# CVLAB-Unibo/Real-time-self-adaptive-deep-stereo

Measured on AMD Instinct MI355X. Metric: adapted stereo pairs/sec (whole node), MADNet full-backprop online adaptation 1242x375, higher is better.
Workload: dtype bf16 MFMA operands, f32 accumulate/storage (forward: split-bf16 = 3 MFMAs per product on the large 3x3 layers, exact f32 MFMA on the others, so the disparity stays within 1e-3 px; gradients: plain bf16); 1 GPU; MADNet FULL adaptation step (fwd+SSIM/L1 loss+EPE+bwd+momentum), 1242x375, 1 pair/GPU/step, private model per stream; precision=mixed, launch=hipGraph replay, step_sync=stream, concurrent_private_streams_per_gpu=1

## Files before the change

### include/madnet_hip_tune.h

```cpp
#ifndef MADNET_HIP_TUNE_H
#define MADNET_HIP_TUNE_H
#include <stdint.h>
#ifdef __cplusplus
extern "C" {
#endif

int mh_tune_conv_tile(int bm, int bn);
int mh_tune_conv_thin(int min_pixels);
int mh_tune_conv_patch(int mode);
int mh_tune_conv_x3_igemm(int on);
int mh_tune_conv_rows(int min_pixels);
int mh_tune_conv_bank_tile(int max_wgs);
int mh_tune_conv_bank_small(int mode);
int mh_tune_conv_bank(int small_maxpix);
int mh_tune_wgrad_wgs(int target_workgroups);
int mh_tune_wgrad_target_pct(int pct);
int mh_tune_wgrad_image(int on);
int mh_tune_wgrad_stream(int dist);
int mh_tune_corr(int direct);
int mh_tune_corr_row(int on);

int mh_tune_conv_planes(int mode);

#ifdef __cplusplus
}
#endif
#endif
```

### real-time-self-adaptive-deep-stereo_amd/csrc/corr.hip

```cpp
#include <algorithm>
#include <atomic>
#include <type_traits>
#include "mh_common.h"

namespace {

constexpr int MAXD_SMALL = 9;

struct CorrArgs {
    const float* L; const float* R; const float* u; float* out;
    int l_ld, r_ld, out_ld, coff;
    int B, H, W, C, md, stride, D;
    int copy_left, zero_tail, segs;
    unsigned l_bytes, r_bytes;
    int remap;
};

template <int LPP, int TW>
__global__ __launch_bounds__(256) void corr_fwd_small(CorrArgs p) {
    HIP_DYNAMIC_SHARED(float, smem)
    const int tid = threadIdx.x;
    const int seg = blockIdx.x % p.segs;
    const int row = blockIdx.x / p.segs;
    const int x0 = seg * TW;
// ... 218 lines not shown
            }
        }
        __syncthreads();
    }
    float w0[DT], w1[DT], uc = 0.f;
    int o0[DT], o1[DT];
#pragma unroll
    for (int j = 0; j < DT; ++j) {
#if defined(__clang__)
#pragma clang fp contract(off)
#endif
        const int xs = x + j - p.md;
        const bool in = live && j < p.D && (unsigned)xs < (unsigned)p.W;
        const int xq = in ? xs : 0;
        const float srcx = (float)xq * p.sx;
        const int x0 = (int)srcx, x1 = min(x0 + 1, p.Wc - 1);
        const float tx = srcx - (float)x0;
        float tl, tr, bl, br;
        if constexpr (HEAD) {
            const float* const Vs = fsm + 4 * (p.cwcap + 2) * p.K + 9 * p.K;
            const int i0 = in ? x0 - c_lo : 0, i1 = in ? x1 - c_lo : 0;
            tl = Vs[i0]; tr = Vs[i1]; bl = Vs[p.cwcap + i0]; br = Vs[p.cwcap + i1];
        } else { tl = V0[x0]; tr = V0[x1]; bl = V1[x0]; br = V1[x1]; }
        const float top = tl + (tr - tl) * tx, bot = bl + (br - bl) * tx;
        const float uj = (top + (bot - top) * ty) * p.mul;
        if (j == p.md) uc = uj;
        const float cx = (float)xq + uj;
        const float f0 = floorf(cx), f1 = f0 + 1.0f;
        const float xmax = (float)(p.W - 1);
        const float f0s = fminf(fmaxf(f0, 0.f), xmax), f1s = fminf(fmaxf(f1, 0.f), xmax);
        w0[j] = in ? (f1 - cx) * (f0 == f0s ? 1.f : 0.f) : 0.f;
        w1[j] = in ? (cx - f0) * (f1 == f1s ? 1.f : 0.f) : 0.f;
        o0[j] = in ? (row + (int)f0s) * p.r_ld * 4 : MH_OOB;
        o1[j] = in ? (row + (int)f1s) * p.r_ld * 4 : MH_OOB;
    }
    float accd[DT];
#pragma unroll
    for (int j = 0; j < DT; ++j) accd[j] = 0.f;
    float* Op = p.out + (int64_t)pp * p.out_ld;
    for (int c4 = sub; c4 < C4; c4 += LPP) {
        const float4 l = mh_buf_load4(rsL, live ? (pp * p.l_ld + c4 * 4) * 4 : MH_OOB);
        float4 a[DT], bb[DT];
#pragma unroll
        for (int j = 0; j < DT; ++j) {
            a[j] = mh_buf_load4(rsR, o0[j] == MH_OOB ? MH_OOB : o0[j] + c4 * 16);
            bb[j] = mh_buf_load4(rsR, o1[j] == MH_OOB ? MH_OOB : o1[j] + c4 * 16);
        }
        if (live) *reinterpret_cast<float4*>(Op + c4 * 4) = l;
        if (live && p.out_hi) {
            uint2 hi, lo;
            mh_split_bf16x2(l.x, l.y, hi.x, lo.x);
            mh_split_bf16x2(l.z, l.w, hi.y, lo.y);
            *reinterpret_cast<uint2*>(p.out_hi + (int64_t)pp * p.out_pld + c4 * 4) = hi;
            if (p.out_lo) *reinterpret_cast<uint2*>(p.out_lo + (int64_t)pp * p.out_pld + c4 * 4) = lo;
        }
#pragma unroll
        for (int j = 0; j < DT; ++j) {
            float4 r;
            r.x = w0[j] * a[j].x + w1[j] * bb[j].x; r.y = w0[j] * a[j].y + w1[j] * bb[j].y;
            r.z = w0[j] * a[j].z + w1[j] * bb[j].z; r.w = w0[j] * a[j].w + w1[j] * bb[j].w;
            accd[j] += l.x * r.x + l.y * r.y + l.z * r.z + l.w * r.w;
            if (j == p.md && live) *reinterpret_cast<float4*>(p.Rw + (int64_t)pp * p.rw_ld + c4 * 4) = r;
        }
    }
#pragma unroll
    for (int j = 0; j < DT; ++j) {
#pragma unroll
        for (int o = LPP >> 1; o > 0; o >>= 1) accd[j] += __shfl_xor(accd[j], o);
    }
    if (live) {
        const int nout = p.zero_tail ? p.out_ld - p.coff : p.D + 1;
        for (int e = sub; e < nout; e += LPP) {
            float v = 0.f;
#pragma unroll
            for (int j = 0; j < DT; ++j) v = (e == j) ? accd[j] * inv_c : v;
            if (e == p.D) v = uc;
            Op[p.coff + e] = v;
            if (p.out_hi && e <= p.D) {
                unsigned hi, lo;
                mh_split_bf16x2(v, 0.f, hi, lo);
                p.out_hi[(int64_t)pp * p.out_pld + p.coff + e] = (unsigned short)hi;
                if (p.out_lo) p.out_lo[(int64_t)pp * p.out_pld + p.coff + e] = (unsigned short)lo;
            }
        }
        if (sub == 0) p.u[pp] = uc;
    }
}

template <int TW>
__global__ __launch_bounds__(256) void corr_fwd_large(CorrArgs p) {
    HIP_DYNAMIC_SHARED(float, smem)
    const int tid = threadIdx.x;
    const int seg = blockIdx.x % p.segs;
    const int row = blockIdx.x / p.segs;
    const int x0 = seg * TW;
    const int C4 = p.C >> 2;
    const int rs = p.C + 4;
    const int win = TW + 2 * p.md;
    float* Ls = smem;
    float* Rs = smem + TW * rs;
    const float* Rrow = p.R + (int64_t)row * p.W * p.r_ld;
    const float* Lrow = p.L + (int64_t)row * p.W * p.l_ld;
    for (int q = tid; q < win * C4; q += 256) {
        const int px = q / C4, c4 = q - px * C4;
        const int xs = x0 - p.md + px;
        float4 v = make_float4(0.f, 0.f, 0.f, 0.f);
        if (xs >= 0 && xs < p.W) v = *reinterpret_cast<const float4*>(Rrow + (int64_t)xs * p.r_ld + c4 * 4);
        *reinterpret_cast<float4*>(&Rs[px * rs + c4 * 4]) = v;
    }
    for (int q = tid; q < TW * C4; q += 256) {
        const int px = q / C4, c4 = q - px * C4;
        const int x = x0 + px;
        float4 v = make_float4(0.f, 0.f, 0.f, 0.f);
        if (x < p.W) {
            v = *reinterpret_cast<const float4*>(Lrow + (int64_t)x * p.l_ld + c4 * 4);
            if (p.copy_left) *reinterpret_cast<float4*>(p.out + ((int64_t)row * p.W + x) * p.out_ld + c4 * 4) = v;
        }
        *reinterpret_cast<float4*>(&Ls[px * rs + c4 * 4]) = v;
    }
    __syncthreads();
    const float inv_c = 1.0f / (float)p.C;
    for (int q = tid; q < TW * p.D; q += 256) {
        const int pp = q / p.D, j = q - pp * p.D;
        const int x = x0 + pp;
        if (x >= p.W) continue;
        const float* l = &Ls[pp * rs];
        const float* r = &Rs[(pp + j * p.stride) * rs];
        float acc = 0.f;
        for (int c4 = 0; c4 < C4; ++c4) {
            const float4 a = *reinterpret_cast<const float4*>(l + c4 * 4);
            const float4 b = *reinterpret_cast<const float4*>(r + c4 * 4);
            acc += a.x * b.x + a.y * b.y + a.z * b.z + a.w * b.w;
        }
        p.out[((int64_t)row * p.W + x) * p.out_ld + p.coff + j] = acc * inv_c;
    }
    for (int pp = tid; pp < TW; pp += 256) {
        const int x = x0 + pp;
        if (x >= p.W) continue;
        const int64_t pix = (int64_t)row * p.W + x;
        float* Op = p.out + pix * p.out_ld;
        int tail = p.coff + p.D;
        if (p.u) { Op[tail] = p.u[pix]; ++tail; }
        if (p.zero_tail)
            for (; tail < p.out_ld; ++tail) Op[tail] = 0.f;
    }
}

struct CorrBwdArgs {
    const float* g; const float* L; const float* R; float* dL; float* dR; float* du;
    int g_ld, coff, l_ld, r_ld, dl_ld, dr_ld;
    int acc_l, acc_r, acc_u;
    int B, H, W, C, md, stride, D, copy_left;
    int64_t total;
};

__global__ __launch_bounds__(256) void corr_bwd_kernel(CorrBwdArgs p) {
    const int C4 = p.C >> 2;
    const float inv_c = 1.0f / (float)p.C;
    for (int64_t q = (int64_t)blockIdx.x * 256 + threadIdx.x; q < p.total; q += (int64_t)gridDim.x * 256) {
        const int c4 = (int)(q % C4);
        const int64_t pix = q / C4;
        const int x = (int)(pix % p.W);
        const int64_t rowbase = pix - x;
        const float* gp = p.g + pix * p.g_ld;
        float4 a = make_float4(0.f, 0.f, 0.f, 0.f), r = make_float4(0.f, 0.f, 0.f, 0.f);
        for (int j = 0; j < p.D; ++j) {
            const int i = j * p.stride - p.md;
            const int xs = x + i;
            if (xs >= 0 && xs < p.W) {
                const float gv = gp[p.coff + j];
                const float4 rv = *reinterpret_cast<const float4*>(p.R + (rowbase + xs) * p.r_ld + c4 * 4);
                a.x += gv * rv.x; a.y += gv * rv.y; a.z += gv * rv.z; a.w += gv * rv.w;
            }
            const int xl = x - i;
            if (xl >= 0 && xl < p.W) {
                const float gv = p.g[(rowbase + xl) * p.g_ld + p.coff + j];
                const float4 lv = *reinterpret_cast<const float4*>(p.L + (rowbase + xl) * p.l_ld + c4 * 4);
                r.x += gv * lv.x; r.y += gv * lv.y; r.z += gv * lv.z; r.w += gv * lv.w;
            }
        }
        a.x *= inv_c; a.y *= inv_c; a.z *= inv_c; a.w *= inv_c;
        r.x *= inv_c; r.y *= inv_c; r.z *= inv_c; r.w *= inv_c;
        if (p.copy_left) {
            const float4 gl = *reinterpret_cast<const float4*>(gp + c4 * 4);
            a.x += gl.x; a.y += gl.y; a.z += gl.z; a.w += gl.w;
        }
        float4* dl = reinterpret_cast<float4*>(p.dL + pix * p.dl_ld + c4 * 4);
        if (p.acc_l) { const float4 o = *dl; a.x += o.x; a.y += o.y; a.z += o.z; a.w += o.w; }
        *dl = a;
        float4* dr = reinterpret_cast<float4*>(p.dR + pix * p.dr_ld + c4 * 4);
        if (p.acc_r) { const float4 o = *dr; r.x += o.x; r.y += o.y; r.z += o.z; r.w += o.w; }
        *dr = r;
        if (p.du && c4 == 0) {
            const float gu = gp[p.coff + p.D];
            p.du[pix] = p.acc_u ? p.du[pix] + gu : gu;
        }
    }
}

template <int DT>
__global__ __launch_bounds__(256) void corr_bwd_direct(CorrBwdArgs p) {
    const int C4 = p.C >> 2;
    const float inv_c = 1.0f / (float)p.C;
    const int npix = p.B * p.H * p.W;
    const int q = blockIdx.x * 256 + threadIdx.x;
    const bool live = q < npix * C4;
    const int pix = live ? q / C4 : 0, c4 = live ? q - pix * C4 : 0;
    const int x = pix % p.W;
    const int rowbase = pix - x;
    const __amdgpu_buffer_rsrc_t rs_g = mh_make_rsrc(p.g, (unsigned)((size_t)npix * p.g_ld * 4));
    const __amdgpu_buffer_rsrc_t rs_r = mh_make_rsrc(p.R, (unsigned)(((size_t)npix - 1) * p.r_ld * 4 + (size_t)p.C * 4));
    const __amdgpu_buffer_rsrc_t rs_l = mh_make_rsrc(p.L, (unsigned)(((size_t)npix - 1) * p.l_ld * 4 + (size_t)p.C * 4));
    const __amdgpu_buffer_rsrc_t rs_dl = mh_make_rsrc(p.dL, (unsigned)(((size_t)npix - 1) * p.dl_ld * 4 + (size_t)p.C * 4));
    const __amdgpu_buffer_rsrc_t rs_dr = mh_make_rsrc(p.dR, (unsigned)(((size_t)npix - 1) * p.dr_ld * 4 + (size_t)p.C * 4));
    float gvr[DT], gvl[DT];
    float4 rvv[DT], lvv[DT];
    bool okr[DT], okl[DT];
#pragma unroll
    for (int j = 0; j < DT; ++j) {
        const int i = j * p.stride - p.md;
        const int xs = x + i, xl = x - i;
        okr[j] = live && j < p.D && xs >= 0 && xs < p.W; okl[j] = live && j < p.D && xl >= 0 && xl < p.W;
        gvr[j] = mh_buf_load1(rs_g, okr[j] ? (pix * p.g_ld + p.coff + j) * 4 : MH_OOB);
        gvl[j] = mh_buf_load1(rs_g, okl[j] ? ((rowbase + xl) * p.g_ld + p.coff + j) * 4 : MH_OOB);
        rvv[j] = mh_buf_load4(rs_r, okr[j] ? ((rowbase + xs) * p.r_ld + c4 * 4) * 4 : MH_OOB);
        lvv[j] = mh_buf_load4(rs_l, okl[j] ? ((rowbase + xl) * p.l_ld + c4 * 4) * 4 : MH_OOB);
    }
    const float4 gl = mh_buf_load4(rs_g, (live && p.copy_left) ? (pix * p.g_ld + c4 * 4) * 4 : MH_OOB);
    const float4 ol = mh_buf_load4(rs_dl, (live && p.acc_l) ? (pix * p.dl_ld + c4 * 4) * 4 : MH_OOB);
    const float4 orr = mh_buf_load4(rs_dr, (live && p.acc_r) ? (pix * p.dr_ld + c4 * 4) * 4 : MH_OOB);
    float4 a = make_float4(0.f, 0.f, 0.f, 0.f), r = make_float4(0.f, 0.f, 0.f, 0.f);
#pragma unroll
    for (int j = 0; j < DT; ++j) {
        if (okr[j]) { a.x += gvr[j] * rvv[j].x; a.y += gvr[j] * rvv[j].y; a.z += gvr[j] * rvv[j].z; a.w += gvr[j] * rvv[j].w; }
        if (okl[j]) { r.x += gvl[j] * lvv[j].x; r.y += gvl[j] * lvv[j].y; r.z += gvl[j] * lvv[j].z; r.w += gvl[j] * lvv[j].w; }
    }
    a.x *= inv_c; a.y *= inv_c; a.z *= inv_c; a.w *= inv_c;
    r.x *= inv_c; r.y *= inv_c; r.z *= inv_c; r.w *= inv_c;
    if (p.copy_left) { a.x += gl.x; a.y += gl.y; a.z += gl.z; a.w += gl.w; }
    if (p.acc_l) { a.x += ol.x; a.y += ol.y; a.z += ol.z; a.w += ol.w; }
    if (p.acc_r) { r.x += orr.x; r.y += orr.y; r.z += orr.z; r.w += orr.w; }
    if (!live) return;
    *reinterpret_cast<float4*>(p.dL + (int64_t)pix * p.dl_ld + c4 * 4) = a;
    *reinterpret_cast<float4*>(p.dR + (int64_t)pix * p.dr_ld + c4 * 4) = r;
    if (p.du && c4 == 0) {
        const float gu = p.g[(int64_t)pix * p.g_ld + p.coff + p.D];
        p.du[pix] = p.acc_u ? p.du[pix] + gu : gu;
    }
}

struct CorrWarpBwdArgs {
    const float* g; const float* L; const float* Rw; const float* img; const float* u;
    float* dL; float* dimg; float* du;
    int g_ld, coff, l_ld, rw_ld, img_ld, dl_ld, dimg_ld;
    int acc_l;
    int acc_img;
    int B, H, W, C, md, stride, D, copy_left;
};
template <int LPP, int DT = 0>
__global__ __launch_bounds__(256) void corr_warp_bwd_kernel(CorrWarpBwdArgs p) {
    const int C4 = p.C >> 2;
    constexpr int PPB = 256 / LPP;
    const float inv_c = 1.0f / (float)p.C;
    const int sub = threadIdx.x % LPP;
    const int64_t npix = (int64_t)p.B * p.H * p.W;
    const int64_t nit = (npix + PPB - 1) / PPB;
    for (int64_t it = blockIdx.x; it < nit; it += gridDim.x) {
        const int64_t pix = it * PPB + threadIdx.x / LPP;
        const bool live = pix < npix;
        const int64_t pp = live ? pix : 0;
        const int x = (int)(pp % p.W);
        const int64_t rowbase = pp - x;
        const float* gp = p.g + pp * p.g_ld;
        const float cx = (float)x + p.u[pp];
        const float x0 = floorf(cx), x1 = x0 + 1.0f;
        const float xmax = (float)(p.W - 1);
        const float x0s = fminf(fmaxf(x0, 0.f), xmax), x1s = fminf(fmaxf(x1, 0.f), xmax);
        const float m0 = (x0 == x0s) ? 1.f : 0.f, m1 = (x1 == x1s) ? 1.f : 0.f;
        const float w0 = (x1 - cx) * m0, w1 = (cx - x0) * m1;
        const int i0 = (int)x0s, i1 = (int)x1s;
        float dcx = 0.f;
        float gvr[DT > 0 ? DT : 1], gvl[DT > 0 ? DT : 1];
        int orw[DT > 0 ? DT : 1], ol[DT > 0 ? DT : 1];
        __amdgpu_buffer_rsrc_t rs_g, rs_rw, rs_l;
        if constexpr (DT > 0) {
            rs_g = mh_make_rsrc(p.g, (unsigned)(npix * p.g_ld * 4));
            rs_rw = mh_make_rsrc(p.Rw, (unsigned)(npix * p.rw_ld * 4));
            rs_l = mh_make_rsrc(p.L, (unsigned)(npix * p.l_ld * 4));
#pragma unroll
            for (int j = 0; j < DT; ++j) {
                const int i = j * p.stride - p.md;
                const int xs = x + i, xl = x - i;
                const bool okr = live && j < p.D && xs >= 0 && xs < p.W, okl = live && j < p.D && xl >= 0 && xl < p.W;
                gvr[j] = mh_buf_load1(rs_g, okr ? (int)((pp * p.g_ld + p.coff + j) * 4) : MH_OOB);
                gvl[j] = mh_buf_load1(rs_g, okl ? (int)(((rowbase + xl) * p.g_ld + p.coff + j) * 4) : MH_OOB);
                orw[j] = okr ? (int)((rowbase + xs) * p.rw_ld * 4) : MH_OOB;
                ol[j] = okl ? (int)((rowbase + xl) * p.l_ld * 4) : MH_OOB;
            }
        }
        for (int c4 = sub; c4 < C4; c4 += LPP) {
            if (!live) continue;
            float4 a = make_float4(0.f, 0.f, 0.f, 0.f), r = make_float4(0.f, 0.f, 0.f, 0.f);
            if constexpr (DT > 0) {
                float4 rvv[DT], lvv[DT];
#pragma unroll
                for (int j = 0; j < DT; ++j) {
                    rvv[j] = mh_buf_load4(rs_rw, orw[j] == MH_OOB ? MH_OOB : orw[j] + c4 * 16);
                    lvv[j] = mh_buf_load4(rs_l, ol[j] == MH_OOB ? MH_OOB : ol[j] + c4 * 16);
                }
#pragma unroll
                for (int j = 0; j < DT; ++j) {
                    if (orw[j] != MH_OOB) { a.x += gvr[j] * rvv[j].x; a.y += gvr[j] * rvv[j].y; a.z += gvr[j] * rvv[j].z; a.w += gvr[j] * rvv[j].w; }
                    if (ol[j] != MH_OOB) { r.x += gvl[j] * lvv[j].x; r.y += gvl[j] * lvv[j].y; r.z += gvl[j] * lvv[j].z; r.w += gvl[j] * lvv[j].w; }
                }
            } else
            for (int j = 0; j < p.D; ++j) {
                const int i = j * p.stride - p.md;
                const int xs = x + i;
                if (xs >= 0 && xs < p.W) {
                    const float gv = gp[p.coff + j];
                    const float4 rv = *reinterpret_cast<const float4*>(p.Rw + (rowbase + xs) * p.rw_ld + c4 * 4);
                    a.x += gv * rv.x; a.y += gv * rv.y; a.z += gv * rv.z; a.w += gv * rv.w;
                }
                const int xl = x - i;
                if (xl >= 0 && xl < p.W) {
                    const float gv = p.g[(rowbase + xl) * p.g_ld + p.coff + j];
                    const float4 lv = *reinterpret_cast<const float4*>(p.L + (rowbase + xl) * p.l_ld + c4 * 4);
                    r.x += gv * lv.x; r.y += gv * lv.y; r.z += gv * lv.z; r.w += gv * lv.w;
                }
            }
            a.x *= inv_c; a.y *= inv_c; a.z *= inv_c; a.w *= inv_c;
            r.x *= inv_c; r.y *= inv_c; r.z *= inv_c; r.w *= inv_c;
            if (p.copy_left) {
                const float4 gl = *reinterpret_cast<const float4*>(gp + c4 * 4);
                a.x += gl.x; a.y += gl.y; a.z += gl.z; a.w += gl.w;
            }
            float4* dl = reinterpret_cast<float4*>(p.dL + pp * p.dl_ld + c4 * 4);
            if (p.acc_l) { const float4 o = *dl; a.x += o.x; a.y += o.y; a.z += o.z; a.w += o.w; }
            *dl = a;
            if (p.dimg) {
                float* d0 = p.dimg + (rowbase + i0) * p.dimg_ld + c4 * 4;
                float* d1 = p.dimg + (rowbase + i1) * p.dimg_ld + c4 * 4;
                if (w0 != 0.f) { mh_atomic_add(d0 + 0, w0 * r.x); mh_atomic_add(d0 + 1, w0 * r.y); mh_atomic_add(d0 + 2, w0 * r.z); mh_atomic_add(d0 + 3, w0 * r.w); }
                if (w1 != 0.f) { mh_atomic_add(d1 + 0, w1 * r.x); mh_atomic_add(d1 + 1, w1 * r.y); mh_atomic_add(d1 + 2, w1 * r.z); mh_atomic_add(d1 + 3, w1 * r.w); }
            }
            if (p.du) {
                const float4 s0 = *reinterpret_cast<const float4*>(p.img + (rowbase + i0) * p.img_ld + c4 * 4);
                const float4 s1 = *reinterpret_cast<const float4*>(p.img + (rowbase + i1) * p.img_ld + c4 * 4);
                dcx += r.x * (m1 * s1.x - m0 * s0.x) + r.y * (m1 * s1.y - m0 * s0.y) + r.z * (m1 * s1.z - m0 * s0.z) + r.w * (m1 * s1.w - m0 * s0.w);
            }
        }
        if (p.du) {
#pragma unroll
            for (int o = LPP >> 1; o > 0; o >>= 1) dcx += __shfl_xor(dcx, o);
            if (live && sub == 0) p.du[pp] = gp[p.coff + p.D] + dcx;
        }
    }
}

template <int LPP, int DT, bool DET>
__global__ __launch_bounds__(1024) void corr_warp_bwd_row_kernel(CorrWarpBwdArgs p) {
    HIP_DYNAMIC_SHARED(float, smem)
    constexpr int NT = 1024, PPB = NT / LPP;
    using acc_t = typename std::conditional<DET, unsigned long long, float>::type;
    acc_t* const racc = reinterpret_cast<acc_t*>(smem);
    float* const su = smem + (size_t)p.W * p.C * (DET ? 2 : 1);
    const int tid = threadIdx.x, sub = tid % LPP;
    const int C4 = p.C >> 2;
    const float inv_c = 1.0f / (float)p.C;
    const int row = blockIdx.x;
    const int rowbase = row * p.W;
    const int npix = p.B * p.H * p.W;
    const __amdgpu_buffer_rsrc_t rs_g = mh_make_rsrc(p.g, (unsigned)((size_t)npix * p.g_ld * 4));
    const __amdgpu_buffer_rsrc_t rs_rw = mh_make_rsrc(p.Rw, (unsigned)((size_t)npix * p.rw_ld * 4));
    const __amdgpu_buffer_rsrc_t rs_l = mh_make_rsrc(p.L, (unsigned)((size_t)npix * p.l_ld * 4));
    const __amdgpu_buffer_rsrc_t rs_img = mh_make_rsrc(p.img, (unsigned)((size_t)npix * p.img_ld * 4));
    const __amdgpu_buffer_rsrc_t rs_dl = mh_make_rsrc(p.dL, (unsigned)((size_t)npix * p.dl_ld * 4));
    const int nq = p.W * C4;
    if constexpr (DET) {
        for (int i = tid; i < p.W * p.C; i += NT) racc[i] = 0ull;
    } else {
        for (int q = tid; q < nq; q += NT) {
            const int x = q / C4, c4 = q - x * C4;
            float4 v = make_float4(0.f, 0.f, 0.f, 0.f);
            if (p.dimg) v = *reinterpret_cast<const float4*>(p.dimg + (int64_t)(rowbase + x) * p.dimg_ld + c4 * 4);
            *reinterpret_cast<float4*>(racc + x * p.C + c4 * 4) = v;
        }
    }
    for (int x = tid; x < p.W; x += NT) su[x] = p.u[rowbase + x];
    __syncthreads();
    for (int xb = 0; xb < p.W; xb += PPB) {
        const int x = xb + tid / LPP;
        const bool live = x < p.W;
        const int pp = rowbase + (live ? x : 0);
// ... 855 lines not shown
    return ((size_t)4 * (cw + 2) * K + 9 * K + 2 * cw) * sizeof(float) <= 48 * 1024 ? 1 : 0;
}

static int level_front_launch(const float* X, int32_t x_ld, int32_t K, const float* hw, const float* hb,
                              const float* Vc, int32_t Hc, int32_t Wc, float mul, const float* L, int32_t l_ld, const float* R,
                              int32_t r_ld, float* out, int32_t out_ld, int32_t coff, float* Rw, int32_t rw_ld, float* u,
                              int32_t B, int32_t H, int32_t W, int32_t C, int32_t max_disp, int32_t zero_tail,
                              void* out_hi, void* out_lo, int32_t out_pld, void* stream) {
    MH_REQUIRE(!out_lo || out_hi, MH_ERR_ARG, "mh_level_front_fwd_planes: the lo plane needs the hi plane");
    MH_REQUIRE(!out_hi || (out_pld >= coff + 2 * max_disp + 2 && (out_pld & 3) == 0 && (((uintptr_t)out_hi) & 7u) == 0 && (((uintptr_t)out_lo) & 7u) == 0), MH_ERR_ARG,
               "mh_level_front_fwd_planes: out_pld must cover coff + D + 1 (multiple of 4), planes 8-byte aligned");
    MH_REQUIRE(Vc && L && R && out && Rw && u, MH_ERR_ARG, "mh_level_front_fwd: null argument");
    MH_REQUIRE(B > 0 && H > 0 && W > 0 && C > 0 && Hc > 0 && Wc > 0 && max_disp >= 0, MH_ERR_ARG, "mh_level_front_fwd: bad dimension");
    const int D = 2 * max_disp + 1;
    MH_REQUIRE(D <= MAXD_SMALL, MH_ERR_UNSUPPORTED, "mh_level_front_fwd: at most %d shifts (use mh_resize_fwd + mh_warp_fwd + mh_corr_fwd)", MAXD_SMALL);
    MH_REQUIRE(C % 4 == 0 && l_ld % 4 == 0 && r_ld % 4 == 0 && rw_ld % 4 == 0 && out_ld % 4 == 0 && mh_aligned16(L) && mh_aligned16(R) &&
               mh_aligned16(Rw) && mh_aligned16(out), MH_ERR_ALIGN, "mh_level_front_fwd: 16-byte rows required");
    MH_REQUIRE(coff >= C && coff + D + 1 <= out_ld && rw_ld >= C, MH_ERR_ARG, "mh_level_front_fwd: out_ld / coff / rw_ld too small");
    const int64_t npix = (int64_t)B * H * W;
    const int64_t lb = ((npix - 1) * l_ld + C) * 4, rb = ((npix - 1) * r_ld + C) * 4;
    MH_REQUIRE(npix < (1ll << 31) - 256 && lb < (1ll << 31) - 64 && rb < (1ll << 31) - 64, MH_ERR_UNSUPPORTED, "mh_level_front_fwd: tensors must be < 2 GiB");
    FrontArgs a;
    a.Vc = Vc; a.L = L; a.R = R; a.out = out; a.Rw = Rw; a.u = u; a.Hc = Hc; a.Wc = Wc; a.mul = mul;
    a.sy = (float)Hc / (float)H; a.sx = (float)Wc / (float)W;
    a.l_ld = l_ld; a.r_ld = r_ld; a.out_ld = out_ld; a.rw_ld = rw_ld; a.coff = coff;
    a.B = B; a.H = H; a.W = W; a.C = C; a.md = max_disp; a.D = D; a.zero_tail = zero_tail;
    a.l_bytes = (unsigned)lb; a.r_bytes = (unsigned)rb;
    a.out_hi = (unsigned short*)out_hi; a.out_lo = (unsigned short*)out_lo; a.out_pld = out_pld;
    a.X = nullptr; a.hw = nullptr; a.hb = nullptr; a.Vw = nullptr; a.x_ld = 0; a.K = 0; a.segs = 0; a.cwcap = 0; a.x_bytes = 0; a.rows2 = 0; a.rowpairs = 0;
    hipStream_t s = (hipStream_t)stream;
    const int C4 = C / 4;
    const int lpp = C4 <= 4 ? 4 : (C4 <= 8 ? 8 : 16);
    if (X) {
        MH_REQUIRE(mh_level_front_head_ok(Hc, Wc, H, W, C, K, max_disp) == 1, MH_ERR_UNSUPPORTED,
                   "mh_level_front_head_fwd: K = %d channels / %dx%d -> %dx%d not served (ask mh_level_front_head_ok; run the head as a launch of its own)", K, Hc, Wc, H, W);
        MH_REQUIRE(hw && x_ld >= K && x_ld % 4 == 0 && mh_aligned16(X) && mh_aligned16(hw), MH_ERR_ALIGN, "mh_level_front_head_fwd: X rows / head weights must be 16-byte aligned");
        const int64_t xb = (((int64_t)B * Hc * Wc - 1) * x_ld + K) * 4;
        MH_REQUIRE(xb < (1ll << 31) - 64, MH_ERR_UNSUPPORTED, "mh_level_front_head_fwd: X must be < 2 GiB");
        a.X = X; a.hw = hw; a.hb = hb; a.Vw = const_cast<float*>(Vc); a.x_ld = x_ld; a.K = K; a.x_bytes = (unsigned)xb;
        const int ppb = 256 / lpp;
        a.rows2 = (H == 2 * Hc && g_front_rows2.load(std::memory_order_relaxed)) ? 1 : 0;
        const int wpx = a.rows2 ? ppb / 2 : ppb;
        a.rowpairs = H / 2;
        a.segs = mh_cdiv(W, wpx);
        a.cwcap = front_head_cwcap(Wc, W, wpx, max_disp);
        const size_t lds = ((size_t)4 * (a.cwcap + 2) * K + 9 * K + 2 * a.cwcap) * sizeof(float);
        const dim3 g((unsigned)((int64_t)a.segs * B * (a.rows2 ? H / 2 : H)));
#define MH_FRONTH(LPPv)                                                                                                      \
    { if (D <= 5) hipLaunchKernelGGL((level_front_kernel<LPPv, 5, true>), g, dim3(256), lds, s, a);                          \
      else hipLaunchKernelGGL((level_front_kernel<LPPv, MAXD_SMALL, true>), g, dim3(256), lds, s, a); }
        if (lpp == 4) MH_FRONTH(4) else if (lpp == 8) MH_FRONTH(8) else MH_FRONTH(16)
#undef MH_FRONTH
        mh_note_kernel("level_front_kernel<LPP=%d,DT=%d,HEAD=%d> grid %d lds %d", lpp, D <= 5 ? 5 : MAXD_SMALL, K, (int)g.x, (int)lds);
        return mh_check_launch("level_front_head_fwd");
    }
    auto grid = [&](int l) { return dim3((unsigned)((npix * l + 255) / 256)); };
#define MH_FRONT(LPPv)                                                                                              \
    { if (D <= 5) hipLaunchKernelGGL((level_front_kernel<LPPv, 5, false>), grid(LPPv), dim3(256), 0, s, a);                \
      else hipLaunchKernelGGL((level_front_kernel<LPPv, MAXD_SMALL, false>), grid(LPPv), dim3(256), 0, s, a); }
    if (lpp == 4) MH_FRONT(4) else if (lpp == 8) MH_FRONT(8) else MH_FRONT(16)
#undef MH_FRONT
    mh_note_kernel("level_front_kernel<LPP=%d,DT=%d>", lpp, D <= 5 ? 5 : MAXD_SMALL);
    return mh_check_launch("level_front_fwd");
}

extern "C" int mh_level_front_fwd_planes(const float* Vc, int32_t Hc, int32_t Wc, float mul, const float* L, int32_t l_ld, const float* R,
                                         int32_t r_ld, float* out, int32_t out_ld, int32_t coff, float* Rw, int32_t rw_ld, float* u,
                                         int32_t B, int32_t H, int32_t W, int32_t C, int32_t max_disp, int32_t zero_tail,
                                         void* out_hi, void* out_lo, int32_t out_pld, void* stream) {
    return level_front_launch(nullptr, 0, 0, nullptr, nullptr, Vc, Hc, Wc, mul, L, l_ld, R, r_ld, out, out_ld, coff, Rw, rw_ld, u, B, H, W, C, max_disp, zero_tail, out_hi, out_lo,
                              out_pld, stream);
}
extern "C" int mh_level_front_head_fwd(const float* X, int32_t x_ld, int32_t K, const float* hw, const float* hb, float* Vc, int32_t Hc, int32_t Wc, float mul,
                                       const float* L, int32_t l_ld, const float* R, int32_t r_ld, float* out, int32_t out_ld, int32_t coff, float* Rw, int32_t rw_ld,
                                       float* u, int32_t B, int32_t H, int32_t W, int32_t C, int32_t max_disp, int32_t zero_tail,
                                       void* out_hi, void* out_lo, int32_t out_pld, void* stream) {
    MH_REQUIRE(X, MH_ERR_ARG, "mh_level_front_head_fwd: null argument");
    return level_front_launch(X, x_ld, K, hw, hb, Vc, Hc, Wc, mul, L, l_ld, R, r_ld, out, out_ld, coff, Rw, rw_ld, u, B, H, W, C, max_disp, zero_tail, out_hi, out_lo, out_pld,
                              stream);
}

extern "C" int mh_corr_warp_bwd(const float* g, int32_t g_ld, int32_t coff, const float* L, int32_t l_ld, const float* Rw, int32_t rw_ld,
                                const float* img, int32_t img_ld, const float* u, float* dL, int32_t dl_ld, int32_t acc_l,
                                float* dimg, int32_t dimg_ld, float* du,
                                int32_t B, int32_t H, int32_t W, int32_t C, int32_t max_disp, int32_t stride, int32_t copy_left, void* stream) {
    MH_REQUIRE(g && L && Rw && img && u && dL && (dimg || du), MH_ERR_ARG, "mh_corr_warp_bwd: null argument");
    MH_REQUIRE(B > 0 && H > 0 && W > 0 && C > 0 && max_disp >= 0 && stride >= 1, MH_ERR_ARG, "mh_corr_warp_bwd: bad dimension");
    MH_REQUIRE(C % 4 == 0 && l_ld % 4 == 0 && rw_ld % 4 == 0 && img_ld % 4 == 0 && dl_ld % 4 == 0 && (!dimg || dimg_ld % 4 == 0) &&
               mh_aligned16(L) && mh_aligned16(Rw) && mh_aligned16(img) && mh_aligned16(dL), MH_ERR_ALIGN,
               "mh_corr_warp_bwd: channel counts / lds must be multiples of 4 and pointers 16-byte aligned");
    MH_REQUIRE(!copy_left || (g_ld % 4 == 0 && mh_aligned16(g)), MH_ERR_ALIGN, "mh_corr_warp_bwd: copy_left needs aligned g rows");
    CorrWarpBwdArgs a;
    a.g = g; a.L = L; a.Rw = Rw; a.img = img; a.u = u; a.dL = dL; a.dimg = dimg; a.du = du;
    a.g_ld = g_ld; a.coff = coff; a.l_ld = l_ld; a.rw_ld = rw_ld; a.img_ld = img_ld; a.dl_ld = dl_ld; a.dimg_ld = dimg_ld;
    a.acc_l = acc_l & 1;
    a.acc_img = (acc_l & MH_CORR_WARP_OVERWRITE_DIMG) ? 0 : 1;
    a.B = B; a.H = H; a.W = W; a.C = C; a.md = max_disp; a.stride = stride; a.D = 2 * max_disp / stride + 1; a.copy_left = copy_left;
    const int C4 = C / 4;
    const int64_t npix = (int64_t)B * H * W;
    hipStream_t s = (hipStream_t)stream;
    auto zero_dimg = [&]() -> int {
        if (a.acc_img || !dimg) return 0;
        hipError_t e = (dimg_ld == C) ? hipMemsetAsync(dimg, 0, (size_t)npix * C * 4, s) : hipMemset2DAsync(dimg, (size_t)dimg_ld * 4, 0, (size_t)C * 4, (size_t)npix, s);
        if (e != hipSuccess) { mh_set_error("mh_corr_warp_bwd: zeroing dimg: %s", hipGetErrorString(e)); return (int)e; }
        a.acc_img = 1;
        return 0;
    };
    auto grid = [&](int lpp) { int64_t b = (npix * lpp + 255) / 256; return (int)(b > (1 << 20) ? (1 << 20) : b); };
    const int64_t ldmax = g_ld > rw_ld ? (g_ld > l_ld ? g_ld : l_ld) : (rw_ld > l_ld ? rw_ld : l_ld);
    const bool fast = a.D <= 5 && npix * ldmax * 4 < (1ll << 31) - 64;
    const bool det = g_corr_det_ranges.load() > 0;
    const size_t row_lds = ((size_t)W * C * (det ? 8 : 4) + (size_t)W * 4 + 15) & ~(size_t)15;
    const int64_t ldmax2 = std::max<int64_t>(std::max<int64_t>(ldmax, img_ld), std::max<int64_t>(dl_ld, dimg ? dimg_ld : 0));
    if (g_corr_row.load() && fast && row_lds <= 150 * 1024 && npix * ldmax2 * 4 < (1ll << 31) - 64 && (int64_t)B * H < (1 << 30)) {
        const dim3 grid((unsigned)(B * H));
        const int lpp = C4 <= 8 ? 8 : C4 <= 16 ? 16 : 32;
        const size_t lds_st = ((size_t)3 * W * C + (size_t)W * (8 + 1 + 2 + 1 + 1 + 2 + 8) + 8) * 4;
        if ((g_corr_row.load() & 2) == 0 && C4 <= 32 && W <= 3 * (1024 / lpp) && (int64_t)W * C4 <= 3 * 1024 && W * 8 <= 3 * 1024 && W < 32768 && lds_st <= 155 * 1024) {
            if (g_corr_row.load() & 4) a.dimg = nullptr;
            if (lpp == 8) hipLaunchKernelGGL((corr_warp_bwd_rowlds_kernel<8, 5>), grid, dim3(1024), lds_st, s, a);
            else if (lpp == 16) hipLaunchKernelGGL((corr_warp_bwd_rowlds_kernel<16, 5>), grid, dim3(1024), lds_st, s, a);
            else hipLaunchKernelGGL((corr_warp_bwd_rowlds_kernel<32, 5>), grid, dim3(1024), lds_st, s, a);
            mh_note_kernel("corr_warp_bwd_rowlds_kernel<LPP=%d,DT=5> C=%d D=%d grid %d x 16 waves lds %d", lpp, C, a.D, B * H, (int)lds_st);
            return mh_check_launch("corr_warp_bwd_rowlds");
        }
        if (int rc = zero_dimg()) return rc;
#define MH_CWB_ROW(LPPv) { if (det) hipLaunchKernelGGL((corr_warp_bwd_row_kernel<LPPv, 5, true>), grid, dim3(1024), row_lds, s, a);   \
                           else hipLaunchKernelGGL((corr_warp_bwd_row_kernel<LPPv, 5, false>), grid, dim3(1024), row_lds, s, a); }
        if (C4 <= 4) MH_CWB_ROW(4) else if (C4 <= 8) MH_CWB_ROW(8) else MH_CWB_ROW(16)
#undef MH_CWB_ROW
        mh_note_kernel("corr_warp_bwd_row_kernel<LPP=%d,DT=5%s> C=%d D=%d grid %d x 16 waves lds %d", C4 <= 4 ? 4 : C4 <= 8 ? 8 : 16, det ? ",det" : "", C, a.D, B * H, (int)row_lds);
        return mh_check_launch("corr_warp_bwd_row");
    }
    if (int rc = zero_dimg()) return rc;
    if (fast) {
        if (C4 <= 4) hipLaunchKernelGGL((corr_warp_bwd_kernel<4, 5>), dim3(grid(4)), dim3(256), 0, s, a);
        else if (C4 <= 8) hipLaunchKernelGGL((corr_warp_bwd_kernel<8, 5>), dim3(grid(8)), dim3(256), 0, s, a);
        else hipLaunchKernelGGL((corr_warp_bwd_kernel<16, 5>), dim3(grid(16)), dim3(256), 0, s, a);
    } else if (C4 <= 4) hipLaunchKernelGGL((corr_warp_bwd_kernel<4>), dim3(grid(4)), dim3(256), 0, s, a);
    else if (C4 <= 8) hipLaunchKernelGGL((corr_warp_bwd_kernel<8>), dim3(grid(8)), dim3(256), 0, s, a);
    else hipLaunchKernelGGL((corr_warp_bwd_kernel<16>), dim3(grid(16)), dim3(256), 0, s, a);
    mh_note_kernel("corr_warp_bwd_kernel<LPP=%d%s> C=%d D=%d", C4 <= 4 ? 4 : C4 <= 8 ? 8 : 16, fast ? ",DT=5" : "", C, a.D);
    return mh_check_launch("corr_warp_bwd");
}

extern "C" int mh_corr_bwd(const float* g, int32_t g_ld, int32_t coff, const float* L, int32_t l_ld,
                           const float* R, int32_t r_ld, float* dL, int32_t dl_ld, int32_t acc_l,
                           float* dR, int32_t dr_ld, int32_t acc_r, float* du, int32_t acc_u,
                           int32_t B, int32_t H, int32_t W, int32_t C, int32_t max_disp, int32_t stride,
                           int32_t copy_left, void* stream) {
    return mh_corr_bwd_prec(g, g_ld, coff, L, l_ld, R, r_ld, dL, dl_ld, acc_l, dR, dr_ld, acc_r, du, acc_u, B, H, W, C, max_disp, stride, copy_left, 0, stream);
}

extern "C" int mh_corr_bwd_prec(const float* g, int32_t g_ld, int32_t coff, const float* L, int32_t l_ld,
                                const float* R, int32_t r_ld, float* dL, int32_t dl_ld, int32_t acc_l,
                                float* dR, int32_t dr_ld, int32_t acc_r, float* du, int32_t acc_u,
                                int32_t B, int32_t H, int32_t W, int32_t C, int32_t max_disp, int32_t stride,
                                int32_t copy_left, int32_t precision, void* stream) {
    MH_REQUIRE(precision >= 0 && precision <= 2, MH_ERR_ARG, "mh_corr_bwd_prec: precision must be 0 (fp32), 1 (bf16) or 2 (split-bf16: runs as fp32)");
    MH_REQUIRE(g && L && R && dL && dR, MH_ERR_ARG, "mh_corr_bwd: null argument");
    MH_REQUIRE(B > 0 && H > 0 && W > 0 && C > 0 && max_disp >= 0 && stride >= 1, MH_ERR_ARG, "mh_corr_bwd: bad dimension");
    MH_REQUIRE(C % 4 == 0 && l_ld % 4 == 0 && r_ld % 4 == 0 && dl_ld % 4 == 0 && dr_ld % 4 == 0 &&
               mh_aligned16(L) && mh_aligned16(R) && mh_aligned16(dL) && mh_aligned16(dR), MH_ERR_ALIGN,
               "mh_corr_bwd: channel counts / lds must be multiples of 4 and pointers 16-byte aligned");
    MH_REQUIRE(!copy_left || (g_ld % 4 == 0 && mh_aligned16(g)), MH_ERR_ALIGN, "mh_corr_bwd: copy_left needs aligned g rows");
    CorrBwdArgs a;
    a.g = g; a.L = L; a.R = R; a.dL = dL; a.dR = dR; a.du = du;
    a.g_ld = g_ld; a.coff = coff; a.l_ld = l_ld; a.r_ld = r_ld; a.dl_ld = dl_ld; a.dr_ld = dr_ld;
    a.acc_l = acc_l; a.acc_r = acc_r; a.acc_u = acc_u;
    a.B = B; a.H = H; a.W = W; a.C = C; a.md = max_disp; a.stride = stride; a.D = 2 * max_disp / stride + 1;
    a.copy_left = copy_left;
    a.total = (int64_t)B * H * W * (C / 4);
    if (precision == 1 && g_corr_direct && a.D > MAXD_SMALL && stride == 1 && !copy_left && !du && C % 16 == 0 && C >= 32 && C <= 256 &&
        (C == 32 || C == 64 || C == 128 || C == 256) && (int64_t)B * H * W * std::max(std::max(g_ld, l_ld), r_ld) * 4 < (1ll << 31) - 64) {
        const int nks = (2 * max_disp + 16 + 31) / 32, rows = 48 + 32 * nks, DPh = (((a.D + 3) & ~3) + 7) & ~7;
        const size_t tile = (size_t)64 * (C + 4) * 4;
        const size_t lds_r = std::max(tile, ((size_t)rows * (C + 16) + (size_t)rows * DPh) * 2);
        if (lds_r <= 150 * 1024) {
            const int segs = mh_cdiv(W, 64);
            const dim3 grid(segs * B * H);
            hipStream_t s = (hipStream_t)stream;
            const int remap = g_corr_remap.load();
#define MH_CORRBH(CSv) { if (g_corr_pair.load()) hipLaunchKernelGGL((corr_bwd_mfma_bf16_pair<CSv>), dim3(2 * segs * B * H), dim3(256), lds_r, s, a, segs, remap);  \
                         else { hipLaunchKernelGGL((corr_bwd_mfma_bf16_one<CSv, false>), dim3(segs * B * H), dim3(256), lds_r, s, a, segs, remap);                   \
                                hipLaunchKernelGGL((corr_bwd_mfma_bf16_one<CSv, true>), dim3(segs * B * H), dim3(256), lds_r, s, a, segs, remap); } }
            switch (C) {
                case 32: MH_CORRBH(2) break;
                case 64: MH_CORRBH(4) break;
                case 128: MH_CORRBH(8) break;
                default: MH_CORRBH(16) break;
            }
#undef MH_CORRBH
            mh_note_kernel("corr_bwd_mfma_bf16_pair<C/16=%d> left + right in %s of %d x 4 waves, lds %d", C / 16, g_corr_pair.load() ? "one grid" : "two grids", (g_corr_pair.load() ? 2 : 1) * segs * B * H, (int)lds_r);
            return mh_check_launch("corr_bwd_mfma_bf16");
        }
    }
    {
        const int nb = (2 * max_disp + 31) / 16, rows = 48 + 16 * nb, DP = (a.D + 3) & ~3;
        const size_t lds_l = ((size_t)rows * (C + 4) + 64 * DP) * sizeof(float), lds_r = ((size_t)rows * (C + 4) + (size_t)rows * DP) * sizeof(float);
        if (g_corr_direct && a.D > MAXD_SMALL && stride == 1 && !copy_left && !du && (C == 16 || C == 32 || C == 64 || C == 128 || C == 256) &&
            lds_r <= 150 * 1024 && (int64_t)B * H * W < (1ll << 31) / 64) {
            const int segs = mh_cdiv(W, 64);
            const dim3 grid(segs * B * H);
            hipStream_t s = (hipStream_t)stream;
#define MH_CORRB(CSv)                                                                                        \
            hipLaunchKernelGGL((corr_bwd_mfma<CSv, false>), grid, dim3(CSv >= 2 ? 512 : 256), lds_l, s, a, segs);  \
            hipLaunchKernelGGL((corr_bwd_mfma<CSv, true>), grid, dim3(CSv >= 2 ? 512 : 256), lds_r, s, a, segs);
            switch (C) {
                case 16: MH_CORRB(1) break;
                case 32: MH_CORRB(2) break;
                case 64: MH_CORRB(4) break;
                case 128: MH_CORRB(8) break;
                default: MH_CORRB(16) break;
            }
#undef MH_CORRB
            mh_note_kernel("corr_bwd_mfma<C/16=%d> left + right (exact fp32)", C / 16);
            return mh_check_launch("corr_bwd_mfma");
        }
    }
    {
        const int64_t npix = (int64_t)B * H * W;
        const int64_t ldm = std::max(std::max(std::max(g_ld, l_ld), std::max(r_ld, dl_ld)), dr_ld);
        if (g_corr_direct && a.D <= 5 && npix * ldm * 4 < (1ll << 31) - 64 && a.total < (1ll << 31) - 256) {
            hipLaunchKernelGGL(corr_bwd_direct<5>, dim3((unsigned)((a.total + 255) / 256)), dim3(256), 0, (hipStream_t)stream, a);
            mh_note_kernel("corr_bwd_direct<DT=5> C=%d D=%d", C, a.D);
            return mh_check_launch("corr_bwd_direct");
        }
    }
    int blocks = (int)((a.total + 255) / 256);
    if (blocks > 256 * 16) blocks = 256 * 16;
    hipLaunchKernelGGL(corr_bwd_kernel, dim3(blocks), dim3(256), 0, (hipStream_t)stream, a);
    mh_note_kernel("corr_bwd_kernel C=%d D=%d", C, a.D);
    return mh_check_launch("corr_bwd");
}

extern "C" int mh_det_sync_corr(const void* t) {
    g_corr_det_ranges = reinterpret_cast<const mh_det_table*>(t)->n;
    return mh_det_upload(*reinterpret_cast<const mh_det_table*>(t));
}
extern "C" int mh_det_ovf_corr(void) { return mh_det_overflow_take(); }
```

### real-time-self-adaptive-deep-stereo_amd/csrc/lib.hip

```cpp
#include "mh_common.h"
#include <stdarg.h>
#include <string.h>
#include <mutex>
#include <vector>

static thread_local char g_err[512] = "";

void mh_set_error(const char* fmt, ...) {
    va_list ap;
    va_start(ap, fmt);
    vsnprintf(g_err, sizeof(g_err), fmt, ap);
    va_end(ap);
}

static thread_local char g_last_kernel[160] = "";
void mh_note_kernel(const char* fmt, ...) {
    va_list ap;
    va_start(ap, fmt);
    vsnprintf(g_last_kernel, sizeof(g_last_kernel), fmt, ap);
    va_end(ap);
}
extern "C" const char* mh_last_kernel(void) { return g_last_kernel; }

int mh_check_launch(const char* what) {
// ... 196 lines not shown
            mh_conv_desc d; desc_from_op(o, d);
            return mh_conv2d_planes_bwd(&d, p[0], i[23], p[1], p[2], i[24], (float*)p[3], p[4], i[25], s);
        }
        case MH_OP_CONV_IMAGE:
            return mh_conv_image_fwd((const float*)p[0], i[0], i[1], i[2], i[3], i[4], i[5], i[6], i[7], o.f[0], o.f[1], (const float*)p[1], (const float*)p[2], i[8], i[9], i[10],
                                     i[11], o.f[2], (float*)p[3], i[12], p[4], i[13], s);
        case MH_OP_DET_FLUSH:
            return mh_det_flush((float*)p[0], p[1], o.n, s);
        case MH_OP_ALLREDUCE: {
            float* bufs[MH_ALLREDUCE_MAX_BUFS]; int64_t counts[MH_ALLREDUCE_MAX_BUFS];
            const int nb = i[0];
            if (nb < 1 || nb > MH_ALLREDUCE_MAX_BUFS) { mh_set_error("MH_OP_ALLREDUCE: %d buffers", nb); return MH_ERR_ARG; }
            for (int k = 0; k < nb; ++k) { bufs[k] = (float*)p[1 + k]; counts[k] = i[1 + k]; }
            return mh_allreduce_sum(bufs, counts, nb, p[0], s);
        }
        case MH_OP_FETCH_INPUTS: {
            float* dst[MH_FETCH_MAX]; int64_t cnt[MH_FETCH_MAX];
            const int nb = i[0];
            if (nb < 1 || nb > MH_FETCH_MAX) { mh_set_error("MH_OP_FETCH_INPUTS: %d entries", nb); return MH_ERR_ARG; }
            for (int k = 0; k < nb; ++k) { dst[k] = (float*)p[1 + k]; cnt[k] = i[1 + k]; }
            return mh_fetch_inputs((const mh_input_table*)p[0], dst, cnt, nb, s);
        }
        case MH_OP_STAMP:
            return mh_stamp(p[0], s);
        case MH_OP_PLANE_SPLIT:
            return mh_plane_split((const mh_plane_seg*)p[0], i[0], i[1], s);
        case MH_OP_PACK_W:
            return mh_pack_weights((const mh_pack_seg*)p[0], i[0], i[1], s);
        case MH_OP_WGRAD_REDUCE:
            return mh_wgrad_reduce((const mh_wgrad_seg*)p[0], i[0], i[1], s);
        case MH_OP_CORR_FWD:
            return mh_corr_fwd_prec((const float*)p[0], i[0], (const float*)p[1], i[1], (const float*)p[2], (float*)p[3], i[2], i[3],
                                    i[4], i[5], i[6], i[7], i[8], i[9], i[10], i[11], i[12], s);
        case MH_OP_CORR_BWD:
            return mh_corr_bwd_prec((const float*)p[0], i[0], i[1], (const float*)p[1], i[2], (const float*)p[2], i[3],
                                    (float*)p[3], i[4], i[5], (float*)p[4], i[6], i[7], (float*)p[5], i[8],
                                    i[9], i[10], i[11], i[12], i[13], i[14], i[15], i[16], s);
        case MH_OP_WARP_FWD:
            return mh_warp_fwd((const float*)p[0], i[0], (const float*)p[1], (float*)p[2], i[1], i[2], i[3], i[4], i[5], s);
        case MH_OP_WARP_BWD:
            return mh_warp_bwd((const float*)p[0], i[0], (const float*)p[1], i[1], (const float*)p[2], (float*)p[3], i[2],
                               (float*)p[4], i[3], i[4], i[5], i[6], i[7], s);
        case MH_OP_RESIZE_FWD:
            return mh_resize_fwd((const float*)p[0], (float*)p[1], i[0], i[1], i[2], i[3], i[4], i[5], i[6], i[7], i[8], o.f[0], i[9], s);
        case MH_OP_RESIZE_BWD:
            return mh_resize_bwd((const float*)p[0], (const float*)p[1], (float*)p[2], i[10], i[0], i[1], i[2], i[3], i[4], i[5], i[6],
                                 i[7], i[8], o.f[0], i[9], s);
        case MH_OP_LEVEL_FRONT:
            if (p[8])
                return mh_level_front_head_fwd((const float*)p[8], i[14], i[15], (const float*)p[9], (const float*)p[10], (float*)p[0], i[0], i[1], o.f[0],
                                               (const float*)p[1], i[2], (const float*)p[2], i[3], (float*)p[3], i[4], i[5], (float*)p[4], i[6], (float*)p[5],
                                               i[7], i[8], i[9], i[10], i[11], i[12], p[6], p[7], i[13], s);
            return mh_level_front_fwd_planes((const float*)p[0], i[0], i[1], o.f[0], (const float*)p[1], i[2], (const float*)p[2], i[3], (float*)p[3],
                                             i[4], i[5], (float*)p[4], i[6], (float*)p[5], i[7], i[8], i[9], i[10], i[11], i[12], p[6], p[7], i[13], s);
        case MH_OP_RESIZE_IMAGE:
            return mh_resize_image_fwd((const float*)p[0], (float*)p[1], i[0], i[1], i[2], i[3], i[4], i[5], s);
        case MH_OP_PAD_REFLECT:
            return mh_pad_reflect((const float*)p[0], (float*)p[1], i[0], i[1], i[2], i[3], i[4], i[5], i[6], i[7], i[8], o.f[0], o.f[1], s);
        case MH_OP_LOSS:
            return mh_reprojection_loss_phase((const float*)p[0], (const float*)p[1], (const float*)p[2], (float*)p[3], (float*)p[4],
                                              (float*)p[5], o.f[0], i[0], i[1], i[2], i[3], s);
        case MH_OP_METRICS:
            return mh_metrics((const float*)p[0], (const float*)p[1], (float*)p[2], (float*)p[3], o.f[0], i[0], i[1], i[2], s);
        case MH_OP_MOMENTUM:
            return mh_momentum((float*)p[0], (float*)p[1], (const float*)p[2], o.n, o.f[0], o.f[1], o.f[2], s);
        case MH_OP_COPY_CH:
            return mh_copy_channels((const float*)p[0], i[0], (float*)p[1], i[1], o.n, i[2], o.f[0], i[3], s);
        case MH_OP_LEAKY_BWD:
            return mh_leaky_bwd((float*)p[0], i[0], (const float*)p[1], i[1], o.n, i[2], o.f[0], s);
        case MH_OP_FILL:
            return mh_fill((float*)p[0], o.n, o.f[0], s);
        case MH_OP_BIAS_GRAD:
            if (i[2] > 0) return mh_bias_grad_partial((const float*)p[0], i[0], o.n, i[1], (float*)p[1], i[2], s);
            return mh_bias_grad((const float*)p[0], i[0], o.n, i[1], (float*)p[1], s);
        default:
            mh_set_error("mh_plan_run: unknown op kind %d", o.kind);
            return MH_ERR_ARG;
    }
}

#define MH_HIP(call)                                                        \
    do {                                                                    \
        hipError_t e_ = (call);                                             \
        if (e_ != hipSuccess) {                                             \
            mh_set_error("%s: %s", #call, hipGetErrorString(e_));           \
            return (int)e_;                                                 \
        }                                                                   \
    } while (0)

namespace {
struct Lanes {
    hipStream_t aux[MH_MAX_LANES] = {};
    hipEvent_t ev[32] = {};
    int next = 0;
    bool ready = false;
};
struct LanePool {
    std::mutex m;
    std::vector<Lanes*> free_[16];
};
LanePool& lane_pool() { static LanePool* p = new LanePool; return *p; }
struct ThreadLanes {
    Lanes* l[16] = {};
    ~ThreadLanes() {
        LanePool& P = lane_pool();
        std::lock_guard<std::mutex> g(P.m);
        for (int d = 0; d < 16; ++d)
            if (l[d]) { P.free_[d].push_back(l[d]); l[d] = nullptr; }
    }
};
thread_local ThreadLanes t_lanes;

int lane_device(int* dev) {
    MH_HIP(hipGetDevice(dev));
    MH_REQUIRE(*dev >= 0 && *dev < 16, MH_ERR_UNSUPPORTED, "device index %d out of range", *dev);
    return 0;
}
int lanes_take(int dev, Lanes** out) {
    LanePool& P = lane_pool();
    Lanes* L = nullptr;
    {
        std::lock_guard<std::mutex> g(P.m);
        if (!P.free_[dev].empty()) { L = P.free_[dev].back(); P.free_[dev].pop_back(); }
    }
    if (!L) {
        L = new Lanes;
        for (int k = 1; k < MH_MAX_LANES; ++k) MH_HIP(hipStreamCreateWithFlags(&L->aux[k], hipStreamNonBlocking));
        for (auto& e : L->ev) MH_HIP(hipEventCreateWithFlags(&e, hipEventDisableTiming));
        L->ready = true;
    }
    *out = L;
    return 0;
}
int lanes_get(Lanes** out) {
    int dev = 0;
    if (int e = lane_device(&dev)) return e;
    if (!t_lanes.l[dev])
        if (int e = lanes_take(dev, &t_lanes.l[dev])) return e;
    *out = t_lanes.l[dev];
    return 0;
}
}
static int mh_lanes_init() { Lanes* L = nullptr; return lanes_get(&L); }
namespace {
int lane_edge(Lanes& L, hipStream_t from, hipStream_t to) {
    hipEvent_t e = L.ev[L.next];
    L.next = (L.next + 1) & 31;
    MH_HIP(hipEventRecord(e, from));
    MH_HIP(hipStreamWaitEvent(to, e, 0));
    return 0;
}
}

static int run_wgrad_batch(const mh_op* ops, int m, void* s) {
    mh_wgrad_item items[16];
    for (int k = 0; k < m; ++k) {
        const mh_op& o = ops[k];
        desc_from_op(o, items[k].d);
        items[k].in = (const float*)o.p[0]; items[k].dout = (const float*)o.p[1];
        items[k].ws = (float*)o.p[2]; items[k].db = (float*)o.p[3];
        items[k].dout_ld = o.i[21]; items[k].splits = o.i[23];
        items[k].group_max_m = o.i[24]; items[k].reserved = 0;
    }
    return mh_conv2d_wgrad_partial_group(items, m, s);
}

static int plan_run_impl(const mh_op* ops, int32_t nops, void* stream, Lanes* fixed) {
    MH_REQUIRE(ops || nops == 0, MH_ERR_ARG, "mh_plan_run: null plan");
    Lanes* L = fixed;
    bool dirty[MH_MAX_LANES] = {};
    bool stale[MH_MAX_LANES];
    for (bool& b : stale) b = true;
    hipStream_t main_s = (hipStream_t)stream;
    auto join = [&]() -> int {
        for (int l = 1; l < MH_MAX_LANES; ++l)
            if (dirty[l]) { if (int e = lane_edge(*L, L->aux[l], main_s)) return e; dirty[l] = false; }
        return 0;
    };
    struct Deferred { int32_t k; int m, lane; };
    Deferred deferred[64];
    int ndef = 0;
    auto flush_deferred = [&]() -> int {
        for (int q = 0; q < ndef; ++q) {
            const Deferred& d = deferred[q];
            const int e = d.m > 1 ? run_wgrad_batch(ops + d.k, d.m, (void*)L->aux[d.lane]) : run_op(ops[d.k], (void*)L->aux[d.lane]);
            if (e) { ndef = 0; return e; }
        }
        ndef = 0;
        return 0;
    };
    for (int32_t k = 0; k < nops; ++k) {
        const int sched = ops[k].i[26];
        const int lane = sched & 0xff;
        int e = 0;
        if (lane >= MH_MAX_LANES) { mh_set_error("lane %d out of range", lane); e = MH_ERR_ARG; }
        if (!e && ndef && ((sched & MH_OP_JOIN) || ((sched >> 16) & 0xff) || ndef >= 60)) e = flush_deferred();
        if (!e && (sched & MH_OP_JOIN)) e = join();
        if (!e && ((sched >> 16) & 0xff)) {
            if (lane > 0 && !L) e = lanes_get(&L);
            hipStream_t tgt = lane > 0 ? L->aux[lane] : main_s;
            for (int l = 1; l < MH_MAX_LANES && !e; ++l)
                if ((((sched >> 16) >> l) & 1) && l != lane && dirty[l]) {
                    e = lane_edge(*L, L->aux[l], tgt);
                    if (lane == 0) dirty[l] = false;
                }
        }
        int m = 1;
        if (ops[k].kind == MH_OP_WGRAD_PARTIAL)
            while (m < 16 && k + m < nops && ops[k + m].kind == MH_OP_WGRAD_PARTIAL && (ops[k + m].i[26] & ~MH_OP_NODEFER) == lane) ++m;
        auto run = [&](void* s) -> int { return m > 1 ? run_wgrad_batch(ops + k, m, s) : run_op(ops[k], s); };
        if (!e && lane > 0) {
            if (!L) e = lanes_get(&L);
            if (!e && stale[lane]) { e = lane_edge(*L, main_s, L->aux[lane]); stale[lane] = false; }
            if (!e) {
                dirty[lane] = true;
                const bool at_once = (sched & MH_OP_NODEFER) && !((sched >> 16) & 0xff);
                if (!at_once) { deferred[ndef].k = k; deferred[ndef].m = m; deferred[ndef].lane = lane; ++ndef; }
                else {
                    if (ndef) e = flush_deferred();
                    if (!e) e = run((void*)L->aux[lane]);
                }
            }
        } else if (!e) {
            e = run(stream);
            for (bool& b : stale) b = true;
            if (!e && ndef) e = flush_deferred();
        }
        if (e != 0) {
            char tmp[400];
            strncpy(tmp, g_err, sizeof(tmp) - 1); tmp[sizeof(tmp) - 1] = 0;
            mh_set_error("plan op %d (kind %d): %s", k, ops[k].kind, tmp);
            ndef = 0;
            join();
            return e;
        }
        k += m - 1;
    }
    if (ndef) { if (int e = flush_deferred()) { join(); return e; } }
    return join();
}

extern "C" int mh_plan_run(const mh_op* ops, int32_t nops, void* stream) { return plan_run_impl(ops, nops, stream, nullptr); }

namespace {
struct ThreadBranches {
    std::vector<Lanes*> sets[16];
    ~ThreadBranches() {
        LanePool& P = lane_pool();
        std::lock_guard<std::mutex> g(P.m);
        for (int d = 0; d < 16; ++d) { for (Lanes* L : sets[d]) P.free_[d].push_back(L); sets[d].clear(); }
    }
};
thread_local ThreadBranches t_branches;
int branch_get(int idx, Lanes** out) {
    int dev = 0;
    if (int e = lane_device(&dev)) return e;
    auto& v = t_branches.sets[dev];
    while ((int)v.size() <= idx) {
        Lanes* L = nullptr;
        if (int e = lanes_take(dev, &L)) return e;
        v.push_back(L);
    }
    *out = v[idx];
    return 0;
}
}
extern "C" int mh_plans_prepare(int32_t nplans) {
    MH_REQUIRE(nplans >= 1 && nplans <= 16, MH_ERR_ARG, "mh_plans_prepare: 1 .. 16 plans");
    for (int i = 1; i < nplans; ++i) { Lanes* L = nullptr; if (int e = branch_get(i - 1, &L)) return e; }
    return mh_lanes_init();
}
extern "C" int mh_plans_run(const mh_plan_ref* plans, int32_t nplans, void* stream) {
    MH_REQUIRE(plans && nplans >= 1 && nplans <= 16, MH_ERR_ARG, "mh_plans_run: 1 .. 16 plans");
    for (int i = 0; i < nplans; ++i) {
        MH_REQUIRE(plans[i].ops || plans[i].nops == 0, MH_ERR_ARG, "mh_plans_run: null plan %d", i);
        for (int k = 0; k < plans[i].nops; ++k)
            MH_REQUIRE((plans[i].ops[k].i[26] & 0xff) < MH_MAX_LANES - 1, MH_ERR_UNSUPPORTED, "mh_plans_run: plan %d uses lane %d (the last lane is the branch stream)", i,
                       plans[i].ops[k].i[26] & 0xff);
    }
    hipStream_t s0 = (hipStream_t)stream;
    Lanes* sets[16] = {};
    for (int i = 1; i < nplans; ++i) {
        if (int e = branch_get(i - 1, &sets[i])) return e;
        if (int e = lane_edge(*sets[i], s0, sets[i]->aux[MH_MAX_LANES - 1])) return e;
    }
    int rc = 0;
    for (int i = 0; i < nplans && !rc; ++i)
        rc = plan_run_impl(plans[i].ops, plans[i].nops, i == 0 ? (void*)s0 : (void*)sets[i]->aux[MH_MAX_LANES - 1], i == 0 ? nullptr : sets[i]);
    for (int i = 1; i < nplans; ++i)
        if (int e = lane_edge(*sets[i], sets[i]->aux[MH_MAX_LANES - 1], s0)) { if (!rc) rc = e; }
    return rc;
}


extern "C" int mh_graph_begin(void* stream) {
    { Lanes* L = nullptr; if (int e = lanes_get(&L)) return e; }
    MH_HIP(hipStreamBeginCapture((hipStream_t)stream, hipStreamCaptureModeThreadLocal));
    return 0;
}
extern "C" int mh_graph_end(void* stream, void** graph_exec_out) {
    MH_REQUIRE(graph_exec_out, MH_ERR_ARG, "mh_graph_end: null output");
    hipGraph_t g = nullptr;
    MH_HIP(hipStreamEndCapture((hipStream_t)stream, &g));
    hipGraphExec_t ge = nullptr;
    hipError_t e = hipGraphInstantiate(&ge, g, nullptr, nullptr, 0);
    (void)hipGraphDestroy(g);
    if (e != hipSuccess) { mh_set_error("hipGraphInstantiate: %s", hipGetErrorString(e)); return (int)e; }
    *graph_exec_out = (void*)ge;
    return 0;
}
extern "C" int mh_graph_launch(void* graph_exec, void* stream) {
    MH_HIP(hipGraphLaunch((hipGraphExec_t)graph_exec, (hipStream_t)stream));
    return 0;
}
extern "C" int mh_graph_destroy(void* graph_exec) {
    if (graph_exec) MH_HIP(hipGraphExecDestroy((hipGraphExec_t)graph_exec));
    return 0;
}
extern "C" int mh_event_create(void** ev) {
    MH_REQUIRE(ev, MH_ERR_ARG, "mh_event_create: null output");
    hipEvent_t e; MH_HIP(hipEventCreate(&e)); *ev = (void*)e; return 0;
}
extern "C" int mh_event_record(void* ev, void* stream) { MH_HIP(hipEventRecord((hipEvent_t)ev, (hipStream_t)stream)); return 0; }
extern "C" int mh_event_elapsed_ms(void* a, void* b, float* ms) {
    MH_REQUIRE(ms, MH_ERR_ARG, "mh_event_elapsed_ms: null output");
    MH_HIP(hipEventSynchronize((hipEvent_t)b));
    MH_HIP(hipEventElapsedTime(ms, (hipEvent_t)a, (hipEvent_t)b));
    return 0;
}
extern "C" int mh_event_destroy(void* ev) { if (ev) MH_HIP(hipEventDestroy((hipEvent_t)ev)); return 0; }
extern "C" int mh_stream_sync(void* stream) { MH_HIP(hipStreamSynchronize((hipStream_t)stream)); return 0; }
```

### real-time-self-adaptive-deep-stereo_amd/csrc/ops.hip

```cpp
#include "mh_common.h"

namespace {

__device__ __forceinline__ float clampf(float v, float lo, float hi) { return fminf(fmaxf(v, lo), hi); }

struct WarpArgs {
    const float* img; const float* u; const float* g; float* out; float* dimg; float* du;
    int img_ld, out_ld, g_ld, dimg_ld, acc_u;
    int B, H, W, C;
    int64_t total;
};

__global__ __launch_bounds__(256) void warp_fwd_kernel(WarpArgs p) {
    const int C4 = p.C >> 2;
    for (int64_t q = (int64_t)blockIdx.x * 256 + threadIdx.x; q < p.total; q += (int64_t)gridDim.x * 256) {
        const int c4 = (int)(q % C4);
        const int64_t pix = q / C4;
        const int x = (int)(pix % p.W);
        const int64_t rowbase = pix - x;
        const float cx = (float)x + p.u[pix];
        const float x0 = floorf(cx), x1 = x0 + 1.0f;
        const float xmax = (float)(p.W - 1);
        const float x0s = clampf(x0, 0.f, xmax), x1s = clampf(x1, 0.f, xmax);
        const float w0 = (x1 - cx) * (x0 == x0s ? 1.f : 0.f);
        const float w1 = (cx - x0) * (x1 == x1s ? 1.f : 0.f);
        const float4 a = *reinterpret_cast<const float4*>(p.img + (rowbase + (int)x0s) * p.img_ld + c4 * 4);
        const float4 b = *reinterpret_cast<const float4*>(p.img + (rowbase + (int)x1s) * p.img_ld + c4 * 4);
        float4 o;
        o.x = w0 * a.x + w1 * b.x; o.y = w0 * a.y + w1 * b.y;
        o.z = w0 * a.z + w1 * b.z; o.w = w0 * a.w + w1 * b.w;
        *reinterpret_cast<float4*>(p.out + pix * p.out_ld + c4 * 4) = o;
    }
}

template <int LPP>
__global__ __launch_bounds__(256) void warp_bwd_kernel(WarpArgs p) {
    const int C4 = p.C >> 2;
    constexpr int PPB = 256 / LPP;
    const int sub = threadIdx.x % LPP;
    const int64_t npix = (int64_t)p.B * p.H * p.W;
    const int64_t nit = (npix + PPB - 1) / PPB;
    for (int64_t it = blockIdx.x; it < nit; it += gridDim.x) {
        const int64_t pix = it * PPB + threadIdx.x / LPP;
        const bool live = pix < npix;
        const int64_t pp = live ? pix : 0;
        const int x = (int)(pp % p.W);
        const int64_t rowbase = pp - x;
        const float cx = (float)x + p.u[pp];
        const float x0 = floorf(cx), x1 = x0 + 1.0f;
        const float xmax = (float)(p.W - 1);
        const float x0s = clampf(x0, 0.f, xmax), x1s = clampf(x1, 0.f, xmax);
        const float m0 = (x0 == x0s) ? 1.f : 0.f, m1 = (x1 == x1s) ? 1.f : 0.f;
        const float w0 = (x1 - cx) * m0, w1 = (cx - x0) * m1;
        const int i0 = (int)x0s, i1 = (int)x1s;
        float dcx = 0.f;
        for (int c4 = sub; c4 < C4; c4 += LPP) {
            if (!live) continue;
            const float4 gv = *reinterpret_cast<const float4*>(p.g + pp * p.g_ld + c4 * 4);
            if (p.dimg) {
                float* d0 = p.dimg + (rowbase + i0) * p.dimg_ld + c4 * 4;
                float* d1 = p.dimg + (rowbase + i1) * p.dimg_ld + c4 * 4;
                if (w0 != 0.f) { mh_atomic_add(d0 + 0, w0 * gv.x); mh_atomic_add(d0 + 1, w0 * gv.y); mh_atomic_add(d0 + 2, w0 * gv.z); mh_atomic_add(d0 + 3, w0 * gv.w); }
                if (w1 != 0.f) { mh_atomic_add(d1 + 0, w1 * gv.x); mh_atomic_add(d1 + 1, w1 * gv.y); mh_atomic_add(d1 + 2, w1 * gv.z); mh_atomic_add(d1 + 3, w1 * gv.w); }
            }
            if (p.du) {
                const float4 a = *reinterpret_cast<const float4*>(p.img + (rowbase + i0) * p.img_ld + c4 * 4);
                const float4 b = *reinterpret_cast<const float4*>(p.img + (rowbase + i1) * p.img_ld + c4 * 4);
                dcx += gv.x * (m1 * b.x - m0 * a.x) + gv.y * (m1 * b.y - m0 * a.y) +
                       gv.z * (m1 * b.z - m0 * a.z) + gv.w * (m1 * b.w - m0 * a.w);
            }
        }
        if (p.du) {
#pragma unroll
            for (int o = LPP >> 1; o > 0; o >>= 1) dcx += __shfl_xor(dcx, o);
            if (live && sub == 0) p.du[pp] = p.acc_u ? p.du[pp] + dcx : dcx;
        }
    }
}

struct ResizeArgs {
    const float* in; const float* g; float* out; float* din;
    int B, Hi, Wi, Hr, Wr, cy, cx, Ho, Wo, mode, accumulate;
    float mul, sy, sx;
};

__device__ __forceinline__ void interp1(int i, float scale, int n, int& lo, int& hi, float& t) {
    const float src = (float)i * scale;
    lo = (int)src;
    hi = min(lo + 1, n - 1);
    t = src - (float)lo;
}

__device__ __forceinline__ float bilerp(const float* img, int Wi, int y0, int y1, float ty, int x0, int x1, float tx,
                                        float mul, bool relu_in) {
#if defined(__clang__)
#pragma clang fp contract(off)
#endif
    float tl = img[(int64_t)y0 * Wi + x0], tr = img[(int64_t)y0 * Wi + x1];
    float bl = img[(int64_t)y1 * Wi + x0], br = img[(int64_t)y1 * Wi + x1];
    if (relu_in) {
        tl = fmaxf(tl * mul, 0.f); tr = fmaxf(tr * mul, 0.f);
        bl = fmaxf(bl * mul, 0.f); br = fmaxf(br * mul, 0.f);
    }
    const float top = tl + (tr - tl) * tx;
    const float bot = bl + (br - bl) * tx;
    return top + (bot - top) * ty;
}

__global__ __launch_bounds__(256) void resize_fwd_kernel(ResizeArgs p) {
    const int64_t total = (int64_t)p.B * p.Ho * p.Wo;
    for (int64_t q = (int64_t)blockIdx.x * 256 + threadIdx.x; q < total; q += (int64_t)gridDim.x * 256) {
        const int x = (int)(q % p.Wo);
        const int64_t t2 = q / p.Wo;
        const int y = (int)(t2 % p.Ho);
        const int b = (int)(t2 / p.Ho);
        int y0, y1, x0, x1; float ty, tx;
        interp1(y + p.cy, p.sy, p.Hi, y0, y1, ty);
        interp1(x + p.cx, p.sx, p.Wi, x0, x1, tx);
        const float* img = p.in + (int64_t)b * p.Hi * p.Wi;
        float v = bilerp(img, p.Wi, y0, y1, ty, x0, x1, tx, p.mul, p.mode == 1);
        if (p.mode == 0) v *= p.mul;
        else if (p.mode == 2) v = fmaxf(v * p.mul, 0.f);
        p.out[q] = v;
    }
}

template <int LPP>
__global__ __launch_bounds__(256) void resize_bwd_kernel(ResizeArgs p) {
    const int64_t total = (int64_t)p.B * p.Hi * p.Wi;
    const float isy = 1.0f / p.sy, isx = 1.0f / p.sx;
    const int sub = LPP > 1 ? (int)(threadIdx.x % LPP) : 0;
    const int64_t nit = (total * LPP + 255) / 256;
    for (int64_t it = blockIdx.x; it < nit; it += gridDim.x) {
        const int64_t q0 = (it * 256 + threadIdx.x) / LPP;
        const bool live = q0 < total;
        const int64_t q = live ? q0 : 0;
        const int sx = (int)(q % p.Wi);
        const int64_t t2 = q / p.Wi;
        const int sy = (int)(t2 % p.Hi);
        const int b = (int)(t2 / p.Hi);
        const float* img = p.in + (int64_t)b * p.Hi * p.Wi;
        const float* gimg = p.g + (int64_t)b * p.Ho * p.Wo;
        const int ya = max(p.cy, (int)floorf((float)(sy - 1) * isy) - 1);
        const int yb = min(p.cy + p.Ho - 1, (int)ceilf((float)(sy + 1) * isy) + 1);
        const int xa = max(p.cx, (int)floorf((float)(sx - 1) * isx) - 1);
        const int xb = min(p.cx + p.Wo - 1, (int)ceilf((float)(sx + 1) * isx) + 1);
        float acc = 0.f;
        for (int Y = ya + sub; Y <= yb && live; Y += LPP) {
            int y0, y1; float ty;
            interp1(Y, p.sy, p.Hi, y0, y1, ty);
            const float wy = (y0 == sy ? 1.0f - ty : 0.f) + (y1 == sy ? ty : 0.f);
            if (wy == 0.f) continue;
            for (int X = xa; X <= xb; ++X) {
                int x0, x1; float tx;
                interp1(X, p.sx, p.Wi, x0, x1, tx);
                const float wx = (x0 == sx ? 1.0f - tx : 0.f) + (x1 == sx ? tx : 0.f);
                if (wx == 0.f) continue;
                float gv = gimg[(int64_t)(Y - p.cy) * p.Wo + (X - p.cx)];
                if (p.mode == 2) {
                    const float z = bilerp(img, p.Wi, y0, y1, ty, x0, x1, tx, p.mul, false) * p.mul;
                    if (!(z > 0.f)) gv = 0.f;
                }
                acc += gv * wy * wx;
            }
        }
#pragma unroll
        for (int o = LPP >> 1; o > 0; o >>= 1) acc += __shfl_xor(acc, o);
        if (live && sub == 0) {
            acc *= p.mul;
            if (p.mode == 1 && !(img[(int64_t)sy * p.Wi + sx] * p.mul > 0.f)) acc = 0.f;
            p.din[q] = p.accumulate ? p.din[q] + acc : acc;
        }
    }
}

struct HeadBwdArgs {
    ResizeArgs rz;
    const float* a1; const float* a2; int a1_ld, a2_ld;
    float* dV; unsigned short* dV_sh; int dV_sh_ld;
    const float* w; float* dx; const float* mask_ref; unsigned short* dx_sh;
    int N, dx_ld, mask_ld, dx_sh_ld, acc_dx, kind;
    float mask_alpha;
    int tiles_x, tiles_y;
};
#define HB_TH 4
#define HB_TW 32
__device__ __forceinline__ float head_dv_from_du(const ResizeArgs& p, int b, int sy, int sx, bool exact2) {
    const float* gimg = p.g + (int64_t)b * p.Ho * p.Wo;
    if (exact2) {
        float v[9], wgt[9];
        bool ok[9];
#pragma unroll
        for (int dy = -1; dy <= 1; ++dy) {
            const int Y = 2 * sy + dy;
            const bool oky = (unsigned)Y < (unsigned)p.Ho;
            const int Yc = oky ? Y : 2 * sy;
            const float wy = dy == 0 ? 1.0f : ((dy == 1 && sy == p.Hi - 1) ? 1.0f : 0.5f);
#pragma unroll
            for (int dx = -1; dx <= 1; ++dx) {
                const int X = 2 * sx + dx;
                const bool okx = (unsigned)X < (unsigned)p.Wo;
                const int Xc = okx ? X : 2 * sx;
                const float wx = dx == 0 ? 1.0f : ((dx == 1 && sx == p.Wi - 1) ? 1.0f : 0.5f);
                const int k = (dy + 1) * 3 + dx + 1;
                v[k] = gimg[(int64_t)Yc * p.Wo + Xc] * wy;
                wgt[k] = wx; ok[k] = oky && okx;
            }
        }
        float acc = 0.f;
#pragma unroll
        for (int k = 0; k < 9; ++k) acc += ok[k] ? v[k] * wgt[k] : 0.f;
        return acc * p.mul;
    }
    const float isy = 1.0f / p.sy, isx = 1.0f / p.sx;
    const int ya = max(p.cy, (int)floorf((float)(sy - 1) * isy) - 1);
    const int yb = min(p.cy + p.Ho - 1, (int)ceilf((float)(sy + 1) * isy) + 1);
    const int xa = max(p.cx, (int)floorf((float)(sx - 1) * isx) - 1);
    const int xb = min(p.cx + p.Wo - 1, (int)ceilf((float)(sx + 1) * isx) + 1);
    float acc = 0.f;
    for (int Y = ya; Y <= yb; ++Y) {
        int y0, y1; float ty;
        interp1(Y, p.sy, p.Hi, y0, y1, ty);
        const float wy = (y0 == sy ? 1.0f - ty : 0.f) + (y1 == sy ? ty : 0.f);
        if (wy == 0.f) continue;
        for (int X = xa; X <= xb; ++X) {
            int x0, x1; float tx;
            interp1(X, p.sx, p.Wi, x0, x1, tx);
            const float wx = (x0 == sx ? 1.0f - tx : 0.f) + (x1 == sx ? tx : 0.f);
            if (wx == 0.f) continue;
            acc += gimg[(int64_t)(Y - p.cy) * p.Wo + (X - p.cx)] * wy * wx;
        }
    }
    return acc * p.mul;
}
__global__ __launch_bounds__(256) void head_bwd_kernel(HeadBwdArgs p) {
    __shared__ float sV[(HB_TH + 2) * (HB_TW + 2)];
    __shared__ __attribute__((aligned(16))) float sW[9 * 64];
    const int tid = threadIdx.x;
    const int H = p.rz.Hi, W = p.rz.Wi;
    const int tx = blockIdx.x % p.tiles_x;
    const int t2 = blockIdx.x / p.tiles_x;
    const int ty = t2 % p.tiles_y, b = t2 / p.tiles_y;
    const int y0 = ty * HB_TH, x0 = tx * HB_TW;
    const bool exact2 = p.kind == 0 && p.rz.Hr == 2 * H && p.rz.Wr == 2 * W && p.rz.cy == 0 && p.rz.cx == 0 && p.rz.Ho == p.rz.Hr && p.rz.Wo == p.rz.Wr;
    for (int i = tid; i < 9 * p.N; i += 256) sW[i] = p.w[i];
    if (tid < (HB_TH + 2) * (HB_TW + 2)) {
        const int ly = tid / (HB_TW + 2), lx = tid - ly * (HB_TW + 2);
        const int y = y0 - 1 + ly, x = x0 - 1 + lx;
        float v = 0.f;
        if ((unsigned)y < (unsigned)H && (unsigned)x < (unsigned)W) {
            const int64_t pix = ((int64_t)b * H + y) * W + x;
            if (p.kind == 0) v = head_dv_from_du(p.rz, b, y, x, exact2);
            else v = (p.a1 ? p.a1[pix * p.a1_ld] : 0.f) + (p.a2 ? p.a2[pix * p.a2_ld] : 0.f);
            if (ly >= 1 && ly <= HB_TH && lx >= 1 && lx <= HB_TW) {
                p.dV[pix] = v;
                if (p.dV_sh) p.dV_sh[pix * p.dV_sh_ld] = (unsigned short)mh_pack_bf16(v, 0.f);
            }
        }
        sV[tid] = v;
    }
    __syncthreads();
    const int G4 = p.N >> 2;
    if (G4 <= 16 && (p.acc_dx || p.mask_ref)) {
        constexpr int MAXIT = HB_TH * HB_TW * 16 / 256;
        float4 oldv[MAXIT], mkv[MAXIT];
#pragma unroll
        for (int it = 0; it < MAXIT; ++it) {
            const int i = tid + it * 256;
            const int g = i % G4, px = i / G4;
            const int iy = px / HB_TW, ix = px - iy * HB_TW;
            const int y = y0 + iy, x = x0 + ix;
            const bool live = i < HB_TH * HB_TW * G4 && y < H && x < W;
            const int64_t m = ((int64_t)b * H + (live ? y : y0)) * W + (live ? x : x0);
            oldv[it] = (live && p.acc_dx) ? *reinterpret_cast<const float4*>(p.dx + m * p.dx_ld + g * 4) : make_float4(0.f, 0.f, 0.f, 0.f);
            mkv[it] = (live && p.mask_ref) ? *reinterpret_cast<const float4*>(p.mask_ref + m * p.mask_ld + g * 4) : make_float4(1.f, 1.f, 1.f, 1.f);
        }
#pragma unroll
        for (int it = 0; it < MAXIT; ++it) {
            const int i = tid + it * 256;
            if (i >= HB_TH * HB_TW * G4) break;
            const int g = i % G4, px = i / G4;
            const int iy = px / HB_TW, ix = px - iy * HB_TW;
            const int y = y0 + iy, x = x0 + ix;
            if (y >= H || x >= W) continue;
            const int n = g * 4;
            float4 v = make_float4(0.f, 0.f, 0.f, 0.f);
#pragma unroll
            for (int t = 0; t < 9; ++t) {
                const int ky = t / 3, kx = t - ky * 3;
                const float z = sV[(iy + 2 - ky) * (HB_TW + 2) + ix + 2 - kx];
                const float4 w = *reinterpret_cast<const float4*>(sW + t * p.N + n);
                v.x += z * w.x; v.y += z * w.y; v.z += z * w.z; v.w += z * w.w;
            }
            const int64_t m = ((int64_t)b * H + y) * W + x;
            float* dst = p.dx + m * p.dx_ld + n;
            if (p.acc_dx) { const float4 o = oldv[it]; v.x += o.x; v.y += o.y; v.z += o.z; v.w += o.w; }
            if (p.mask_ref) {
                const float4 mk = mkv[it];
                v.x *= mk.x > 0.f ? 1.0f : p.mask_alpha; v.y *= mk.y > 0.f ? 1.0f : p.mask_alpha;
                v.z *= mk.z > 0.f ? 1.0f : p.mask_alpha; v.w *= mk.w > 0.f ? 1.0f : p.mask_alpha;
            }
            *reinterpret_cast<float4*>(dst) = v;
            if (p.dx_sh) *reinterpret_cast<uint2*>(p.dx_sh + m * p.dx_sh_ld + n) = make_uint2(mh_pack_bf16(v.x, v.y), mh_pack_bf16(v.z, v.w));
        }
        return;
    }
    for (int i = tid; i < HB_TH * HB_TW * G4; i += 256) {
        const int g = i % G4, px = i / G4;
        const int iy = px / HB_TW, ix = px - iy * HB_TW;
        const int y = y0 + iy, x = x0 + ix;
        if (y >= H || x >= W) continue;
        const int n = g * 4;
        float4 v = make_float4(0.f, 0.f, 0.f, 0.f);
#pragma unroll
        for (int t = 0; t < 9; ++t) {
            const int ky = t / 3, kx = t - ky * 3;
            const float z = sV[(iy + 2 - ky) * (HB_TW + 2) + ix + 2 - kx];
            const float4 w = *reinterpret_cast<const float4*>(sW + t * p.N + n);
            v.x += z * w.x; v.y += z * w.y; v.z += z * w.z; v.w += z * w.w;
        }
        const int64_t m = ((int64_t)b * H + y) * W + x;
        float* dst = p.dx + m * p.dx_ld + n;
        if (p.acc_dx) { const float4 o = *reinterpret_cast<const float4*>(dst); v.x += o.x; v.y += o.y; v.z += o.z; v.w += o.w; }
        if (p.mask_ref) {
            const float4 mk = *reinterpret_cast<const float4*>(p.mask_ref + m * p.mask_ld + n);
            v.x *= mk.x > 0.f ? 1.0f : p.mask_alpha; v.y *= mk.y > 0.f ? 1.0f : p.mask_alpha;
            v.z *= mk.z > 0.f ? 1.0f : p.mask_alpha; v.w *= mk.w > 0.f ? 1.0f : p.mask_alpha;
        }
        *reinterpret_cast<float4*>(dst) = v;
        if (p.dx_sh) *reinterpret_cast<uint2*>(p.dx_sh + m * p.dx_sh_ld + n) = make_uint2(mh_pack_bf16(v.x, v.y), mh_pack_bf16(v.z, v.w));
    }
}

struct ResizeImgArgs { const float* in; const float* g; float* out; float* din; int B, Hi, Wi, C, Ho, Wo; float sy, sx; };

__global__ __launch_bounds__(256) void resize_image_fwd_kernel(ResizeImgArgs p) {
    const int64_t total = (int64_t)p.B * p.Ho * p.Wo * p.C;
    for (int64_t q = (int64_t)blockIdx.x * 256 + threadIdx.x; q < total; q += (int64_t)gridDim.x * 256) {
        const int c = (int)(q % p.C);
        int64_t t = q / p.C;
        const int x = (int)(t % p.Wo); t /= p.Wo;
        const int y = (int)(t % p.Ho);
        const int b = (int)(t / p.Ho);
        int y0, y1, x0, x1; float ty, tx;
        interp1(y, p.sy, p.Hi, y0, y1, ty);
        interp1(x, p.sx, p.Wi, x0, x1, tx);
        const float* img = p.in + (int64_t)b * p.Hi * p.Wi * p.C + c;
        const float tl = img[((int64_t)y0 * p.Wi + x0) * p.C], tr = img[((int64_t)y0 * p.Wi + x1) * p.C];
        const float bl = img[((int64_t)y1 * p.Wi + x0) * p.C], br = img[((int64_t)y1 * p.Wi + x1) * p.C];
        const float top = tl + (tr - tl) * tx, bot = bl + (br - bl) * tx;
        p.out[q] = top + (bot - top) * ty;
    }
}

__global__ __launch_bounds__(256) void resize_image_bwd_kernel(ResizeImgArgs p) {
    const int64_t total = (int64_t)p.B * p.Hi * p.Wi * p.C;
    const float isy = 1.0f / p.sy, isx = 1.0f / p.sx;
    for (int64_t q = (int64_t)blockIdx.x * 256 + threadIdx.x; q < total; q += (int64_t)gridDim.x * 256) {
        const int c = (int)(q % p.C);
        int64_t t = q / p.C;
        const int sx = (int)(t % p.Wi); t /= p.Wi;
        const int sy = (int)(t % p.Hi);
        const int b = (int)(t / p.Hi);
        const float* gimg = p.g + (int64_t)b * p.Ho * p.Wo * p.C + c;
        const int ya = max(0, (int)floorf((float)(sy - 1) * isy) - 1), yb = min(p.Ho - 1, (int)ceilf((float)(sy + 1) * isy) + 1);
        const int xa = max(0, (int)floorf((float)(sx - 1) * isx) - 1), xb = min(p.Wo - 1, (int)ceilf((float)(sx + 1) * isx) + 1);
        float acc = 0.f;
        for (int Y = ya; Y <= yb; ++Y) {
            int y0, y1; float ty;
            interp1(Y, p.sy, p.Hi, y0, y1, ty);
            const float wy = (y0 == sy ? 1.0f - ty : 0.f) + (y1 == sy ? ty : 0.f);
            if (wy == 0.f) continue;
            for (int X = xa; X <= xb; ++X) {
                int x0, x1; float tx;
                interp1(X, p.sx, p.Wi, x0, x1, tx);
                const float wx = (x0 == sx ? 1.0f - tx : 0.f) + (x1 == sx ? tx : 0.f);
                if (wx != 0.f) acc += gimg[((int64_t)Y * p.Wo + X) * p.C] * wy * wx;
            }
        }
        p.din[q] = acc;
    }
}

struct SamplerArgs { const float* img; const float* coords; const float* g; float* out; float* dcoords; float* dimg;
                     int B, Hs, Ws, C, Ht, Wt; };

__device__ __forceinline__ void sampler_taps(const SamplerArgs& p, int b, float cx, float cy, int64_t (&idx)[4], float (&w)[4],
                                             float& wx0, float& wx1, float& wy0, float& wy1) {
    const float x0 = floorf(cx), x1 = x0 + 1.0f, y0 = floorf(cy), y1 = y0 + 1.0f;
    wx0 = x1 - cx; wx1 = cx - x0; wy0 = y1 - cy; wy1 = cy - y0;
    const float xm = (float)(p.Ws - 1), ym = (float)(p.Hs - 1);
    const float x0s = clampf(x0, 0.f, xm), x1s = clampf(x1, 0.f, xm), y0s = clampf(y0, 0.f, ym), y1s = clampf(y1, 0.f, ym);
    const float dim2 = (float)p.Ws, base = (float)b * (float)(p.Ws * p.Hs);
    const float by0 = base + y0s * dim2, by1 = base + y1s * dim2;
    idx[0] = (int64_t)(int)(x0s + by0); idx[1] = (int64_t)(int)(x0s + by1);
    idx[2] = (int64_t)(int)(x1s + by0); idx[3] = (int64_t)(int)(x1s + by1);
    w[0] = wx0 * wy0; w[1] = wx0 * wy1; w[2] = wx1 * wy0; w[3] = wx1 * wy1;
}

__global__ __launch_bounds__(256) void sampler_fwd_kernel(SamplerArgs p) {
    const int64_t total = (int64_t)p.B * p.Ht * p.Wt;
    for (int64_t q = (int64_t)blockIdx.x * 256 + threadIdx.x; q < total; q += (int64_t)gridDim.x * 256) {
        const int b = (int)(q / ((int64_t)p.Ht * p.Wt));
        int64_t idx[4]; float w[4], wx0, wx1, wy0, wy1;
        sampler_taps(p, b, p.coords[q * 2], p.coords[q * 2 + 1], idx, w, wx0, wx1, wy0, wy1);
        for (int c = 0; c < p.C; ++c) {
            float v = w[0] * p.img[idx[0] * p.C + c];
            v += w[1] * p.img[idx[1] * p.C + c];
            v += w[2] * p.img[idx[2] * p.C + c];
            v += w[3] * p.img[idx[3] * p.C + c];
            p.out[q * p.C + c] = v;
        }
    }
}

__global__ __launch_bounds__(256) void sampler_bwd_kernel(SamplerArgs p) {
    const int64_t total = (int64_t)p.B * p.Ht * p.Wt;
    for (int64_t q = (int64_t)blockIdx.x * 256 + threadIdx.x; q < total; q += (int64_t)gridDim.x * 256) {
        const int b = (int)(q / ((int64_t)p.Ht * p.Wt));
        int64_t idx[4]; float w[4], wx0, wx1, wy0, wy1;
        sampler_taps(p, b, p.coords[q * 2], p.coords[q * 2 + 1], idx, w, wx0, wx1, wy0, wy1);
        float gx = 0.f, gy = 0.f;
        for (int c = 0; c < p.C; ++c) {
            const float gv = p.g[q * p.C + c];
            const float i00 = p.img[idx[0] * p.C + c], i01 = p.img[idx[1] * p.C + c], i10 = p.img[idx[2] * p.C + c], i11 = p.img[idx[3] * p.C + c];
            gx += gv * (wy0 * (i10 - i00) + wy1 * (i11 - i01));
            gy += gv * (wx0 * (i01 - i00) + wx1 * (i11 - i10));
            if (p.dimg) {
                mh_atomic_add(p.dimg + idx[0] * p.C + c, gv * w[0]); mh_atomic_add(p.dimg + idx[1] * p.C + c, gv * w[1]);
                mh_atomic_add(p.dimg + idx[2] * p.C + c, gv * w[2]); mh_atomic_add(p.dimg + idx[3] * p.C + c, gv * w[3]);
            }
        }
        if (p.dcoords) { p.dcoords[q * 2] = gx; p.dcoords[q * 2 + 1] = gy; }
    }
}

struct PadArgs { const float* in; float* out; int B, H, W, C, Hp, Wp, pt, pl, out_ld; float div, sub; };

__global__ __launch_bounds__(256) void pad_reflect_kernel(PadArgs p) {
    const int64_t total = (int64_t)p.B * p.Hp * p.Wp;
    for (int64_t q = (int64_t)blockIdx.x * 256 + threadIdx.x; q < total; q += (int64_t)gridDim.x * 256) {
        const int x = (int)(q % p.Wp);
        const int64_t t2 = q / p.Wp;
        const int y = (int)(t2 % p.Hp);
        const int b = (int)(t2 / p.Hp);
        int sy = y - p.pt, sx = x - p.pl;
        sy = sy < 0 ? -sy : (sy >= p.H ? 2 * (p.H - 1) - sy : sy);
        sx = sx < 0 ? -sx : (sx >= p.W ? 2 * (p.W - 1) - sx : sx);
        const float* src = p.in + (((int64_t)b * p.H + sy) * p.W + sx) * p.C;
        float* dst = p.out + q * p.out_ld;
        for (int c = 0; c < p.out_ld; ++c) dst[c] = c < p.C ? (p.div == 1.0f ? src[c] : src[c] / p.div) - p.sub : 0.f;
    }
}

struct LossArgs {
    const float* left; const float* right; const float* disp;
    float* rep; float* drep; float* coef; float* part1; float* part2; float* result; float* ddisp;
    int B, H, W, nblk1, nblk2;
    float grad_scale;
};

__device__ __forceinline__ float block_sum(float v, float* red) {
    v = mh_wave_sum(v);
    const int lane = threadIdx.x & 63, wave = threadIdx.x >> 6;
    __syncthreads();
    if (lane == 0) red[wave] = v;
    __syncthreads();
    return red[0] + red[1] + red[2] + red[3];
}

#define LT_H 16
#define LT_W 32
#define LT_HH (LT_H + 4)
#define LT_HW (LT_W + 4)
#define LT_WH (LT_H + 2)
#define LT_WW (LT_W + 2)
__global__ __launch_bounds__(256) void loss_tile_kernel(LossArgs p, int tiles_x, int tiles_y, int with_grad) {
    __shared__ float red[4];
    __shared__ float s_rep[LT_HH * LT_HW * 3];
    __shared__ float s_y[LT_HH * LT_HW * 3];
    __shared__ float s_drep[LT_H * LT_W * 3];
    __shared__ float s_coef[LT_WH * LT_WW * 9];
    const int tid = threadIdx.x;
    const int tx = blockIdx.x % tiles_x;
    const int t2 = blockIdx.x / tiles_x;
    const int ty = t2 % tiles_y, b = t2 / tiles_y;
    const int y0t = ty * LT_H, x0t = tx * LT_W;
    const float s = 1.0f / 256.0f;
    const float xmax = (float)(p.W - 1);
    float l1 = 0.f;
    {
        constexpr int NI = (LT_HH * LT_HW + 255) / 256;
        const unsigned npx = (unsigned)p.B * (unsigned)p.H * (unsigned)p.W;
        const __amdgpu_buffer_rsrc_t rs_d = mh_make_rsrc(p.disp, npx * 4u);
        const __amdgpu_buffer_rsrc_t rs_l = mh_make_rsrc(p.left, npx * 12u);
        const __amdgpu_buffer_rsrc_t rs_r = mh_make_rsrc(p.right, npx * 12u);
        int qv[NI], rbv[NI];
        bool inb[NI];
        float dv[NI];
#pragma unroll
        for (int u = 0; u < NI; ++u) {
            const int i = tid + u * 256;
            const int ly = i / LT_HW, lx = i - ly * LT_HW;
            const int y = y0t - 2 + ly, x = x0t - 2 + lx;
            inb[u] = i < LT_HH * LT_HW && (unsigned)y < (unsigned)p.H && (unsigned)x < (unsigned)p.W;
            rbv[u] = (b * p.H + y) * p.W;
            qv[u] = rbv[u] + x;
            dv[u] = mh_buf_load1(rs_d, inb[u] ? qv[u] * 4 : MH_OOB);
        }
        float av[NI][3], bv[NI][3], lv[NI][3], w0v[NI], w1v[NI];
#pragma unroll
        for (int u = 0; u < NI; ++u) {
            const int i = tid + u * 256;
            const int ly = i / LT_HW, lx = i - ly * LT_HW;
            const int x = x0t - 2 + lx;
            const float cx = (float)x - dv[u];
            const float xf0 = floorf(cx), xf1 = xf0 + 1.0f;
            w0v[u] = xf1 - cx; w1v[u] = cx - xf0;
            const int i0 = (int)clampf(xf0, 0.f, xmax), i1 = (int)clampf(xf1, 0.f, xmax);
            int o0 = (rbv[u] + i0) * 12, o1 = (rbv[u] + i1) * 12, ol = qv[u] * 12;
            MH_KEEP_VGPR(o0); MH_KEEP_VGPR(o1); MH_KEEP_VGPR(ol);
#pragma unroll
            for (int c = 0; c < 3; ++c) {
                av[u][c] = mh_buf_load1(rs_r, inb[u] ? o0 + 4 * c : MH_OOB);
                bv[u][c] = mh_buf_load1(rs_r, inb[u] ? o1 + 4 * c : MH_OOB);
                lv[u][c] = mh_buf_load1(rs_l, inb[u] ? ol + 4 * c : MH_OOB);
            }
        }
#pragma unroll
        for (int u = 0; u < NI; ++u) {
            const int i = tid + u * 256;
            if (i >= LT_HH * LT_HW) break;
            const int ly = i / LT_HW, lx = i - ly * LT_HW;
            float r0v = 0.f, r1v = 0.f, r2v = 0.f, y0v = 0.f, y1v = 0.f, y2v = 0.f;
            if (inb[u]) {
                const float a0 = av[u][0] * s, a1 = av[u][1] * s, a2 = av[u][2] * s;
                const float b0 = bv[u][0] * s, b1 = bv[u][1] * s, b2 = bv[u][2] * s;
                const float w0 = w0v[u], w1 = w1v[u];
                r0v = w0 * a0 + w1 * b0; r1v = w0 * a1 + w1 * b1; r2v = w0 * a2 + w1 * b2;
                y0v = lv[u][0] * s; y1v = lv[u][1] * s; y2v = lv[u][2] * s;
                const int iy = ly - 2, ix = lx - 2;
                if ((unsigned)iy < (unsigned)LT_H && (unsigned)ix < (unsigned)LT_W) {
                    float* d = s_drep + (iy * LT_W + ix) * 3;
                    d[0] = b0 - a0; d[1] = b1 - a1; d[2] = b2 - a2;
                    l1 += fabsf(r0v - y0v) + fabsf(r1v - y1v) + fabsf(r2v - y2v);
                }
            }
            s_rep[i * 3 + 0] = r0v; s_rep[i * 3 + 1] = r1v; s_rep[i * 3 + 2] = r2v;
            s_y[i * 3 + 0] = y0v; s_y[i * 3 + 1] = y1v; s_y[i * 3 + 2] = y2v;
        }
    }
    __syncthreads();
    const int Hw = p.H - 2, Ww = p.W - 2;
    float ssum = 0.f;
    for (int i = tid; i < LT_WH * LT_WW; i += 256) {
        const int ly = i / LT_WW, lx = i - ly * LT_WW;
        const int wy = y0t - 2 + ly, wx = x0t - 2 + lx;
        float co[9] = {0, 0, 0, 0, 0, 0, 0, 0, 0};
        if ((unsigned)wy < (unsigned)Hw && (unsigned)wx < (unsigned)Ww) {
            const float C1 = 0.01f * 0.01f, C2 = 0.03f * 0.03f;
            float sx[3] = {0, 0, 0}, sy[3] = {0, 0, 0}, sxx[3] = {0, 0, 0}, syy[3] = {0, 0, 0}, sxy[3] = {0, 0, 0};
            for (int dy = 0; dy < 3; ++dy)
                for (int dx = 0; dx < 3; ++dx) {
                    const int h = ((ly + dy) * LT_HW + lx + dx) * 3;
#pragma unroll
                    for (int c = 0; c < 3; ++c) {
                        const float xv = s_rep[h + c], yv = s_y[h + c];
                        sx[c] += xv; sy[c] += yv; sxx[c] += xv * xv; syy[c] += yv * yv; sxy[c] += xv * yv;
                    }
                }
            const bool own = ly >= 2 && lx >= 2 && ly < 2 + LT_H && lx < 2 + LT_W;
#pragma unroll
            for (int c = 0; c < 3; ++c) {
                const float inv9 = 1.0f / 9.0f;
                const float mx = sx[c] * inv9, my = sy[c] * inv9;
                const float vx = sxx[c] * inv9 - mx * mx, vy = syy[c] * inv9 - my * my, vxy = sxy[c] * inv9 - mx * my;
                const float n1 = 2.f * mx * my + C1, n2 = 2.f * vxy + C2;
                const float d1 = mx * mx + my * my + C1, d2 = vx + vy + C2;
                const float S = (n1 * n2) / (d1 * d2);
                const float mraw = (1.0f - S) * 0.5f;
                if (own) ssum += clampf(mraw, 0.f, 1.f);
                const float pass = (mraw >= 0.f && mraw <= 1.f) ? -0.5f * (2.0f / 9.0f) : 0.f;
                const float idd = 1.0f / (d1 * d2);
                const float beta = n1 * idd;
                const float gamma = -S / d2;
                const float alpha = (my * n2 - n1 * my) * idd - S * (mx * d2 - d1 * mx) * idd;
                co[c * 3 + 0] = pass * alpha; co[c * 3 + 1] = pass * beta; co[c * 3 + 2] = pass * gamma;
            }
        }
#pragma unroll
        for (int k = 0; k < 9; ++k) s_coef[i * 9 + k] = co[k];
    }
    const float tot1 = block_sum(l1, red);
    const float tot2 = block_sum(ssum, red);
    if (tid == 0) { p.part1[blockIdx.x] = tot1; p.part2[blockIdx.x] = tot2; }
    if (!with_grad) return;
    const float k_ssim = 0.85f / ((float)p.B * (float)Hw * (float)Ww * 3.0f);
    const float k_l1 = 0.15f / ((float)p.B * (float)p.H * (float)p.W * 3.0f);
    for (int i = tid; i < LT_H * LT_W; i += 256) {
        const int iy = i / LT_W, ix = i - iy * LT_W;
        const int y = y0t + iy, x = x0t + ix;
        if (y >= p.H || x >= p.W) continue;
        float A[3] = {0, 0, 0}, Bc[3] = {0, 0, 0}, Gc[3] = {0, 0, 0};
        for (int dy = 0; dy < 3; ++dy)
            for (int dx = 0; dx < 3; ++dx) {
                const float* cp = s_coef + ((iy + dy) * LT_WW + ix + dx) * 9;
                A[0] += cp[0]; Bc[0] += cp[1]; Gc[0] += cp[2];
                A[1] += cp[3]; Bc[1] += cp[4]; Gc[1] += cp[5];
                A[2] += cp[6]; Bc[2] += cp[7]; Gc[2] += cp[8];
            }
        const int h = ((iy + 2) * LT_HW + ix + 2) * 3;
        float gd = 0.f;
#pragma unroll
        for (int c = 0; c < 3; ++c) {
            const float xv = s_rep[h + c], yv = s_y[h + c];
            const float diff = xv - yv;
            const float sgn = diff > 0.f ? 1.f : (diff < 0.f ? -1.f : 0.f);
            const float grep = k_ssim * (A[c] + Bc[c] * yv + Gc[c] * xv) + k_l1 * sgn;
            gd -= grep * s_drep[i * 3 + c];
        }
        p.ddisp[((int64_t)b * p.H + y) * p.W + x] = gd * p.grad_scale;
    }
}

__global__ __launch_bounds__(256) void loss_final_kernel(LossArgs p) {
    __shared__ double red[256];
    double a = 0.0, b = 0.0;
    for (int i = threadIdx.x; i < p.nblk1; i += 256) a += (double)p.part1[i];
    for (int i = threadIdx.x; i < p.nblk2; i += 256) b += (double)p.part2[i];
    red[threadIdx.x] = a; __syncthreads();
    for (int o = 128; o > 0; o >>= 1) { if ((int)threadIdx.x < o) red[threadIdx.x] += red[threadIdx.x + o]; __syncthreads(); }
    const double l1 = red[0]; __syncthreads();
    red[threadIdx.x] = b; __syncthreads();
    for (int o = 128; o > 0; o >>= 1) { if ((int)threadIdx.x < o) red[threadIdx.x] += red[threadIdx.x + o]; __syncthreads(); }
    if (threadIdx.x == 0) {
        const double n1 = (double)p.B * p.H * p.W * 3.0;
        const double n2 = (double)p.B * (p.H - 2) * (p.W - 2) * 3.0;
        const double ms = red[0] / n2, ml = l1 / n1;
        p.result[0] = (float)(0.85 * ms + 0.15 * ml);
        p.result[1] = (float)ms;
        p.result[2] = (float)ml;
    }
}

struct MetArgs { const float* disp; const float* gt; float* part; float* result; int64_t total; int nblk; float th; };

__global__ __launch_bounds__(256) void metrics_kernel(MetArgs p) {
    __shared__ float red[4];
    const int64_t q = (int64_t)blockIdx.x * 256 + threadIdx.x;
    float e = 0.f, bad = 0.f, v = 0.f;
    if (q < p.total) {
        const float gt = p.gt[q];
        v = (gt == 0.f) ? 0.f : 1.f;
        e = fabsf(p.disp[q] - gt) * v;
        bad = e > p.th ? 1.f : 0.f;
    }
    const float se = block_sum(e, red);
    const float sb = block_sum(bad, red);
    const float sv = block_sum(v, red);
    if (threadIdx.x == 0) { p.part[blockIdx.x * 3 + 0] = se; p.part[blockIdx.x * 3 + 1] = sb; p.part[blockIdx.x * 3 + 2] = sv; }
}
// ... 66 lines not shown
}

struct ProxySArgs { const float* pred; const float* proxy; float* part; const float* result; float* dpred; int B, H, W, Hs, Ws; float sy, sx, fs, weight, gs; };

__device__ __forceinline__ void interp1_exact(int i, float scale, int n, int& lo, int& hi, float& t) {
#if defined(__clang__)
#pragma clang fp contract(off)
#endif
    const float src = (float)i * scale;
    lo = (int)src;
    hi = min(lo + 1, n - 1);
    t = src - (float)lo;
}

__device__ __forceinline__ float proxy_s_diff(const ProxySArgs& p, const float* pred, const float* proxy, int y0, int y1, float ty, int x0, int x1, float tx,
                                              float& v) {
    const float pv = bilerp(pred, p.W, y0, y1, ty, x0, x1, tx, 1.0f, false);
    const float q = bilerp(proxy, p.W, y0, y1, ty, x0, x1, tx, 1.0f, false) / p.fs;
    v = (q <= 0.f || q >= 192.0f) ? 0.f : 1.f;
    return pv - q;
}

__global__ __launch_bounds__(256) void proxy_s_partial_kernel(ProxySArgs p) {
    __shared__ float red[4];
    const int64_t total = (int64_t)p.B * p.Hs * p.Ws;
    const int64_t q = (int64_t)blockIdx.x * 256 + threadIdx.x;
    float e = 0.f, v = 0.f;
    if (q < total) {
        const int x = (int)(q % p.Ws);
        const int64_t t2 = q / p.Ws;
        const int y = (int)(t2 % p.Hs);
        const int64_t off = (t2 / p.Hs) * p.H * p.W;
        int y0, y1, x0, x1; float ty, tx;
        interp1_exact(y, p.sy, p.H, y0, y1, ty);
        interp1_exact(x, p.sx, p.W, x0, x1, tx);
        e = fabsf(proxy_s_diff(p, p.pred + off, p.proxy + off, y0, y1, ty, x0, x1, tx, v)) * v;
    }
    const float se = block_sum(e, red);
    const float sv = block_sum(v, red);
    if (threadIdx.x == 0) { p.part[blockIdx.x * 2 + 0] = se; p.part[blockIdx.x * 2 + 1] = sv; }
}

__global__ __launch_bounds__(256) void proxy_s_grad_kernel(ProxySArgs p) {
    const int64_t total = (int64_t)p.B * p.H * p.W;
    const float isy = 1.0f / p.sy, isx = 1.0f / p.sx;
    const float k = p.gs * p.weight;
    const float nvalid = p.result[1];
    for (int64_t q = (int64_t)blockIdx.x * 256 + threadIdx.x; q < total; q += (int64_t)gridDim.x * 256) {
        const int sx = (int)(q % p.W);
        const int64_t t2 = q / p.W;
        const int sy = (int)(t2 % p.H);
        const int64_t off = (t2 / p.H) * p.H * p.W;
        const int ya = max(0, (int)floorf((float)(sy - 1) * isy) - 1), yb = min(p.Hs - 1, (int)ceilf((float)(sy + 1) * isy) + 1);
        const int xa = max(0, (int)floorf((float)(sx - 1) * isx) - 1), xb = min(p.Ws - 1, (int)ceilf((float)(sx + 1) * isx) + 1);
        float acc = 0.f;
        for (int Y = ya; Y <= yb; ++Y) {
            int y0, y1; float ty;
            interp1_exact(Y, p.sy, p.H, y0, y1, ty);
            const float wy = (y0 == sy ? 1.0f - ty : 0.f) + (y1 == sy ? ty : 0.f);
            if (wy == 0.f) continue;
            for (int X = xa; X <= xb; ++X) {
                int x0, x1; float tx;
                interp1_exact(X, p.sx, p.W, x0, x1, tx);
                const float wx = (x0 == sx ? 1.0f - tx : 0.f) + (x1 == sx ? tx : 0.f);
                if (wx == 0.f) continue;
                float v;
                const float d = proxy_s_diff(p, p.pred + off, p.proxy + off, y0, y1, ty, x0, x1, tx, v);
                const float sgn = d > 0.f ? 1.f : (d < 0.f ? -1.f : 0.f);
                acc += v * sgn * wy * wx;
            }
        }
        p.dpred[q] = k * acc / nvalid;
    }
}

struct KittiArgs { const float* disp; const float* gt; float* part; float* result; int64_t total; int nblk; };

__global__ __launch_bounds__(256) void metrics_kitti_kernel(KittiArgs p) {
    __shared__ float red[4];
    __shared__ double dred[256];
    const int64_t q = (int64_t)blockIdx.x * 256 + threadIdx.x;
    float diff = 0.f, bad = 0.f, v = 0.f;
    if (q < p.total) {
        const float gt = p.gt[q];
        if (gt > 0.f) {
            v = 1.f;
            diff = fabsf(gt - p.disp[q]);
            bad = (diff > 3.0f && diff / gt >= 0.05f) ? 1.f : 0.f;
        }
    }
    dred[threadIdx.x] = (double)diff;
    __syncthreads();
    for (int o = 128; o > 0; o >>= 1) { if ((int)threadIdx.x < o) dred[threadIdx.x] += dred[threadIdx.x + o]; __syncthreads(); }
    const float sb = block_sum(bad, red);
    const float sv = block_sum(v, red);
    if (threadIdx.x == 0) { p.part[blockIdx.x * 3 + 0] = (float)dred[0]; p.part[blockIdx.x * 3 + 1] = sb; p.part[blockIdx.x * 3 + 2] = sv; }
}

__global__ __launch_bounds__(256) void metrics_kitti_final_kernel(KittiArgs p) {
    __shared__ double red[3][256];
    double a = 0, b = 0, c = 0;
    for (int i = threadIdx.x; i < p.nblk; i += 256) { a += p.part[i * 3]; b += p.part[i * 3 + 1]; c += p.part[i * 3 + 2]; }
    red[0][threadIdx.x] = a; red[1][threadIdx.x] = b; red[2][threadIdx.x] = c;
    __syncthreads();
    for (int o = 128; o > 0; o >>= 1) {
        if ((int)threadIdx.x < o) {
            red[0][threadIdx.x] += red[0][threadIdx.x + o];
            red[1][threadIdx.x] += red[1][threadIdx.x + o];
            red[2][threadIdx.x] += red[2][threadIdx.x + o];
        }
        __syncthreads();
    }
    if (threadIdx.x == 0) {
        p.result[0] = (float)(red[0][0] / red[2][0]);
        p.result[1] = (float)(100.0 * (red[1][0] / red[2][0]));
        p.result[2] = (float)red[2][0];
    }
}

__global__ __launch_bounds__(256) void momentum4_kernel(float4* var, float4* acc, const float4* g, int64_t n4, float lr, float mom, float gs) {
    for (int64_t i = (int64_t)blockIdx.x * 256 + threadIdx.x; i < n4; i += (int64_t)gridDim.x * 256) {
        const float4 m = acc[i], gg = g[i];
        float4 v = var[i];
        float4 a;
        a.x = mom * m.x + gs * gg.x; a.y = mom * m.y + gs * gg.y; a.z = mom * m.z + gs * gg.z; a.w = mom * m.w + gs * gg.w;
        acc[i] = a;
        v.x -= lr * a.x; v.y -= lr * a.y; v.z -= lr * a.z; v.w -= lr * a.w;
        var[i] = v;
    }
}
__global__ __launch_bounds__(256) void momentum_kernel(float* var, float* acc, const float* g, int64_t n, float lr, float mom, float gs) {
    for (int64_t i = (int64_t)blockIdx.x * 256 + threadIdx.x; i < n; i += (int64_t)gridDim.x * 256) {
        const float a = mom * acc[i] + gs * g[i];
        acc[i] = a;
        var[i] -= lr * a;
    }
}

__global__ __launch_bounds__(256) void adam_kernel(float* var, float* m, float* v, const float* g, int64_t n, const float* state,
                                                   float lr, float b1, float b2, float eps, float gs) {
    const float lr_t = lr * sqrtf(1.0f - state[1]) / (1.0f - state[0]);
    for (int64_t i = (int64_t)blockIdx.x * 256 + threadIdx.x; i < n; i += (int64_t)gridDim.x * 256) {
        const float gi = gs * g[i];
        const float mi = m[i] + (gi - m[i]) * (1.0f - b1);
        const float vi = v[i] + (gi * gi - v[i]) * (1.0f - b2);
        m[i] = mi; v[i] = vi;
        var[i] -= (mi * lr_t) / (sqrtf(vi) + eps);
    }
}
__global__ void adam_advance_kernel(float* state, float b1, float b2) {
    if (threadIdx.x == 0 && blockIdx.x == 0) { state[0] *= b1; state[1] *= b2; }
}

__global__ __launch_bounds__(256) void copy_channels_kernel(const float* src, int src_ld, float* dst, int dst_ld, int64_t npix,
                                                            int nch, float scale, int accumulate) {
    const int64_t total = npix * nch;
    for (int64_t q = (int64_t)blockIdx.x * 256 + threadIdx.x; q < total; q += (int64_t)gridDim.x * 256) {
        const int c = (int)(q % nch);
        const int64_t pix = q / nch;
        const float v = scale * src[pix * src_ld + c];
        float* d = dst + pix * dst_ld + c;
        *d = accumulate ? *d + v : v;
    }
}

__global__ __launch_bounds__(256) void leaky_bwd_kernel(float* dy, int dy_ld, const float* y, int y_ld, int64_t npix, int nch, float alpha) {
    const int64_t total = npix * nch;
    for (int64_t q = (int64_t)blockIdx.x * 256 + threadIdx.x; q < total; q += (int64_t)gridDim.x * 256) {
        const int c = (int)(q % nch);
        const int64_t pix = q / nch;
        if (!(y[pix * y_ld + c] > 0.f)) dy[pix * dy_ld + c] *= alpha;
    }
}

__global__ __launch_bounds__(256) void bias_grad_kernel(const float* dz, int dz_ld, int64_t npix, int nch, float* db, int nchp, float* ws) {
    __shared__ float red[4][64];
    const int lane = threadIdx.x & 63, w = threadIdx.x >> 6;
    const int ppw = 64 / nchp;
    const int c = blockIdx.y * 64 + (lane & (nchp - 1));
    const int pl = lane / nchp;
    float v = 0.f;
    if (c < nch) {
        const int64_t st = (int64_t)gridDim.x * 4 * ppw;
        int64_t q = ((int64_t)blockIdx.x * 4 + w) * ppw + pl;
        float a[8] = {0.f, 0.f, 0.f, 0.f, 0.f, 0.f, 0.f, 0.f};
        for (; q + 7 * st < npix; q += 8 * st) {
            float t[8];
#pragma unroll
            for (int u = 0; u < 8; ++u) t[u] = dz[(q + u * st) * dz_ld + c];
#pragma unroll
            for (int u = 0; u < 8; ++u) a[u] += t[u];
        }
        for (; q < npix; q += st) a[0] += dz[q * dz_ld + c];
        v = ((a[0] + a[1]) + (a[2] + a[3])) + ((a[4] + a[5]) + (a[6] + a[7]));
    }
    for (int o = nchp; o < 64; o <<= 1) v += __shfl_xor(v, o);
    red[w][lane] = v;
    __syncthreads();
    if (w == 0 && pl == 0 && c < nch) {
        const float t = (red[0][lane] + red[1][lane]) + (red[2][lane] + red[3][lane]);
        if (ws) ws[(int64_t)blockIdx.x * nch + c] = t; else mh_atomic_add(db + c, t);
    }
}

__global__ __launch_bounds__(256) void fill_kernel(float* p, int64_t n, float v) {
    for (int64_t i = (int64_t)blockIdx.x * 256 + threadIdx.x; i < n; i += (int64_t)gridDim.x * 256) p[i] = v;
}

inline int grid_for(int64_t n, int cap = 256 * 16) {
    int64_t b = (n + 255) / 256;
    if (b > cap) b = cap;
    if (b < 1) b = 1;
    return (int)b;
}

}

extern "C" int mh_warp_fwd(const float* img, int32_t img_ld, const float* u, float* out, int32_t out_ld,
                           int32_t B, int32_t H, int32_t W, int32_t C, void* stream) {
    MH_REQUIRE(img && u && out, MH_ERR_ARG, "mh_warp_fwd: null argument");
    MH_REQUIRE(B > 0 && H > 0 && W > 0 && C > 0, MH_ERR_ARG, "mh_warp_fwd: bad dimension");
    MH_REQUIRE(C % 4 == 0 && img_ld % 4 == 0 && out_ld % 4 == 0 && mh_aligned16(img) && mh_aligned16(out), MH_ERR_ALIGN,
               "mh_warp_fwd: C and lds must be multiples of 4, pointers 16-byte aligned");
    WarpArgs a{}; a.img = img; a.u = u; a.out = out; a.img_ld = img_ld; a.out_ld = out_ld;
    a.B = B; a.H = H; a.W = W; a.C = C; a.total = (int64_t)B * H * W * (C / 4);
    hipLaunchKernelGGL(warp_fwd_kernel, dim3(grid_for(a.total)), dim3(256), 0, (hipStream_t)stream, a);
    return mh_check_launch("warp_fwd");
}

extern "C" int mh_warp_bwd(const float* g, int32_t g_ld, const float* img, int32_t img_ld, const float* u,
                           float* dimg, int32_t dimg_ld, float* du, int32_t acc_u,
                           int32_t B, int32_t H, int32_t W, int32_t C, void* stream) {
    MH_REQUIRE(g && img && u && (dimg || du), MH_ERR_ARG, "mh_warp_bwd: null argument");
    MH_REQUIRE(B > 0 && H > 0 && W > 0 && C > 0, MH_ERR_ARG, "mh_warp_bwd: bad dimension");
    MH_REQUIRE(C % 4 == 0 && img_ld % 4 == 0 && g_ld % 4 == 0 && mh_aligned16(img) && mh_aligned16(g), MH_ERR_ALIGN,
               "mh_warp_bwd: C and lds must be multiples of 4, pointers 16-byte aligned");
    WarpArgs a{}; a.g = g; a.img = img; a.u = u; a.dimg = dimg; a.du = du; a.acc_u = acc_u;
    a.g_ld = g_ld; a.img_ld = img_ld; a.dimg_ld = dimg_ld; a.B = B; a.H = H; a.W = W; a.C = C;
    const int C4 = C / 4;
    const int64_t npix = (int64_t)B * H * W;
    hipStream_t s = (hipStream_t)stream;
    if (C4 <= 4) hipLaunchKernelGGL((warp_bwd_kernel<4>), dim3(grid_for(npix * 4)), dim3(256), 0, s, a);
    else if (C4 <= 8) hipLaunchKernelGGL((warp_bwd_kernel<8>), dim3(grid_for(npix * 8)), dim3(256), 0, s, a);
    else hipLaunchKernelGGL((warp_bwd_kernel<16>), dim3(grid_for(npix * 16)), dim3(256), 0, s, a);
    return mh_check_launch("warp_bwd");
}

static int resize_args(ResizeArgs& a, int B, int Hi, int Wi, int Hr, int Wr, int cy, int cx, int Ho, int Wo, float mul, int mode) {
    MH_REQUIRE(B > 0 && Hi > 0 && Wi > 0 && Hr > 0 && Wr > 0 && Ho > 0 && Wo > 0, MH_ERR_ARG, "mh_resize: bad dimension");
    MH_REQUIRE(cy >= 0 && cx >= 0 && cy + Ho <= Hr && cx + Wo <= Wr, MH_ERR_ARG, "mh_resize: crop outside the resized image");
    MH_REQUIRE(mode >= 0 && mode <= 2, MH_ERR_ARG, "mh_resize: mode must be 0,1,2");
    a.B = B; a.Hi = Hi; a.Wi = Wi; a.Hr = Hr; a.Wr = Wr; a.cy = cy; a.cx = cx; a.Ho = Ho; a.Wo = Wo; a.mode = mode;
    a.mul = mul; a.sy = (float)Hi / (float)Hr; a.sx = (float)Wi / (float)Wr;
    return 0;
}

extern "C" int mh_resize_fwd(const float* in, float* out, int32_t B, int32_t Hi, int32_t Wi, int32_t Hr, int32_t Wr,
                             int32_t cy, int32_t cx, int32_t Ho, int32_t Wo, float mul, int32_t mode, void* stream) {
    MH_REQUIRE(in && out, MH_ERR_ARG, "mh_resize_fwd: null argument");
    ResizeArgs a{}; a.in = in; a.out = out;
    if (int e = resize_args(a, B, Hi, Wi, Hr, Wr, cy, cx, Ho, Wo, mul, mode)) return e;
    hipLaunchKernelGGL(resize_fwd_kernel, dim3(grid_for((int64_t)B * Ho * Wo)), dim3(256), 0, (hipStream_t)stream, a);
    return mh_check_launch("resize_fwd");
}

__global__ __launch_bounds__(256) void u8_to_f32_kernel(const unsigned char* __restrict__ in, float* __restrict__ out, int64_t n) {
    const int64_t q4 = ((int64_t)blockIdx.x * 256 + threadIdx.x) * 4;
    if (q4 + 4 <= n && ((((uintptr_t)in) | ((uintptr_t)out)) & 3u) == 0 && (((uintptr_t)out) & 15u) == 0) {
        const unsigned v = *reinterpret_cast<const unsigned*>(in + q4);
        *reinterpret_cast<float4*>(out + q4) = make_float4((float)(v & 0xffu), (float)((v >> 8) & 0xffu), (float)((v >> 16) & 0xffu), (float)(v >> 24));
    } else {
        for (int64_t q = q4; q < q4 + 4 && q < n; ++q) out[q] = (float)in[q];
    }
}

struct FetchArgs { const mh_input_table* tab; float* dst[MH_FETCH_MAX]; int64_t n[MH_FETCH_MAX]; int64_t q0[MH_FETCH_MAX + 1]; };
__global__ __launch_bounds__(256) void fetch_inputs_kernel(FetchArgs a) {
    const int64_t q = (int64_t)blockIdx.x * 256 + threadIdx.x;
    int k = 0;
#pragma unroll
    for (int j = 1; j < MH_FETCH_MAX; ++j) k += q >= a.q0[j] ? 1 : 0;
    if (q >= a.q0[MH_FETCH_MAX]) return;
    const void* src = a.tab->src[k];
    float* dst = a.dst[k];
    if (!src || src == (const void*)dst) return;
    const int64_t e0 = (q - a.q0[k]) * 4, n = a.n[k];
    if (a.tab->u8[k]) {
        const unsigned char* in = (const unsigned char*)src;
        if (e0 + 4 <= n && ((((uintptr_t)in) & 3u) | (((uintptr_t)dst) & 15u)) == 0) {
            const unsigned v = *reinterpret_cast<const unsigned*>(in + e0);
            *reinterpret_cast<float4*>(dst + e0) = make_float4((float)(v & 0xffu), (float)((v >> 8) & 0xffu), (float)((v >> 16) & 0xffu), (float)(v >> 24));
        } else {
            for (int64_t e = e0; e < e0 + 4 && e < n; ++e) dst[e] = (float)in[e];
        }
    } else {
        const float* in = (const float*)src;
        if (e0 + 4 <= n && ((((uintptr_t)in) | ((uintptr_t)dst)) & 15u) == 0) *reinterpret_cast<float4*>(dst + e0) = *reinterpret_cast<const float4*>(in + e0);
        else for (int64_t e = e0; e < e0 + 4 && e < n; ++e) dst[e] = in[e];
    }
}

extern "C" int mh_fetch_inputs(const mh_input_table* table, float* const* dst, const int64_t* n, int32_t count, void* stream) {
    MH_REQUIRE(table && dst && n && count >= 1 && count <= MH_FETCH_MAX, MH_ERR_ARG, "mh_fetch_inputs: bad argument");
    FetchArgs a{};
    a.tab = table;
    int64_t q = 0;
    for (int k = 0; k < MH_FETCH_MAX; ++k) {
        a.q0[k] = q;
        if (k < count) {
            MH_REQUIRE(dst[k] && n[k] >= 0, MH_ERR_ARG, "mh_fetch_inputs: null destination / negative count");
            a.dst[k] = dst[k]; a.n[k] = n[k];
            q += (n[k] + 3) / 4;
        }
    }
    a.q0[MH_FETCH_MAX] = q;
    if (q == 0) return 0;
// ... 711 lines not shown
    for (int k = 0; k < 4; ++k) {
        const int i = (int)threadIdx.x + 256 * k, x = x0 + (i & (SGM_ST_W - 1)), y = y0 + i / SGM_ST_W;
        if (x >= a.W || y >= a.H) continue;
        const int g = frame + y * a.W + x, r = root[k];
        a.parent[g] = r < 0 ? -1 : frame + (y0 + r / SGM_ST_W) * a.W + x0 + (r & (SGM_ST_W - 1));
        a.cnt[g] = r == i ? s_cnt[i] : 0;
    }
}

__device__ __forceinline__ int sgm_speckle_find_atomic(int* parent, int x) {
    for (;;) { const int p = atomicMin(parent + x, x); if (p == x) return x; x = p; }
}

__device__ __forceinline__ int sgm_speckle_local_root(const SpeckleArgs& a, int x) { return a.cnt[x] > 0 ? x : a.parent[x]; }

__global__ __launch_bounds__(256) void sgm_speckle_merge_kernel(SpeckleArgs a) {
    int e = (int)blockIdx.x * 256 + (int)threadIdx.x;
    const int frame = (int)blockIdx.y * a.H * a.W;
    int p, q, back;
    if (e < a.nvb * a.H) { const int bx = e / a.H, y = e - bx * a.H; q = frame + y * a.W + (bx + 1) * SGM_ST_W; p = q - 1; back = y ? a.W : 0; }
    else {
        e -= a.nvb * a.H;
        if (e >= a.nhb * a.W) return;
        const int by = e / a.W, x = e - by * a.W;
        q = frame + (by + 1) * SGM_ST_H * a.W + x; p = q - a.W; back = x ? 1 : 0;
    }
    if (!sgm_speckle_joined(a.in[p], a.in[q], a.max_diff)) return;
    const int pp = p - back, pq = q - back;
    p = sgm_speckle_local_root(a, p); q = sgm_speckle_local_root(a, q);
    if (back && sgm_speckle_joined(a.in[pp], a.in[pq], a.max_diff) && sgm_speckle_local_root(a, pp) == p && sgm_speckle_local_root(a, pq) == q) return;
    for (;;) {
        p = sgm_speckle_find_atomic(a.parent, p); q = sgm_speckle_find_atomic(a.parent, q);
        if (p == q) return;
        if (p < q) { const int t = p; p = q; q = t; }
        const int old = atomicMin(a.parent + p, q);
        if (old == p) return;
        p = old;
    }
}

__device__ __forceinline__ int sgm_speckle_find(const int* __restrict__ parent, int x) {
    for (;;) { const int p = parent[x]; if (p == x) return x; x = p; }
}

__global__ __launch_bounds__(256) void sgm_speckle_count_kernel(SpeckleArgs a) {
    const int p = (int)blockIdx.x * 256 + (int)threadIdx.x;
    if (p >= a.npix) return;
    const int c = a.cnt[p];
    if (c <= 0) return;
    const int r = sgm_speckle_find(a.parent, p);
    if (r == p) return;
    atomicAdd(a.cnt + r, c);
    a.cnt[p] = -(r + 1);
}

__global__ __launch_bounds__(256) void sgm_speckle_apply_kernel(SpeckleArgs a) {
    const int p = (int)blockIdx.x * 256 + (int)threadIdx.x;
    if (p >= a.npix) return;
    const float v = a.in[p];
    float o = 0.f;
    if (v > 0.f) {
        int n = a.cnt[p];
        if (n == 0) n = a.cnt[a.parent[p]];
        if (n < 0) n = a.cnt[-n - 1];
        if (n > a.max_size) o = v;
    }
    a.out[p] = o;
}

extern "C" int64_t mh_sgm_speckle_ws_bytes(int32_t B, int32_t H, int32_t W) {
    if (B <= 0 || H <= 0 || W <= 0) return 0;
    return 2 * sgm_align16((int64_t)B * H * W * 4);
}

extern "C" int mh_sgm_speckle(const float* labels, float* out, void* ws, int32_t B, int32_t H, int32_t W, int32_t max_size, float max_diff, void* stream) {
    MH_REQUIRE(labels && out && ws, MH_ERR_ARG, "mh_sgm_speckle: null argument");
    MH_REQUIRE(B > 0 && H > 0 && W > 0, MH_ERR_ARG, "mh_sgm_speckle: bad dimension");
    MH_REQUIRE(max_size >= 0, MH_ERR_ARG, "mh_sgm_speckle: max_size must not be negative");
    MH_REQUIRE(max_diff >= 0.f && max_diff < __builtin_inff(), MH_ERR_ARG, "mh_sgm_speckle: max_diff must be finite and not negative");
    MH_REQUIRE(mh_aligned16(ws), MH_ERR_ALIGN, "mh_sgm_speckle: ws must be 16-byte aligned");
    MH_REQUIRE((int64_t)B * H * W < (1ll << 31) - 256 && B < 65536 && H < 65536 * SGM_ST_H, MH_ERR_UNSUPPORTED, "mh_sgm_speckle: too many pixels or frames");
    const int64_t npix = (int64_t)B * H * W;
    SpeckleArgs a{};
    a.in = labels; a.out = out;
    a.parent = (int*)ws; a.cnt = (int*)((char*)ws + sgm_align16(npix * 4));
    a.B = B; a.H = H; a.W = W; a.npix = (int)npix; a.max_size = max_size; a.max_diff = max_diff;
    a.nvb = (W - 1) / SGM_ST_W; a.nhb = (H - 1) / SGM_ST_H;
    hipStream_t s = (hipStream_t)stream;
    hipLaunchKernelGGL(sgm_speckle_tile_kernel, dim3((unsigned)mh_cdiv(W, SGM_ST_W), (unsigned)mh_cdiv(H, SGM_ST_H), (unsigned)B), dim3(256), 0, s, a);
    if (int e = mh_check_launch("sgm_speckle_tile")) return e;
    const int64_t pairs = (int64_t)a.nvb * H + (int64_t)a.nhb * W;
    if (pairs > 0) {
        hipLaunchKernelGGL(sgm_speckle_merge_kernel, dim3((unsigned)mh_cdiv(pairs, 256), (unsigned)B), dim3(256), 0, s, a);
        if (int e = mh_check_launch("sgm_speckle_merge")) return e;
        hipLaunchKernelGGL(sgm_speckle_count_kernel, dim3((unsigned)mh_cdiv(npix, 256)), dim3(256), 0, s, a);
        if (int e = mh_check_launch("sgm_speckle_count")) return e;
    }
    hipLaunchKernelGGL(sgm_speckle_apply_kernel, dim3((unsigned)mh_cdiv(npix, 256)), dim3(256), 0, s, a);
    mh_note_kernel("sgm_speckle_tile_kernel grid %d x %d x %d, %d launches", mh_cdiv(W, SGM_ST_W), mh_cdiv(H, SGM_ST_H), B, pairs > 0 ? 4 : 2);
    return mh_check_launch("sgm_speckle_apply");
}

extern "C" int mh_resize_image_fwd(const float* in, float* out, int32_t B, int32_t Hi, int32_t Wi, int32_t C, int32_t Ho, int32_t Wo,
                                   void* stream) {
    MH_REQUIRE(in && out && B > 0 && Hi > 0 && Wi > 0 && C > 0 && Ho > 0 && Wo > 0, MH_ERR_ARG, "mh_resize_image_fwd: bad argument");
    ResizeImgArgs a{in, nullptr, out, nullptr, B, Hi, Wi, C, Ho, Wo, (float)Hi / (float)Ho, (float)Wi / (float)Wo};
    hipLaunchKernelGGL(resize_image_fwd_kernel, dim3(grid_for((int64_t)B * Ho * Wo * C)), dim3(256), 0, (hipStream_t)stream, a);
    return mh_check_launch("resize_image_fwd");
}

extern "C" int mh_resize_image_bwd(const float* g, float* din, int32_t B, int32_t Hi, int32_t Wi, int32_t C, int32_t Ho, int32_t Wo,
                                   void* stream) {
    MH_REQUIRE(g && din && B > 0 && Hi > 0 && Wi > 0 && C > 0 && Ho > 0 && Wo > 0, MH_ERR_ARG, "mh_resize_image_bwd: bad argument");
    ResizeImgArgs a{nullptr, g, nullptr, din, B, Hi, Wi, C, Ho, Wo, (float)Hi / (float)Ho, (float)Wi / (float)Wo};
    hipLaunchKernelGGL(resize_image_bwd_kernel, dim3(grid_for((int64_t)B * Hi * Wi * C)), dim3(256), 0, (hipStream_t)stream, a);
    return mh_check_launch("resize_image_bwd");
}

extern "C" int mh_bilinear_sampler_fwd(const float* imgs, const float* coords, float* out, int32_t B, int32_t Hs, int32_t Ws, int32_t C,
                                       int32_t Ht, int32_t Wt, void* stream) {
    MH_REQUIRE(imgs && coords && out && B > 0 && Hs > 0 && Ws > 0 && C > 0 && Ht > 0 && Wt > 0, MH_ERR_ARG, "mh_bilinear_sampler_fwd: bad argument");
    MH_REQUIRE((int64_t)B * Hs * Ws < (1 << 24), MH_ERR_UNSUPPORTED,
               "mh_bilinear_sampler_fwd: B*Hs*Ws must stay below 2^24 (the reference computes the gather index in float32)");
    SamplerArgs a{imgs, coords, nullptr, out, nullptr, nullptr, B, Hs, Ws, C, Ht, Wt};
    hipLaunchKernelGGL(sampler_fwd_kernel, dim3(grid_for((int64_t)B * Ht * Wt)), dim3(256), 0, (hipStream_t)stream, a);
    return mh_check_launch("bilinear_sampler_fwd");
}

extern "C" int mh_bilinear_sampler_bwd(const float* g, const float* imgs, const float* coords, float* dcoords, float* dimgs, int32_t B,
                                       int32_t Hs, int32_t Ws, int32_t C, int32_t Ht, int32_t Wt, void* stream) {
    MH_REQUIRE(g && imgs && coords && (dcoords || dimgs) && B > 0 && Hs > 0 && Ws > 0 && C > 0 && Ht > 0 && Wt > 0, MH_ERR_ARG,
               "mh_bilinear_sampler_bwd: bad argument");
    MH_REQUIRE((int64_t)B * Hs * Ws < (1 << 24), MH_ERR_UNSUPPORTED, "mh_bilinear_sampler_bwd: B*Hs*Ws must stay below 2^24");
    SamplerArgs a{imgs, coords, g, nullptr, dcoords, dimgs, B, Hs, Ws, C, Ht, Wt};
    hipLaunchKernelGGL(sampler_bwd_kernel, dim3(grid_for((int64_t)B * Ht * Wt)), dim3(256), 0, (hipStream_t)stream, a);
    return mh_check_launch("bilinear_sampler_bwd");
}

extern "C" int mh_resize_bwd(const float* g, const float* in, float* din, int32_t accumulate, int32_t B, int32_t Hi, int32_t Wi,
                             int32_t Hr, int32_t Wr, int32_t cy, int32_t cx, int32_t Ho, int32_t Wo, float mul, int32_t mode,
                             void* stream) {
    MH_REQUIRE(g && in && din, MH_ERR_ARG, "mh_resize_bwd: null argument");
    ResizeArgs a{}; a.in = in; a.g = g; a.din = din; a.accumulate = accumulate;
    if (int e = resize_args(a, B, Hi, Wi, Hr, Wr, cy, cx, Ho, Wo, mul, mode)) return e;
    const int64_t npx = (int64_t)B * Hi * Wi;
    hipStream_t s = (hipStream_t)stream;
    if (a.sy <= 1.0f / 12.0f) hipLaunchKernelGGL((resize_bwd_kernel<64>), dim3(grid_for(npx * 64)), dim3(256), 0, s, a);
    else if (a.sy <= 1.0f / 6.0f) hipLaunchKernelGGL((resize_bwd_kernel<16>), dim3(grid_for(npx * 16)), dim3(256), 0, s, a);
    else if (a.sy <= 1.0f / 3.0f) hipLaunchKernelGGL((resize_bwd_kernel<4>), dim3(grid_for(npx * 4)), dim3(256), 0, s, a);
    else hipLaunchKernelGGL((resize_bwd_kernel<1>), dim3(grid_for(npx)), dim3(256), 0, s, a);
    return mh_check_launch("resize_bwd");
}

extern "C" int mh_head_bwd(const mh_head_bwd_desc* d, const float* src0, const float* src1, float* dV, void* dV_shadow, const float* w,
                           float* dx, const float* mask_ref, void* dx_shadow, void* stream) {
    MH_REQUIRE(d && dV && w && dx && (src0 || src1), MH_ERR_ARG, "mh_head_bwd: null argument");
    MH_REQUIRE(d->kind == 0 || d->kind == 1, MH_ERR_ARG, "mh_head_bwd: kind must be 0 (resize gradient of a finer level's du) or 1 (addends)");
    MH_REQUIRE(d->B > 0 && d->H > 0 && d->W > 0 && d->N >= 4 && d->N <= 64 && d->N % 4 == 0, MH_ERR_ARG, "mh_head_bwd: bad dimension (N = 4 .. 64, multiple of 4)");
    MH_REQUIRE(d->dx_ld % 4 == 0 && d->dx_ld >= d->N && mh_aligned16(dx) && mh_aligned16(w) && (!mask_ref || (d->mask_ld % 4 == 0 && mh_aligned16(mask_ref))) &&
               (!dx_shadow || mh_aligned16(dx_shadow)), MH_ERR_ALIGN, "mh_head_bwd: dx / mask / w must be 16-byte aligned with lds that are multiples of 4");
    HeadBwdArgs a{};
    if (d->kind == 0) {
        MH_REQUIRE(src0, MH_ERR_ARG, "mh_head_bwd: kind 0 needs the finer level's coordinate gradient");
        a.rz.g = src0;
        if (int e = resize_args(a.rz, d->B, d->H, d->W, d->Hr, d->Wr, d->cy, d->cx, d->Ho, d->Wo, d->mul, 0)) return e;
    } else {
        a.rz.B = d->B; a.rz.Hi = d->H; a.rz.Wi = d->W;
        a.a1 = src0; a.a2 = src1; a.a1_ld = d->src0_ld; a.a2_ld = d->src1_ld;
        MH_REQUIRE((!src0 || d->src0_ld >= 1) && (!src1 || d->src1_ld >= 1), MH_ERR_ARG, "mh_head_bwd: addend pixel strides must be >= 1");
    }
    a.dV = dV; a.dV_sh = (unsigned short*)dV_shadow; a.dV_sh_ld = 32;
    a.w = w; a.dx = dx; a.mask_ref = mask_ref; a.dx_sh = (unsigned short*)dx_shadow;
    a.N = d->N; a.dx_ld = d->dx_ld; a.mask_ld = d->mask_ld; a.dx_sh_ld = (d->N + 31) / 32 * 32; a.acc_dx = d->accumulate_dx; a.kind = d->kind;
    a.mask_alpha = d->mask_alpha;
    a.tiles_x = (d->W + HB_TW - 1) / HB_TW; a.tiles_y = (d->H + HB_TH - 1) / HB_TH;
    const int64_t grid = (int64_t)d->B * a.tiles_x * a.tiles_y;
    MH_REQUIRE(grid < (1ll << 31), MH_ERR_ARG, "mh_head_bwd: too many tiles");
    hipLaunchKernelGGL(head_bwd_kernel, dim3((unsigned)grid), dim3(256), 0, (hipStream_t)stream, a);
    mh_note_kernel("head_bwd_kernel kind %d N=%d", d->kind, d->N);
    return mh_check_launch("head_bwd");
}

extern "C" int mh_pad_reflect(const float* in, float* out, int32_t B, int32_t H, int32_t W, int32_t C,
                              int32_t Hp, int32_t Wp, int32_t pad_t, int32_t pad_l, int32_t out_ld,
                              float div, float sub, void* stream) {
    MH_REQUIRE(in && out, MH_ERR_ARG, "mh_pad_reflect: null argument");
    MH_REQUIRE(B > 0 && H > 1 && W > 1 && C > 0 && Hp >= H && Wp >= W && out_ld >= C, MH_ERR_ARG, "mh_pad_reflect: bad dimension");
    MH_REQUIRE(pad_t >= 0 && pad_l >= 0 && pad_t < H && pad_l < W && Hp - H - pad_t < H && Wp - W - pad_l < W &&
               Hp - H - pad_t >= 0 && Wp - W - pad_l >= 0, MH_ERR_ARG, "mh_pad_reflect: REFLECT pad must be smaller than the image");
    MH_REQUIRE(div != 0.f, MH_ERR_ARG, "mh_pad_reflect: div must be non-zero");
    PadArgs a{in, out, B, H, W, C, Hp, Wp, pad_t, pad_l, out_ld, div, sub};
    hipLaunchKernelGGL(pad_reflect_kernel, dim3(grid_for((int64_t)B * Hp * Wp)), dim3(256), 0, (hipStream_t)stream, a);
    return mh_check_launch("pad_reflect");
}

static inline int64_t nblk(int64_t n) { return (n + 255) / 256; }

static inline int64_t loss_tiles(int32_t B, int32_t H, int32_t W) { return (int64_t)B * mh_cdiv(W, LT_W) * mh_cdiv(H, LT_H); }

extern "C" int64_t mh_loss_ws_floats(int32_t B, int32_t H, int32_t W) {
    const int64_t n = (int64_t)B * H * W, nw = (int64_t)B * (H - 2) * (W - 2);
    return 8 * n + 12 * nw + 2 * loss_tiles(B, H, W);
}

extern "C" int mh_reprojection_loss(const float* left, const float* right, const float* disp, float* ws, float* result,
                                    float* ddisp, float grad_scale, int32_t B, int32_t H, int32_t W, void* stream) {
    return mh_reprojection_loss_phase(left, right, disp, ws, result, ddisp, grad_scale, B, H, W, 0, stream);
}

extern "C" int mh_reprojection_loss_phase(const float* left, const float* right, const float* disp, float* ws, float* result,
                                          float* ddisp, float grad_scale, int32_t B, int32_t H, int32_t W, int32_t phase, void* stream) {
    MH_REQUIRE(phase >= 0 && phase <= 2, MH_ERR_ARG, "mh_reprojection_loss_phase: phase must be 0 (all), 1 (maps + gradient) or 2 (final reduction)");
    MH_REQUIRE(left && right && disp && ws && result, MH_ERR_ARG, "mh_reprojection_loss: null argument");
    MH_REQUIRE(B > 0 && H >= 3 && W >= 3, MH_ERR_ARG, "mh_reprojection_loss: image must be at least 3x3");
    MH_REQUIRE(mh_aligned16(ws), MH_ERR_ALIGN, "mh_reprojection_loss: workspace must be 16-byte aligned");
    const int64_t n = (int64_t)B * H * W, nw = (int64_t)B * (H - 2) * (W - 2);
    MH_REQUIRE(n * 12 < (1ll << 31) - 64, MH_ERR_ARG, "mh_reprojection_loss: too many pixels (32-bit byte offsets into the frames)");
    LossArgs a{};
    a.left = left; a.right = right; a.disp = disp; a.result = result; a.ddisp = ddisp; a.grad_scale = grad_scale;
    a.B = B; a.H = H; a.W = W;
    const int tiles_x = mh_cdiv(W, LT_W), tiles_y = mh_cdiv(H, LT_H);
    const int64_t ntiles = loss_tiles(B, H, W);
    MH_REQUIRE(ntiles < (1ll << 31), MH_ERR_ARG, "mh_reprojection_loss: too many tiles");
    a.rep = ws; a.drep = ws + 4 * n; a.coef = ws + 8 * n;
    a.part1 = ws + 8 * n + 12 * nw; a.nblk1 = (int)ntiles;
    a.part2 = a.part1 + ntiles; a.nblk2 = (int)ntiles;
    hipStream_t s = (hipStream_t)stream;
    if (phase != 2) hipLaunchKernelGGL(loss_tile_kernel, dim3((unsigned)ntiles), dim3(256), 0, s, a, tiles_x, tiles_y, ddisp ? 1 : 0);
    if (phase != 1) hipLaunchKernelGGL(loss_final_kernel, dim3(1), dim3(256), 0, s, a);
    return mh_check_launch("reprojection_loss");
}

extern "C" int64_t mh_metrics_ws_floats(int32_t B, int32_t H, int32_t W) { return 3 * nblk((int64_t)B * H * W) + 16; }

extern "C" int mh_metrics(const float* disp, const float* gt, float* ws, float* result, float pixel_th,
                          int32_t B, int32_t H, int32_t W, void* stream) {
    MH_REQUIRE(disp && gt && ws && result, MH_ERR_ARG, "mh_metrics: null argument");
    MH_REQUIRE(B > 0 && H > 0 && W > 0, MH_ERR_ARG, "mh_metrics: bad dimension");
    MetArgs a{disp, gt, ws, result, (int64_t)B * H * W, (int)nblk((int64_t)B * H * W), pixel_th};
    hipStream_t s = (hipStream_t)stream;
    hipLaunchKernelGGL(metrics_kernel, dim3(a.nblk), dim3(256), 0, s, a);
    hipLaunchKernelGGL(metrics_final_kernel, dim3(1), dim3(256), 0, s, a);
    return mh_check_launch("metrics");
}

extern "C" int64_t mh_proxy_ws_floats(int32_t B, int32_t H, int32_t W) { return 2 * nblk((int64_t)B * H * W); }

static int masked_l1(const char* what, const float* pred, const float* target, float* ws, float* result, float* dpred, float weight,
                     float grad_scale, float hi, int zero_only, int32_t B, int32_t H, int32_t W, void* stream) {
    MH_REQUIRE(pred && target && ws && result, MH_ERR_ARG, "%s: null argument", what);
    MH_REQUIRE(B > 0 && H > 0 && W > 0, MH_ERR_ARG, "%s: bad dimension", what);
    ProxyArgs a{pred, target, ws, result, dpred, (int64_t)B * H * W, (int)nblk((int64_t)B * H * W), weight, grad_scale, hi, zero_only};
    hipStream_t s = (hipStream_t)stream;
    hipLaunchKernelGGL(proxy_partial_kernel, dim3(a.nblk), dim3(256), 0, s, a);
    hipLaunchKernelGGL(proxy_final_kernel, dim3(1), dim3(256), 0, s, a);
    if (dpred) hipLaunchKernelGGL(proxy_grad_kernel, dim3(a.nblk), dim3(256), 0, s, a);
    return mh_check_launch(what);
}

extern "C" int mh_proxy_loss(const float* pred, const float* proxy, float* ws, float* result, float* dpred, float weight,
                             float grad_scale, int32_t B, int32_t H, int32_t W, void* stream) {
    return masked_l1("mh_proxy_loss", pred, proxy, ws, result, dpred, weight, grad_scale, 192.0f, 0, B, H, W, stream);
}

extern "C" int mh_supervised_loss(const float* pred, const float* target, float* ws, float* result, float* dpred, float weight,
                                  float grad_scale, float max_disp, int32_t B, int32_t H, int32_t W, void* stream) {
    MH_REQUIRE(max_disp > 0.f, MH_ERR_ARG, "mh_supervised_loss: max_disp must be positive");
    return masked_l1("mh_supervised_loss", pred, target, ws, result, dpred, weight, grad_scale, max_disp, 1, B, H, W, stream);
}

extern "C" int64_t mh_proxy_scaled_ws_floats(int32_t B, int32_t H, int32_t W, int32_t scale) {
    if (scale < 1) scale = 1;
    return 2 * nblk((int64_t)B * (H / scale) * (W / scale));
}

extern "C" int mh_proxy_loss_scaled(const float* pred, const float* proxy, float* ws, float* result, float* dpred, float weight,
                                    float grad_scale, int32_t scale, int32_t B, int32_t H, int32_t W, void* stream) {
    MH_REQUIRE(pred && proxy && ws && result, MH_ERR_ARG, "mh_proxy_loss_scaled: null argument");
    MH_REQUIRE(B > 0 && H > 0 && W > 0 && H < 65536 && W < 65536, MH_ERR_ARG, "mh_proxy_loss_scaled: bad dimension");
    MH_REQUIRE(scale >= 1 && scale <= H && scale <= W, MH_ERR_ARG, "mh_proxy_loss_scaled: scale must lie in 1 .. min(H, W)");
    const int Hs = H / scale, Ws = W / scale;
    const int64_t nout = (int64_t)B * Hs * Ws;
    MH_REQUIRE((int64_t)B * H * W < (1ll << 31), MH_ERR_ARG, "mh_proxy_loss_scaled: too many pixels");
    ProxySArgs a{pred, proxy, ws, result, dpred, B, H, W, Hs, Ws, (float)H / (float)Hs, (float)W / (float)Ws, (float)scale, weight, grad_scale};
    ProxyArgs f{};
    f.part = ws; f.result = result; f.nblk = (int)nblk(nout); f.weight = weight;
    hipStream_t s = (hipStream_t)stream;
    hipLaunchKernelGGL(proxy_s_partial_kernel, dim3(f.nblk), dim3(256), 0, s, a);
    hipLaunchKernelGGL(proxy_final_kernel, dim3(1), dim3(256), 0, s, f);
    if (dpred) hipLaunchKernelGGL(proxy_s_grad_kernel, dim3(grid_for((int64_t)B * H * W)), dim3(256), 0, s, a);
    return mh_check_launch("mh_proxy_loss_scaled");
}

extern "C" int64_t mh_metrics_kitti_ws_floats(int32_t B, int32_t H, int32_t W) { return 3 * nblk((int64_t)B * H * W) + 16; }

extern "C" int mh_metrics_kitti(const float* disp, const float* gt, float* ws, float* result, int32_t B, int32_t H, int32_t W, void* stream) {
    MH_REQUIRE(disp && gt && ws && result, MH_ERR_ARG, "mh_metrics_kitti: null argument");
    MH_REQUIRE(B > 0 && H > 0 && W > 0, MH_ERR_ARG, "mh_metrics_kitti: bad dimension");
    MH_REQUIRE((int64_t)B * H * W < (1ll << 31), MH_ERR_ARG, "mh_metrics_kitti: too many pixels");
    KittiArgs a{disp, gt, ws, result, (int64_t)B * H * W, (int)nblk((int64_t)B * H * W)};
    hipStream_t s = (hipStream_t)stream;
    hipLaunchKernelGGL(metrics_kitti_kernel, dim3(a.nblk), dim3(256), 0, s, a);
    hipLaunchKernelGGL(metrics_kitti_final_kernel, dim3(1), dim3(256), 0, s, a);
    return mh_check_launch("mh_metrics_kitti");
}

extern "C" int mh_adam(float* var, float* m, float* v, const float* grad, int64_t n, const float* state, float lr, float beta1,
                       float beta2, float eps, float grad_scale, void* stream) {
    MH_REQUIRE(var && m && v && grad && state && n > 0, MH_ERR_ARG, "mh_adam: bad argument");
    MH_REQUIRE(beta1 >= 0.f && beta1 < 1.f && beta2 >= 0.f && beta2 < 1.f, MH_ERR_ARG, "mh_adam: beta out of [0, 1)");
    hipLaunchKernelGGL(adam_kernel, dim3(grid_for(n)), dim3(256), 0, (hipStream_t)stream, var, m, v, grad, n, state, lr, beta1, beta2, eps, grad_scale);
    return mh_check_launch("adam");
}

extern "C" int mh_adam_advance(float* state, float beta1, float beta2, void* stream) {
    MH_REQUIRE(state, MH_ERR_ARG, "mh_adam_advance: null state");
    hipLaunchKernelGGL(adam_advance_kernel, dim3(1), dim3(64), 0, (hipStream_t)stream, state, beta1, beta2);
    return mh_check_launch("adam_advance");
}

extern "C" int mh_momentum(float* var, float* accum, const float* grad, int64_t n, float lr, float momentum,
                           float grad_scale, void* stream) {
    MH_REQUIRE(var && accum && grad && n > 0, MH_ERR_ARG, "mh_momentum: bad argument");
    const int64_t n4 = n >> 2;
    if (n4 > 0 && (((uintptr_t)var | (uintptr_t)accum | (uintptr_t)grad) & 15u) == 0)
        hipLaunchKernelGGL(momentum4_kernel, dim3(grid_for(n4)), dim3(256), 0, (hipStream_t)stream, (float4*)var, (float4*)accum, (const float4*)grad, n4, lr, momentum,
                           grad_scale);
    else if (n4 > 0) { hipLaunchKernelGGL(momentum_kernel, dim3(grid_for(n)), dim3(256), 0, (hipStream_t)stream, var, accum, grad, n, lr, momentum, grad_scale); return mh_check_launch("momentum"); }
    if (n & 3)
        hipLaunchKernelGGL(momentum_kernel, dim3(1), dim3(256), 0, (hipStream_t)stream, var + 4 * n4, accum + 4 * n4, grad + 4 * n4, n & 3, lr, momentum, grad_scale);
    return mh_check_launch("momentum");
}

extern "C" int mh_copy_channels(const float* src, int32_t src_ld, float* dst, int32_t dst_ld, int64_t npix,
                                int32_t nch, float scale, int32_t accumulate, void* stream) {
    MH_REQUIRE(src && dst && npix > 0 && nch > 0 && src_ld >= nch && dst_ld >= nch, MH_ERR_ARG, "mh_copy_channels: bad argument");
    hipLaunchKernelGGL(copy_channels_kernel, dim3(grid_for(npix * nch)), dim3(256), 0, (hipStream_t)stream,
                       src, src_ld, dst, dst_ld, npix, nch, scale, accumulate);
    return mh_check_launch("copy_channels");
}

extern "C" int mh_leaky_bwd(float* dy, int32_t dy_ld, const float* y, int32_t y_ld, int64_t npix, int32_t nch,
                            float alpha, void* stream) {
    MH_REQUIRE(dy && y && npix > 0 && nch > 0, MH_ERR_ARG, "mh_leaky_bwd: bad argument");
    hipLaunchKernelGGL(leaky_bwd_kernel, dim3(grid_for(npix * nch)), dim3(256), 0, (hipStream_t)stream, dy, dy_ld, y, y_ld, npix, nch, alpha);
    return mh_check_launch("leaky_bwd");
}

extern "C" int mh_bias_grad(const float* dz, int32_t dz_ld, int64_t npix, int32_t nch, float* db, void* stream) {
    MH_REQUIRE(dz && db && npix > 0 && nch > 0 && dz_ld >= nch, MH_ERR_ARG, "mh_bias_grad: bad argument");
    int nchp = 1;
    while (nchp < nch && nchp < 64) nchp <<= 1;
    const int64_t rows = (npix + (64 / nchp) - 1) / (64 / nchp);
    int gx = (int)((rows + 4 * 8 - 1) / (4 * 8));
    if (gx > 1024) gx = 1024;
    if (gx < 1) gx = 1;
    hipLaunchKernelGGL(bias_grad_kernel, dim3(gx, (nch + 63) / 64), dim3(256), 0, (hipStream_t)stream, dz, dz_ld, npix, nch, db, nchp, (float*)nullptr);
    return mh_check_launch("bias_grad");
}

extern "C" int mh_bias_grad_blocks(int64_t npix, int32_t nch) {
    if (npix <= 0 || nch <= 0) return 0;
    int nchp = 1;
    while (nchp < nch && nchp < 64) nchp <<= 1;
    const int64_t rows = (npix + (64 / nchp) - 1) / (64 / nchp);
    int64_t gx = (rows + 4 * 8 - 1) / (4 * 8);
    return (int)(gx > 1024 ? 1024 : (gx < 1 ? 1 : gx));
}

extern "C" int mh_bias_grad_partial(const float* dz, int32_t dz_ld, int64_t npix, int32_t nch, float* ws, int32_t nblocks, void* stream) {
    MH_REQUIRE(dz && ws && npix > 0 && nch > 0 && dz_ld >= nch, MH_ERR_ARG, "mh_bias_grad_partial: bad argument");
    MH_REQUIRE(nblocks == mh_bias_grad_blocks(npix, nch), MH_ERR_ARG, "mh_bias_grad_partial: nblocks %d must be mh_bias_grad_blocks(npix, nch) = %d (the workspace was sized for it)",
               nblocks, mh_bias_grad_blocks(npix, nch));
    int nchp = 1;
    while (nchp < nch && nchp < 64) nchp <<= 1;
    hipLaunchKernelGGL(bias_grad_kernel, dim3(nblocks, (nch + 63) / 64), dim3(256), 0, (hipStream_t)stream, dz, dz_ld, npix, nch, (float*)nullptr, nchp, ws);
    return mh_check_launch("bias_grad_partial");
}

__global__ __launch_bounds__(256) void det_flush_kernel(float* dst, long long* acc, int64_t n) {
    for (int64_t i = (int64_t)blockIdx.x * 256 + threadIdx.x; i < n; i += (int64_t)gridDim.x * 256) {
        const long long a = acc[i];
        if (a) { dst[i] += (float)((double)a * (1.0 / 281474976710656.0)); acc[i] = 0; }
    }
}
extern "C" int mh_det_flush(float* dst, void* acc, int64_t n, void* stream) {
    MH_REQUIRE(dst && acc && n >= 0, MH_ERR_ARG, "mh_det_flush: null buffer");
    if (n == 0) return 0;
    const int64_t blocks = (n + 255) / 256;
    hipLaunchKernelGGL(det_flush_kernel, dim3((unsigned)(blocks < 4096 ? blocks : 4096)), dim3(256), 0, (hipStream_t)stream, dst, (long long*)acc, n);
    return mh_check_launch("det_flush");
}

__global__ void stamp_kernel(long long* slot) { *slot = wall_clock64(); }
extern "C" int mh_stamp(void* slot, void* stream) {
    MH_REQUIRE(slot && (((uintptr_t)slot) & 7u) == 0, MH_ERR_ARG, "mh_stamp: 8-byte aligned slot");
    hipLaunchKernelGGL(stamp_kernel, dim3(1), dim3(1), 0, (hipStream_t)stream, (long long*)slot);
    return mh_check_launch("stamp");
}
extern "C" int64_t mh_stamp_rate_khz(void) {
    int dev = 0, khz = 0;
    if (hipGetDevice(&dev) != hipSuccess) return 0;
    if (hipDeviceGetAttribute(&khz, hipDeviceAttributeWallClockRate, dev) != hipSuccess) return 0;
    return khz;
}

extern "C" int mh_fill(float* p, int64_t n, float v, void* stream) {
    MH_REQUIRE(p && n > 0, MH_ERR_ARG, "mh_fill: bad argument");
    hipLaunchKernelGGL(fill_kernel, dim3(grid_for(n)), dim3(256), 0, (hipStream_t)stream, p, n, v);
    return mh_check_launch("fill");
}

extern "C" int mh_det_sync_ops(const void* t) { return mh_det_upload(*reinterpret_cast<const mh_det_table*>(t)); }
extern "C" int mh_det_ovf_ops(void) { return mh_det_overflow_take(); }
```

### real-time-self-adaptive-deep-stereo_amd/madnet_hip/_ffi.py

```python
import ctypes as C
import os

_HERE = os.path.dirname(os.path.abspath(__file__))
LIB_PATH = os.environ.get("MADNET_HIP_LIB") or os.path.join(_HERE, "libmadnet_hip.so")


class ConvDesc(C.Structure):
    _fields_ = [(n, C.c_int32) for n in
                ("B", "Hi", "Wi", "Ho", "Wo", "K", "N", "kh", "kw", "stride", "dil", "pad_t", "pad_l",
                 "mode", "w_trans", "in_ld", "out_ld", "mask_ld", "accumulate")] + \
               [("alpha", C.c_float), ("mask_alpha", C.c_float), ("mask_c0", C.c_int32), ("mask_c1", C.c_int32), ("precision", C.c_int32)]


class Op(C.Structure):
    _fields_ = [("kind", C.c_int32), ("i", C.c_int32 * 27), ("f", C.c_float * 4),
                ("p", C.c_void_p * 12), ("n", C.c_int64)]


(OP_CONV, OP_WGRAD, OP_CORR_FWD, OP_CORR_BWD, OP_WARP_FWD, OP_WARP_BWD, OP_RESIZE_FWD, OP_RESIZE_BWD,
 OP_PAD_REFLECT, OP_LOSS, OP_METRICS, OP_MOMENTUM, OP_COPY_CH, OP_LEAKY_BWD, OP_FILL, OP_BIAS_GRAD,
 OP_WGRAD_PARTIAL, OP_WGRAD_REDUCE, OP_PROXY_LOSS, OP_SUPERVISED_LOSS, OP_ADAM, OP_ADAM_ADVANCE, OP_RESIZE_IMAGE, OP_LEVEL_FRONT, OP_RESERVED_25, OP_PACK_W, OP_CORR_WARP_BWD,
 OP_SHADOW_CAST, OP_WGRAD_STREAM, OP_HEAD_BWD, OP_HEAD_FWD, OP_CONV_PLANES, OP_PLANE_SPLIT, OP_STAMP, OP_CONV_PLANES_BWD, OP_DET_FLUSH, OP_CONV_IMAGE, OP_ALLREDUCE, OP_FETCH_INPUTS,
 OP_PROXY_LOSS_SCALED, OP_METRICS_KITTI) = range(1, 42)


COMM_ID_BYTES = 128
ALLREDUCE_MAX_BUFS = 8
FETCH_MAX = 4


class InputTable(C.Structure):
    _fields_ = [("src", C.c_void_p * FETCH_MAX), ("u8", C.c_int32 * FETCH_MAX)]
OP_JOIN = 0x100
OP_NODEFER = 0x200
MAX_LANES = 5


class WgradSeg(C.Structure):
    _fields_ = [("ws", C.c_void_p), ("dst", C.c_void_p), ("size", C.c_int32), ("splits", C.c_int32),
                ("blk0", C.c_int32), ("accumulate", C.c_int32)]

class PackSeg(C.Structure):
    _fields_ = [("src", C.c_void_p), ("dst", C.c_void_p), ("taps", C.c_int32), ("K", C.c_int32), ("N", C.c_int32),
                ("planes", C.c_int32), ("blk0", C.c_int32), ("trans", C.c_int32), ("kc16", C.c_int32), ("reserved", C.c_int32)]


class WgradItem(C.Structure):
    _fields_ = [("d", ConvDesc), ("inp", C.c_void_p), ("dout", C.c_void_p), ("ws", C.c_void_p), ("db", C.c_void_p),
                ("dout_ld", C.c_int32), ("splits", C.c_int32), ("group_max_m", C.c_int32), ("reserved", C.c_int32)]

class ShadowSeg(C.Structure):
    _fields_ = [("src", C.c_void_p), ("dst", C.c_void_p), ("npix", C.c_int64), ("C", C.c_int32), ("src_ld", C.c_int32),
                ("dst_ld", C.c_int32), ("blk0", C.c_int32)]


class PlaneSeg(C.Structure):
    _fields_ = [("src", C.c_void_p), ("hi", C.c_void_p), ("lo", C.c_void_p), ("npix", C.c_int64), ("C", C.c_int32), ("src_ld", C.c_int32),
                ("dst_ld", C.c_int32), ("blk0", C.c_int32), ("src2", C.c_void_p), ("C2", C.c_int32), ("src2_ld", C.c_int32)]


class FrameSeg(C.Structure):
    _fields_ = [("left", C.c_void_p), ("right", C.c_void_p), ("gt", C.c_void_p)] + \
               [(n, C.c_int32) for n in ("Hs", "Ws", "r0", "c0", "gt_kind", "active")] + [("delta", C.c_float), ("contrast", C.c_float), ("hue", C.c_float)]


class PlanRef(C.Structure):
    _fields_ = [("ops", C.c_void_p), ("nops", C.c_int32), ("reserved", C.c_int32)]


class HeadBwdDesc(C.Structure):
    _fields_ = [(n, C.c_int32) for n in ("kind", "B", "H", "W", "N", "Hr", "Wr", "cy", "cx", "Ho", "Wo")] + [("mul", C.c_float)] + \
               [(n, C.c_int32) for n in ("src0_ld", "src1_ld", "dx_ld", "mask_ld", "accumulate_dx")] + [("mask_alpha", C.c_float)]


class WgsLayer(C.Structure):
    _fields_ = [("x", C.c_void_p), ("dz", C.c_void_p), ("ws", C.c_void_p), ("db", C.c_void_p)] + \
               [(n, C.c_int32) for n in ("B", "H", "W", "K", "N", "dil", "x_ld", "dz_ld", "ktiles", "ntiles", "splits", "blk0", "stride", "reserved")]


_P = C.c_void_p
_I = C.c_int32
_F = C.c_float
_L = C.c_int64

SIGNATURES = {
    "mh_last_error": (C.c_char_p, []),
    "mh_last_kernel": (C.c_char_p, []),
    "mh_abi_version": (_I, []),
    "mh_planes_kc16": (_I, [_I]),
    "mh_crc32c": (C.c_uint32, [C.c_char_p, _L, C.c_uint32]),
    "mh_device_count": (_I, []),
    "mh_init": (_I, []),
    "mh_tune_conv_tile": (_I, [_I, _I]),
    "mh_tune_conv_thin": (_I, [_I]),
    "mh_tune_conv_patch": (_I, [_I]),
    "mh_tune_wgrad_wgs": (_I, [_I]),
    "mh_tune_corr": (_I, [_I]),
    "mh_tune_corr_row": (_I, [_I]),
    "mh_conv2d": (_I, [C.POINTER(ConvDesc), _P, _P, _P, _P, _P, _P]),
    "mh_conv2d_wgrad": (_I, [C.POINTER(ConvDesc), _P, _P, _I, _P, _P, _P]),
    "mh_conv2d_wgrad_partial": (_I, [C.POINTER(ConvDesc), _P, _P, _I, _P, C.POINTER(C.c_int32), _P, _P]),
    "mh_corr_warp_bwd": (_I, [_P, _I, _I, _P, _I, _P, _I, _P, _I, _P, _P, _I, _I, _P, _I, _P, _I, _I, _I, _I, _I, _I, _I, _P]),
    "mh_conv2d_wb": (_I, [C.POINTER(ConvDesc), _P, _P, _P, _P, _P, _P, _P]),
    "mh_conv2d_sh": (_I, [C.POINTER(ConvDesc), _P, _P, _P, _P, _P, _P, _P, _P]),
    "mh_pack_weights": (_I, [_P, _I, _I, _P]),
    "mh_pack_bytes": (_L, [_I, _I, _I, _I]),
    "mh_pack32_bytes": (_L, [_I, _I, _I]),
    "mh_conv2d_planes_ok": (_I, [C.POINTER(ConvDesc)]),
    "mh_conv2d_planes": (_I, [C.POINTER(ConvDesc), _P, _P, _I, _P, _P, _P, _P, _P, _I, _P]),
    "mh_plane_split": (_I, [_P, _I, _I, _P]),
    "mh_conv2d_planes_bwd_ok": (_I, [C.POINTER(ConvDesc)]),
    "mh_conv2d_planes_bwd": (_I, [C.POINTER(ConvDesc), _P, _I, _P, _P, _I, _P, _P, _I, _P]),
    "mh_tune_conv_planes": (_I, [_I]),
    "mh_tune_conv_bank": (_I, [_I]),
    "mh_tune_wgrad_image": (_I, [_I]),
    "mh_tune_conv_bank_tile": (_I, [_I]),
    "mh_tune_conv_bank_small": (_I, [_I]),
    "mh_tune_conv_rows": (_I, [_I]),
    "mh_tune_wgrad_target_pct": (_I, [_I]),
    "mh_tune_conv_x3_igemm": (_I, [_I]),
    "mh_conv2d_wgrad_partial_group": (_I, [C.POINTER(WgradItem), _I, _P]),
    "mh_wgrad_reduce": (_I, [_P, _I, _I, _P]),
    "mh_shadow_cast": (_I, [_P, _I, _I, _P]),
    "mh_plans_prepare": (_I, [_I]),
    "mh_plans_run": (_I, [C.POINTER(PlanRef), _I, _P]),
    "mh_conv2d_sh2": (_I, [C.POINTER(ConvDesc), _P, _P, _P, _P, _P, _P, _P, _P, _P]),
    "mh_conv2d_sh3": (_I, [C.POINTER(ConvDesc), _P, _P, _P, _P, _P, _P, _P, _P, _P, _I, _P]),
    "mh_conv2d_takes_shadows": (_I, [C.POINTER(ConvDesc), _P, _P, _P, _P, _P]),
    "mh_conv2d_sh4": (_I, [C.POINTER(ConvDesc), _P, _P, _P, _P, _P, _P, _P, _P, _P]),
    "mh_level_front_fwd_planes": (_I, [_P, _I, _I, _F, _P, _I, _P, _I, _P, _I, _I, _P, _I, _P, _I, _I, _I, _I, _I, _I, _P, _P, _I, _P]),
    "mh_level_front_head_fwd": (_I, [_P, _I, _I, _P, _P, _P, _I, _I, _F, _P, _I, _P, _I, _P, _I, _I, _P, _I, _P, _I, _I, _I, _I, _I, _I, _P, _P, _I, _P]),
    "mh_level_front_head_ok": (_I, [_I, _I, _I, _I, _I, _I, _I]),
    "mh_conv_image_fwd": (_I, [_P, _I, _I, _I, _I, _I, _I, _I, _I, _F, _F, _P, _P, _I, _I, _I, _I, _F, _P, _I, _P, _I, _P]),
    "mh_conv_image_ok": (_I, [_I, _I, _I, _I, _I]),
    "mh_conv2d_head": (_I, [C.POINTER(ConvDesc), _P, _P, _P, _P, _P, _I, _P, _I, _P]),
    "mh_head_bwd": (_I, [C.POINTER(HeadBwdDesc), _P, _P, _P, _P, _P, _P, _P, _P, _P]),
    "mh_wgrad_stream_plan": (_I, [C.POINTER(WgsLayer), _I, _I, _I, C.POINTER(C.c_int32)]),
    "mh_wgrad_stream": (_I, [_P, _I, _I, _I, _I, _P]),
    "mh_tune_wgrad_stream": (_I, [_I]),
    "mh_proxy_ws_floats": (_L, [_I, _I, _I]),
    "mh_proxy_loss": (_I, [_P, _P, _P, _P, _P, _F, _F, _I, _I, _I, _P]),
    "mh_proxy_scaled_ws_floats": (_L, [_I, _I, _I, _I]),
    "mh_proxy_loss_scaled": (_I, [_P, _P, _P, _P, _P, _F, _F, _I, _I, _I, _I, _P]),
    "mh_supervised_loss": (_I, [_P, _P, _P, _P, _P, _F, _F, _F, _I, _I, _I, _P]),
    "mh_adam": (_I, [_P, _P, _P, _P, _L, _P, _F, _F, _F, _F, _F, _P]),
    "mh_adam_advance": (_I, [_P, _F, _F, _P]),
    "mh_corr_fwd": (_I, [_P, _I, _P, _I, _P, _P, _I, _I, _I, _I, _I, _I, _I, _I, _I, _I, _P]),
    "mh_corr_fwd_prec": (_I, [_P, _I, _P, _I, _P, _P, _I, _I, _I, _I, _I, _I, _I, _I, _I, _I, _I, _P]),
    "mh_level_front_fwd": (_I, [_P, _I, _I, _F, _P, _I, _P, _I, _P, _I, _I, _P, _I, _P, _I, _I, _I, _I, _I, _I, _P]),
    "mh_corr_bwd": (_I, [_P, _I, _I, _P, _I, _P, _I, _P, _I, _I, _P, _I, _I, _P, _I, _I, _I, _I, _I, _I, _I, _I, _P]),
    "mh_corr_bwd_prec": (_I, [_P, _I, _I, _P, _I, _P, _I, _P, _I, _I, _P, _I, _I, _P, _I, _I, _I, _I, _I, _I, _I, _I, _I, _P]),
    "mh_shift_corr": (_I, [_P, _P, _I, _I, _I, _I, _I, _P, _P]),
    "mh_shift_corr_grad": (_I, [_P, _P, _P, _I, _I, _I, _I, _I, _P, _P, _P]),
    "mh_warp_fwd": (_I, [_P, _I, _P, _P, _I, _I, _I, _I, _I, _P]),
    "mh_warp_bwd": (_I, [_P, _I, _P, _I, _P, _P, _I, _P, _I, _I, _I, _I, _I, _P]),
    "mh_resize_fwd": (_I, [_P, _P, _I, _I, _I, _I, _I, _I, _I, _I, _I, _F, _I, _P]),
    "mh_resize_bwd": (_I, [_P, _P, _P, _I, _I, _I, _I, _I, _I, _I, _I, _I, _I, _F, _I, _P]),
    "mh_resize_image_fwd": (_I, [_P, _P, _I, _I, _I, _I, _I, _I, _P]),
    "mh_resize_image_bwd": (_I, [_P, _P, _I, _I, _I, _I, _I, _I, _P]),
    "mh_bilinear_sampler_fwd": (_I, [_P, _P, _P, _I, _I, _I, _I, _I, _I, _P]),
    "mh_bilinear_sampler_bwd": (_I, [_P, _P, _P, _P, _P, _I, _I, _I, _I, _I, _I, _P]),
    "mh_u8_to_f32": (_I, [_P, _P, _L, _P]),
    "mh_fetch_inputs": (_I, [_P, C.POINTER(C.c_void_p), C.POINTER(C.c_int64), _I, _P]),
    "mh_host_device_pointer": (_I, [_P, C.POINTER(C.c_void_p)]),
    "mh_frame_prepare_ws_floats": (_L, [_I, _I, _I]),
    "mh_frame_prepare": (_I, [_P, _I, _I, _I, _P, _P, _P, _P, _P]),
    "mh_sgm_ws_bytes": (_L, [_I, _I, _I, _I]),
    "mh_sgm_proxy": (_I, [_P, _P, _I, _P, _P, _I, _I, _I, _I, _I, _I, _I, _I, _P]),
    "mh_sgm_ws_bytes_ex": (_L, [_I, _I, _I, _I, _I, _I]),
    "mh_sgm_proxy_ex": (_I, [_P, _P, _I, _P, _P, _I, _I, _I, _I, _I, _I, _I, _I, _I, _I, _P]),
    "mh_sgm_ws_bytes_scaled": (_L, [_I, _I, _I, _I, _I, _I, _I]),
    "mh_sgm_proxy_scaled": (_I, [_P, _P, _I, _P, _P, _I, _I, _I, _I, _I, _I, _I, _I, _I, _I, _I, _P]),
    "mh_sgm_speckle_ws_bytes": (_L, [_I, _I, _I]),
    "mh_sgm_speckle": (_I, [_P, _P, _P, _I, _I, _I, _I, _F, _P]),
    "mh_pad_reflect": (_I, [_P, _P, _I, _I, _I, _I, _I, _I, _I, _I, _I, _F, _F, _P]),
    "mh_loss_ws_floats": (_L, [_I, _I, _I]),
    "mh_reprojection_loss": (_I, [_P, _P, _P, _P, _P, _P, _F, _I, _I, _I, _P]),
    "mh_reprojection_loss_phase": (_I, [_P, _P, _P, _P, _P, _P, _F, _I, _I, _I, _I, _P]),
    "mh_metrics_ws_floats": (_L, [_I, _I, _I]),
    "mh_metrics": (_I, [_P, _P, _P, _P, _F, _I, _I, _I, _P]),
    "mh_metrics_kitti_ws_floats": (_L, [_I, _I, _I]),
    "mh_metrics_kitti": (_I, [_P, _P, _P, _P, _I, _I, _I, _P]),
    "mh_momentum": (_I, [_P, _P, _P, _L, _F, _F, _F, _P]),
    "mh_copy_channels": (_I, [_P, _I, _P, _I, _L, _I, _F, _I, _P]),
    "mh_leaky_bwd": (_I, [_P, _I, _P, _I, _L, _I, _F, _P]),
    "mh_fill": (_I, [_P, _L, _F, _P]),
    "mh_stamp": (_I, [_P, _P]),
    "mh_deterministic_add": (_I, [_P, C.c_int64, _P]),
    "mh_deterministic_remove": (_I, [_P]),
    "mh_deterministic_ranges": (_I, []),
    "mh_deterministic_overflow": (_I, []),
    "mh_det_flush": (_I, [_P, _P, C.c_int64, _P]),
    "mh_stamp_rate_khz": (_L, []),
    "mh_bias_grad": (_I, [_P, _I, _L, _I, _P, _P]),
    "mh_bias_grad_blocks": (_I, [_L, _I]),
    "mh_comm_available": (_I, []),
    "mh_comm_unique_id": (_I, [_P]),
    "mh_comm_init": (_I, [_P, _I, _I, C.POINTER(C.c_void_p)]),
    "mh_comm_destroy": (_I, [_P]),
    "mh_comm_info": (_I, [_P, C.POINTER(C.c_int32), C.POINTER(C.c_int32), C.POINTER(C.c_int32)]),
    "mh_allreduce_sum": (_I, [C.POINTER(C.c_void_p), C.POINTER(C.c_int64), _I, _P, _P]),
    "mh_bias_grad_partial": (_I, [_P, _I, _L, _I, _P, _I, _P]),
    "mh_plan_run": (_I, [C.POINTER(Op), _I, _P]),
    "mh_graph_begin": (_I, [_P]),
    "mh_graph_end": (_I, [_P, C.POINTER(_P)]),
    "mh_graph_launch": (_I, [_P, _P]),
    "mh_graph_destroy": (_I, [_P]),
    "mh_event_create": (_I, [C.POINTER(_P)]),
    "mh_event_record": (_I, [_P, _P]),
    "mh_event_elapsed_ms": (_I, [_P, _P, C.POINTER(_F)]),
    "mh_event_destroy": (_I, [_P]),
    "mh_stream_sync": (_I, [_P]),
}
_NO_STATUS = {"mh_comm_available", "mh_deterministic_overflow", "mh_bias_grad_blocks", "mh_tune_conv_bank_small", "mh_conv_image_ok", "mh_level_front_head_ok", "mh_deterministic_ranges", "mh_planes_kc16", "mh_conv2d_planes_bwd_ok", "mh_stamp_rate_khz", "mh_pack32_bytes", "mh_conv2d_planes_ok", "mh_tune_conv_planes", "mh_tune_wgrad_target_pct", "mh_tune_wgrad_image", "mh_conv2d_takes_shadows", "mh_tune_conv_bank_tile", "mh_tune_conv_rows", "mh_last_error", "mh_last_kernel", "mh_tune_conv_bank", "mh_pack_bytes", "mh_abi_version", "mh_tune_conv_patch", "mh_crc32c", "mh_device_count", "mh_loss_ws_floats", "mh_metrics_ws_floats", "mh_proxy_ws_floats", "mh_proxy_scaled_ws_floats", "mh_metrics_kitti_ws_floats", "mh_frame_prepare_ws_floats", "mh_sgm_ws_bytes", "mh_sgm_ws_bytes_ex", "mh_sgm_ws_bytes_scaled", "mh_sgm_speckle_ws_bytes"}


class MadnetHipError(RuntimeError):
    pass


class Lib(object):

    def __init__(self, path=LIB_PATH):
        if not os.path.exists(path):
            raise MadnetHipError(
                "HIP extension not built: %s is missing (run `python -c 'import __graft_entry__ as g; g.build()'` "
                "or `make -C real-time-self-adaptive-deep-stereo_amd/csrc`). There is no CPU fallback." % path)
        self.path = path
        self._dll = C.CDLL(path)
        for name, (res, args) in SIGNATURES.items():
            fn = getattr(self._dll, name)
            fn.restype = res
            fn.argtypes = args
            setattr(self, "_raw_" + name, fn)
            if name in _NO_STATUS:
                setattr(self, name[3:], fn)
            else:
                setattr(self, name[3:], self._checked(name, fn))
        self._inited = set()

    def ensure_init(self, device_index=None):
        if device_index not in self._inited:
            self.init()
            self._inited.add(device_index)

    def _checked(self, name, fn):
        def call(*a):
            rc = fn(*a)
            if rc != 0:
                msg = self._dll.mh_last_error()
                raise MadnetHipError("%s failed (%d): %s" % (name, rc, msg.decode() if msg else "?"))
            return 0
        call.__name__ = name
        return call


_lib = None


def lib():
    global _lib
    if _lib is None:
        l = Lib(LIB_PATH)
        n = l.device_count()
        if n <= 0:
            raise MadnetHipError("libmadnet_hip.so loaded but no HIP device is visible (mh_device_count=%d); "
                                 "the MI355X path has no CPU fallback" % n)
        l.ensure_init()
        _lib = l
    return _lib
```

Baseline: 745.0 pairs/s.

## Fuse adjacent plan ops: resize into loss, corr-bwd with leaky-bwd, head-bwd with copy

Adds a peephole fuser to the plan runner that merges adjacent op pairs into single kernels. It folds the disparity resize into the reprojection loss tile kernel, applies the leaky-ReLU backward mask in the corr_bwd_direct epilogue, and optionally merges head backward with a channel copy. Each fusion is guarded by address-overlap and shape checks, and a tune mask controls it; resize+loss and corr+leaky are on by default. The aim is fewer launches and fewer intermediate round trips through global memory. The cost is extra branching in the kernels and more complex plan execution.

```diff
diff --git a/include/madnet_hip_tune.h b/include/madnet_hip_tune.h
--- a/include/madnet_hip_tune.h
+++ b/include/madnet_hip_tune.h
@@ -22,6 +22,8 @@
 
 int mh_tune_conv_planes(int mode);
 
+int mh_tune_plan_fuse(int mask);
+
 #ifdef __cplusplus
 }
 #endif
diff --git a/real-time-self-adaptive-deep-stereo_amd/csrc/corr.hip b/real-time-self-adaptive-deep-stereo_amd/csrc/corr.hip
--- a/real-time-self-adaptive-deep-stereo_amd/csrc/corr.hip
+++ b/real-time-self-adaptive-deep-stereo_amd/csrc/corr.hip
@@ -394,6 +394,7 @@
     int acc_l, acc_r, acc_u;
     int B, H, W, C, md, stride, D, copy_left;
     int64_t total;
+    int leaky; float leaky_alpha;
 };
 
 __global__ __launch_bounds__(256) void corr_bwd_kernel(CorrBwdArgs p) {
@@ -471,6 +472,8 @@
     const float4 gl = mh_buf_load4(rs_g, (live && p.copy_left) ? (pix * p.g_ld + c4 * 4) * 4 : MH_OOB);
     const float4 ol = mh_buf_load4(rs_dl, (live && p.acc_l) ? (pix * p.dl_ld + c4 * 4) * 4 : MH_OOB);
     const float4 orr = mh_buf_load4(rs_dr, (live && p.acc_r) ? (pix * p.dr_ld + c4 * 4) * 4 : MH_OOB);
+    const float4 ml = mh_buf_load4(rs_l, (live && p.leaky) ? (pix * p.l_ld + c4 * 4) * 4 : MH_OOB);
+    const float4 mr = mh_buf_load4(rs_r, (live && p.leaky) ? (pix * p.r_ld + c4 * 4) * 4 : MH_OOB);
     float4 a = make_float4(0.f, 0.f, 0.f, 0.f), r = make_float4(0.f, 0.f, 0.f, 0.f);
 #pragma unroll
     for (int j = 0; j < DT; ++j) {
@@ -482,6 +485,10 @@
     if (p.copy_left) { a.x += gl.x; a.y += gl.y; a.z += gl.z; a.w += gl.w; }
     if (p.acc_l) { a.x += ol.x; a.y += ol.y; a.z += ol.z; a.w += ol.w; }
     if (p.acc_r) { r.x += orr.x; r.y += orr.y; r.z += orr.z; r.w += orr.w; }
+    if (p.leaky) {
+        if (!(ml.x > 0.f)) a.x *= p.leaky_alpha; if (!(ml.y > 0.f)) a.y *= p.leaky_alpha; if (!(ml.z > 0.f)) a.z *= p.leaky_alpha; if (!(ml.w > 0.f)) a.w *= p.leaky_alpha;
+        if (!(mr.x > 0.f)) r.x *= p.leaky_alpha; if (!(mr.y > 0.f)) r.y *= p.leaky_alpha; if (!(mr.z > 0.f)) r.z *= p.leaky_alpha; if (!(mr.w > 0.f)) r.w *= p.leaky_alpha;
+    }
     if (!live) return;
     *reinterpret_cast<float4*>(p.dL + (int64_t)pix * p.dl_ld + c4 * 4) = a;
     *reinterpret_cast<float4*>(p.dR + (int64_t)pix * p.dr_ld + c4 * 4) = r;
@@ -1643,11 +1650,39 @@
     return mh_corr_bwd_prec(g, g_ld, coff, L, l_ld, R, r_ld, dL, dl_ld, acc_l, dR, dr_ld, acc_r, du, acc_u, B, H, W, C, max_disp, stride, copy_left, 0, stream);
 }
 
+static bool corr_bwd_direct_ok(int32_t g_ld, int32_t l_ld, int32_t r_ld, int32_t dl_ld, int32_t dr_ld, int32_t B, int32_t H, int32_t W, int32_t C, int32_t max_disp,
+                               int32_t stride) {
+    static_assert(MAXD_SMALL >= 5, "the large-D kernels must leave D <= 5 alone");
+    const int64_t npix = (int64_t)B * H * W;
+    const int64_t ldm = std::max(std::max(std::max(g_ld, l_ld), std::max(r_ld, dl_ld)), dr_ld);
+    return g_corr_direct && 2 * max_disp / stride + 1 <= 5 && npix * ldm * 4 < (1ll << 31) - 64 && npix * (C / 4) < (1ll << 31) - 256;
+}
+static int corr_bwd_impl(const float* g, int32_t g_ld, int32_t coff, const float* L, int32_t l_ld, const float* R, int32_t r_ld, float* dL, int32_t dl_ld, int32_t acc_l,
+                         float* dR, int32_t dr_ld, int32_t acc_r, float* du, int32_t acc_u, int32_t B, int32_t H, int32_t W, int32_t C, int32_t max_disp, int32_t stride,
+                         int32_t copy_left, int32_t precision, int32_t leaky, float leaky_alpha, void* stream);
+
 extern "C" int mh_corr_bwd_prec(const float* g, int32_t g_ld, int32_t coff, const float* L, int32_t l_ld,
                                 const float* R, int32_t r_ld, float* dL, int32_t dl_ld, int32_t acc_l,
                                 float* dR, int32_t dr_ld, int32_t acc_r, float* du, int32_t acc_u,
                                 int32_t B, int32_t H, int32_t W, int32_t C, int32_t max_disp, int32_t stride,
                                 int32_t copy_left, int32_t precision, void* stream) {
+    return corr_bwd_impl(g, g_ld, coff, L, l_ld, R, r_ld, dL, dl_ld, acc_l, dR, dr_ld, acc_r, du, acc_u, B, H, W, C, max_disp, stride, copy_left, precision, 0, 1.0f, stream);
+}
+
+extern "C" int mh_fuse_corr_bwd_leaky_ok(int32_t g_ld, int32_t l_ld, int32_t r_ld, int32_t dl_ld, int32_t dr_ld, int32_t B, int32_t H, int32_t W, int32_t C, int32_t max_disp,
+                                         int32_t stride) {
+    return B > 0 && H > 0 && W > 0 && C > 0 && C % 4 == 0 && max_disp >= 0 && stride >= 1 && corr_bwd_direct_ok(g_ld, l_ld, r_ld, dl_ld, dr_ld, B, H, W, C, max_disp, stride) ? 1 : 0;
+}
+extern "C" int mh_fuse_corr_bwd_leaky(const float* g, int32_t g_ld, int32_t coff, const float* L, int32_t l_ld, const float* R, int32_t r_ld, float* dL, int32_t dl_ld,
+                                      float* dR, int32_t dr_ld, float* du, int32_t acc_u, int32_t B, int32_t H, int32_t W, int32_t C, int32_t max_disp, int32_t stride,
+                                      int32_t copy_left, int32_t precision, float alpha, void* stream) {
+    MH_REQUIRE(mh_fuse_corr_bwd_leaky_ok(g_ld, l_ld, r_ld, dl_ld, dr_ld, B, H, W, C, max_disp, stride), MH_ERR_UNSUPPORTED, "mh_fuse_corr_bwd_leaky: not a corr_bwd_direct launch");
+    return corr_bwd_impl(g, g_ld, coff, L, l_ld, R, r_ld, dL, dl_ld, 0, dR, dr_ld, 0, du, acc_u, B, H, W, C, max_disp, stride, copy_left, precision, 1, alpha, stream);
+}
+
+static int corr_bwd_impl(const float* g, int32_t g_ld, int32_t coff, const float* L, int32_t l_ld, const float* R, int32_t r_ld, float* dL, int32_t dl_ld, int32_t acc_l,
+                         float* dR, int32_t dr_ld, int32_t acc_r, float* du, int32_t acc_u, int32_t B, int32_t H, int32_t W, int32_t C, int32_t max_disp, int32_t stride,
+                         int32_t copy_left, int32_t precision, int32_t leaky, float leaky_alpha, void* stream) {
     MH_REQUIRE(precision >= 0 && precision <= 2, MH_ERR_ARG, "mh_corr_bwd_prec: precision must be 0 (fp32), 1 (bf16) or 2 (split-bf16: runs as fp32)");
     MH_REQUIRE(g && L && R && dL && dR, MH_ERR_ARG, "mh_corr_bwd: null argument");
     MH_REQUIRE(B > 0 && H > 0 && W > 0 && C > 0 && max_disp >= 0 && stride >= 1, MH_ERR_ARG, "mh_corr_bwd: bad dimension");
@@ -1662,6 +1697,7 @@
     a.B = B; a.H = H; a.W = W; a.C = C; a.md = max_disp; a.stride = stride; a.D = 2 * max_disp / stride + 1;
     a.copy_left = copy_left;
     a.total = (int64_t)B * H * W * (C / 4);
+    a.leaky = leaky; a.leaky_alpha = leaky_alpha;
     if (precision == 1 && g_corr_direct && a.D > MAXD_SMALL && stride == 1 && !copy_left && !du && C % 16 == 0 && C >= 32 && C <= 256 &&
         (C == 32 || C == 64 || C == 128 || C == 256) && (int64_t)B * H * W * std::max(std::max(g_ld, l_ld), r_ld) * 4 < (1ll << 31) - 64) {
         const int nks = (2 * max_disp + 16 + 31) / 32, rows = 48 + 32 * nks, DPh = (((a.D + 3) & ~3) + 7) & ~7;
@@ -1709,15 +1745,12 @@
             return mh_check_launch("corr_bwd_mfma");
         }
     }
-    {
-        const int64_t npix = (int64_t)B * H * W;
-        const int64_t ldm = std::max(std::max(std::max(g_ld, l_ld), std::max(r_ld, dl_ld)), dr_ld);
-        if (g_corr_direct && a.D <= 5 && npix * ldm * 4 < (1ll << 31) - 64 && a.total < (1ll << 31) - 256) {
-            hipLaunchKernelGGL(corr_bwd_direct<5>, dim3((unsigned)((a.total + 255) / 256)), dim3(256), 0, (hipStream_t)stream, a);
-            mh_note_kernel("corr_bwd_direct<DT=5> C=%d D=%d", C, a.D);
-            return mh_check_launch("corr_bwd_direct");
-        }
-    }
+    if (corr_bwd_direct_ok(g_ld, l_ld, r_ld, dl_ld, dr_ld, B, H, W, C, max_disp, stride)) {
+        hipLaunchKernelGGL(corr_bwd_direct<5>, dim3((unsigned)((a.total + 255) / 256)), dim3(256), 0, (hipStream_t)stream, a);
+        mh_note_kernel("corr_bwd_direct<DT=5> C=%d D=%d%s", C, a.D, leaky ? " + leaky" : "");
+        return mh_check_launch("corr_bwd_direct");
+    }
+    MH_REQUIRE(!leaky, MH_ERR_UNSUPPORTED, "mh_corr_bwd: the leaky epilogue exists in corr_bwd_direct only");
     int blocks = (int)((a.total + 255) / 256);
     if (blocks > 256 * 16) blocks = 256 * 16;
     hipLaunchKernelGGL(corr_bwd_kernel, dim3(blocks), dim3(256), 0, (hipStream_t)stream, a);
diff --git a/real-time-self-adaptive-deep-stereo_amd/csrc/lib.hip b/real-time-self-adaptive-deep-stereo_amd/csrc/lib.hip
--- a/real-time-self-adaptive-deep-stereo_amd/csrc/lib.hip
+++ b/real-time-self-adaptive-deep-stereo_amd/csrc/lib.hip
@@ -372,6 +372,87 @@
 }
 }
 
+enum { FUSE_RESIZE_LOSS = 1, FUSE_RESIZE_BWD_HEAD = 2, FUSE_HEAD_COPY = 4, FUSE_CORR_LEAKY = 8, FUSE_ALL = 15, FUSE_DEFAULT = FUSE_RESIZE_LOSS | FUSE_CORR_LEAKY };
+static std::atomic<int> g_plan_fuse{FUSE_DEFAULT};
+static std::atomic<int> g_plan_fused{0};
+extern "C" int mh_tune_plan_fuse(int mask) {
+    g_plan_fuse.store(mask < 0 ? FUSE_DEFAULT : (mask & FUSE_ALL));
+    return g_plan_fused.exchange(0);
+}
+extern "C" int mh_fuse_resize_loss(const float* in, float* disp, int32_t Hi, int32_t Wi, int32_t Hr, int32_t Wr, int32_t cy, int32_t cx, float mul, int32_t mode,
+                                   const float* left, const float* right, float* ws, float* result, float* ddisp, float grad_scale, int32_t B, int32_t H, int32_t W,
+                                   int32_t phase, void* stream);
+extern "C" int mh_fuse_head_bwd_copy(const mh_head_bwd_desc* d, const float* src0, const float* src1, float* dV, void* dV_shadow, const float* w,
+                                     float* dx, const float* mask_ref, void* dx_shadow, const float* csrc, int32_t csrc_ld, float* cdst, int32_t cdst_ld,
+                                     int64_t cnpix, int32_t cnch, float cscale, void* stream);
+extern "C" int mh_fuse_corr_bwd_leaky_ok(int32_t g_ld, int32_t l_ld, int32_t r_ld, int32_t dl_ld, int32_t dr_ld, int32_t B, int32_t H, int32_t W, int32_t C, int32_t max_disp,
+                                         int32_t stride);
+extern "C" int mh_fuse_corr_bwd_leaky(const float* g, int32_t g_ld, int32_t coff, const float* L, int32_t l_ld, const float* R, int32_t r_ld, float* dL, int32_t dl_ld,
+                                      float* dR, int32_t dr_ld, float* du, int32_t acc_u, int32_t B, int32_t H, int32_t W, int32_t C, int32_t max_disp, int32_t stride,
+                                      int32_t copy_left, int32_t precision, float alpha, void* stream);
+
+static void head_bwd_desc_from_op(const mh_op& o, mh_head_bwd_desc& d) {
+    const int32_t* i = o.i;
+    d.kind = i[0]; d.B = i[1]; d.H = i[2]; d.W = i[3]; d.N = i[4]; d.Hr = i[5]; d.Wr = i[6]; d.cy = i[7]; d.cx = i[8]; d.Ho = i[9]; d.Wo = i[10];
+    d.src0_ld = i[11]; d.src1_ld = i[12]; d.dx_ld = i[13]; d.mask_ld = i[14]; d.accumulate_dx = i[15];
+    d.mul = o.f[0]; d.mask_alpha = o.f[1];
+}
+namespace {
+struct ByteRange { const char* lo; const char* hi; };
+inline ByteRange byte_range(const void* p, int64_t bytes) { const char* c = (const char*)p; return ByteRange{c, p && bytes > 0 ? c + bytes : c}; }
+inline bool ranges_meet(const ByteRange& a, const ByteRange& b) { return a.lo < a.hi && b.lo < b.hi && a.lo < b.hi && b.lo < a.hi; }
+}
+
+static bool try_fuse(const mh_op& a, const mh_op& b, void* s, int* err) {
+    *err = 0;
+    const int mask = g_plan_fuse.load();
+    if (!mask || b.i[26] != 0 || (a.i[26] & 0xff) != 0) return false;
+    const int32_t* ai = a.i; const int32_t* bi = b.i;
+    if ((mask & FUSE_RESIZE_LOSS) && a.kind == MH_OP_RESIZE_FWD && b.kind == MH_OP_LOSS) {
+        if (!((ai[9] == 1 || ai[9] == 2) && (bi[3] == 0 || bi[3] == 1) && a.p[1] && b.p[2] == a.p[1] && bi[0] == ai[0] && bi[1] == ai[7] && bi[2] == ai[8])) return false;
+        const ByteRange out = byte_range(a.p[1], (int64_t)ai[0] * ai[7] * ai[8] * 4);
+        const int64_t n = (int64_t)bi[0] * bi[1] * bi[2];
+        if (ranges_meet(out, byte_range(b.p[0], n * 12)) || ranges_meet(out, byte_range(b.p[1], n * 12)) || ranges_meet(out, byte_range(b.p[5], n * 4)) ||
+            ranges_meet(out, byte_range(a.p[0], (int64_t)ai[0] * ai[1] * ai[2] * 4)) || ranges_meet(byte_range(b.p[5], n * 4), byte_range(a.p[0], (int64_t)ai[0] * ai[1] * ai[2] * 4)))
+            return false;
+        *err = mh_fuse_resize_loss((const float*)a.p[0], (float*)a.p[1], ai[1], ai[2], ai[3], ai[4], ai[5], ai[6], a.f[0], ai[9], (const float*)b.p[0], (const float*)b.p[1],
+                                   (float*)b.p[3], (float*)b.p[4], (float*)b.p[5], b.f[0], bi[0], bi[1], bi[2], bi[3], s);
+        return true;
+    }
+    if ((mask & FUSE_HEAD_COPY) && a.kind == MH_OP_HEAD_BWD && b.kind == MH_OP_COPY_CH) {
+        if (bi[3] != 0 || !b.p[0] || !b.p[1] || b.n <= 0 || bi[2] <= 0 || bi[0] < bi[2] || bi[1] < bi[2]) return false;
+        mh_head_bwd_desc d; head_bwd_desc_from_op(a, d);
+        if (d.B <= 0 || d.H <= 0 || d.W <= 0 || d.N <= 0 || (d.kind != 0 && d.kind != 1)) return false;
+        const int64_t npix = (int64_t)d.B * d.H * d.W;
+        const ByteRange head[8] = {
+            d.kind == 0 ? byte_range(a.p[0], (int64_t)d.B * d.Ho * d.Wo * 4) : byte_range(a.p[0], ((npix - 1) * (int64_t)d.src0_ld + 1) * 4),
+            d.kind == 0 ? byte_range(nullptr, 0) : byte_range(a.p[1], ((npix - 1) * (int64_t)d.src1_ld + 1) * 4),
+            byte_range(a.p[2], npix * 4), byte_range(a.p[3], npix * 32 * 2), byte_range(a.p[4], (int64_t)9 * d.N * 4),
+            byte_range(a.p[5], ((npix - 1) * (int64_t)d.dx_ld + d.N) * 4), byte_range(a.p[6], ((npix - 1) * (int64_t)d.mask_ld + d.N) * 4),
+            byte_range(a.p[7], npix * ((d.N + 31) / 32 * 32) * 2)};
+        const ByteRange cdst = byte_range(b.p[1], ((b.n - 1) * (int64_t)bi[1] + bi[2]) * 4), csrc = byte_range(b.p[0], ((b.n - 1) * (int64_t)bi[0] + bi[2]) * 4);
+        for (int k = 0; k < 8; ++k) if (ranges_meet(cdst, head[k])) return false;
+        for (int k : {2, 3, 5, 7}) if (ranges_meet(csrc, head[k])) return false;
+        if (ranges_meet(csrc, cdst)) return false;
+        *err = mh_fuse_head_bwd_copy(&d, (const float*)a.p[0], (const float*)a.p[1], (float*)a.p[2], a.p[3], (const float*)a.p[4], (float*)a.p[5], (const float*)a.p[6], a.p[7],
+                                     (const float*)b.p[0], bi[0], (float*)b.p[1], bi[1], b.n, bi[2], b.f[0], s);
+        return true;
+    }
+    if ((mask & FUSE_CORR_LEAKY) && a.kind == MH_OP_CORR_BWD && b.kind == MH_OP_LEAKY_BWD) {
+        const int64_t npix = (int64_t)ai[9] * ai[10] * ai[11];
+        const int C = ai[12];
+        if (ai[5] != 0 || ai[7] != 0 || npix <= 0 || !a.p[1] || !a.p[2] || !a.p[3] || !a.p[4]) return false;
+        if (!(b.p[0] == a.p[3] && bi[0] == ai[4] && ai[6] == ai[4] && (const float*)a.p[4] == (const float*)a.p[3] + npix * ai[4] &&
+              b.p[1] == a.p[1] && bi[1] == ai[2] && ai[3] == ai[2] && (const float*)a.p[2] == (const float*)a.p[1] + npix * ai[2] &&
+              b.n == 2 * npix && bi[2] == C)) return false;
+        if (!mh_fuse_corr_bwd_leaky_ok(ai[0], ai[2], ai[3], ai[4], ai[6], ai[9], ai[10], ai[11], C, ai[13], ai[14])) return false;
+        *err = mh_fuse_corr_bwd_leaky((const float*)a.p[0], ai[0], ai[1], (const float*)a.p[1], ai[2], (const float*)a.p[2], ai[3], (float*)a.p[3], ai[4], (float*)a.p[4], ai[6],
+                                      (float*)a.p[5], ai[8], ai[9], ai[10], ai[11], C, ai[13], ai[14], ai[15], ai[16], b.f[0], s);
+        return true;
+    }
+    return false;
+}
+
 static int run_wgrad_batch(const mh_op* ops, int m, void* s) {
     mh_wgrad_item items[16];
     for (int k = 0; k < m; ++k) {
@@ -429,6 +510,7 @@
         if (ops[k].kind == MH_OP_WGRAD_PARTIAL)
             while (m < 16 && k + m < nops && ops[k + m].kind == MH_OP_WGRAD_PARTIAL && (ops[k + m].i[26] & ~MH_OP_NODEFER) == lane) ++m;
         auto run = [&](void* s) -> int { return m > 1 ? run_wgrad_batch(ops + k, m, s) : run_op(ops[k], s); };
+        bool fused = false;
         if (!e && lane > 0) {
             if (!L) e = lanes_get(&L);
             if (!e && stale[lane]) { e = lane_edge(*L, main_s, L->aux[lane]); stale[lane] = false; }
@@ -442,7 +524,9 @@
                 }
             }
         } else if (!e) {
-            e = run(stream);
+            if (m == 1 && k + 1 < nops) fused = try_fuse(ops[k], ops[k + 1], stream, &e);
+            if (fused) { if (!e) ++g_plan_fused; }
+            else e = run(stream);
             for (bool& b : stale) b = true;
             if (!e && ndef) e = flush_deferred();
         }
@@ -454,7 +538,7 @@
             join();
             return e;
         }
-        k += m - 1;
+        k += m - 1 + (fused ? 1 : 0);
     }
     if (ndef) { if (int e = flush_deferred()) { join(); return e; } }
     return join();
diff --git a/real-time-self-adaptive-deep-stereo_amd/csrc/ops.hip b/real-time-self-adaptive-deep-stereo_amd/csrc/ops.hip
--- a/real-time-self-adaptive-deep-stereo_amd/csrc/ops.hip
+++ b/real-time-self-adaptive-deep-stereo_amd/csrc/ops.hip
@@ -107,6 +107,17 @@
     return top + (bot - top) * ty;
 }
 
+__device__ __forceinline__ float resize_fwd_value(const ResizeArgs& p, int b, int y, int x) {
+    int y0, y1, x0, x1; float ty, tx;
+    interp1(y + p.cy, p.sy, p.Hi, y0, y1, ty);
+    interp1(x + p.cx, p.sx, p.Wi, x0, x1, tx);
+    const float* img = p.in + (int64_t)b * p.Hi * p.Wi;
+    float v = bilerp(img, p.Wi, y0, y1, ty, x0, x1, tx, p.mul, p.mode == 1);
+    if (p.mode == 0) v *= p.mul;
+    else if (p.mode == 2) v = fmaxf(v * p.mul, 0.f);
+    return v;
+}
+
 __global__ __launch_bounds__(256) void resize_fwd_kernel(ResizeArgs p) {
     const int64_t total = (int64_t)p.B * p.Ho * p.Wo;
     for (int64_t q = (int64_t)blockIdx.x * 256 + threadIdx.x; q < total; q += (int64_t)gridDim.x * 256) {
@@ -114,14 +125,7 @@
         const int64_t t2 = q / p.Wo;
         const int y = (int)(t2 % p.Ho);
         const int b = (int)(t2 / p.Ho);
-        int y0, y1, x0, x1; float ty, tx;
-        interp1(y + p.cy, p.sy, p.Hi, y0, y1, ty);
-        interp1(x + p.cx, p.sx, p.Wi, x0, x1, tx);
-        const float* img = p.in + (int64_t)b * p.Hi * p.Wi;
-        float v = bilerp(img, p.Wi, y0, y1, ty, x0, x1, tx, p.mul, p.mode == 1);
-        if (p.mode == 0) v *= p.mul;
-        else if (p.mode == 2) v = fmaxf(v * p.mul, 0.f);
-        p.out[q] = v;
+        p.out[q] = resize_fwd_value(p, b, y, x);
     }
 }
 
@@ -233,13 +237,11 @@
     }
     return acc * p.mul;
 }
-__global__ __launch_bounds__(256) void head_bwd_kernel(HeadBwdArgs p) {
-    __shared__ float sV[(HB_TH + 2) * (HB_TW + 2)];
-    __shared__ __attribute__((aligned(16))) float sW[9 * 64];
+__device__ __forceinline__ void head_bwd_body(const HeadBwdArgs& p, int blk, float* sV, float* sW) {
     const int tid = threadIdx.x;
     const int H = p.rz.Hi, W = p.rz.Wi;
-    const int tx = blockIdx.x % p.tiles_x;
-    const int t2 = blockIdx.x / p.tiles_x;
+    const int tx = blk % p.tiles_x;
+    const int t2 = blk / p.tiles_x;
     const int ty = t2 % p.tiles_y, b = t2 / p.tiles_y;
     const int y0 = ty * HB_TH, x0 = tx * HB_TW;
     const bool exact2 = p.kind == 0 && p.rz.Hr == 2 * H && p.rz.Wr == 2 * W && p.rz.cy == 0 && p.rz.cx == 0 && p.rz.Ho == p.rz.Hr && p.rz.Wo == p.rz.Wr;
@@ -330,6 +332,11 @@
         *reinterpret_cast<float4*>(dst) = v;
         if (p.dx_sh) *reinterpret_cast<uint2*>(p.dx_sh + m * p.dx_sh_ld + n) = make_uint2(mh_pack_bf16(v.x, v.y), mh_pack_bf16(v.z, v.w));
     }
+}
+__global__ __launch_bounds__(256) void head_bwd_kernel(HeadBwdArgs p) {
+    __shared__ float sV[(HB_TH + 2) * (HB_TW + 2)];
+    __shared__ __attribute__((aligned(16))) float sW[9 * 64];
+    head_bwd_body(p, blockIdx.x, sV, sW);
 }
 
 struct ResizeImgArgs { const float* in; const float* g; float* out; float* din; int B, Hi, Wi, C, Ho, Wo; float sy, sx; };
@@ -458,6 +465,7 @@
     float* rep; float* drep; float* coef; float* part1; float* part2; float* result; float* ddisp;
     int B, H, W, nblk1, nblk2;
     float grad_scale;
+    ResizeArgs rz;
 };
 
 __device__ __forceinline__ float block_sum(float v, float* red) {
@@ -475,6 +483,7 @@
 #define LT_HW (LT_W + 4)
 #define LT_WH (LT_H + 2)
 #define LT_WW (LT_W + 2)
+template <bool RESIZE>
 __global__ __launch_bounds__(256) void loss_tile_kernel(LossArgs p, int tiles_x, int tiles_y, int with_grad) {
     __shared__ float red[4];
     __shared__ float s_rep[LT_HH * LT_HW * 3];
@@ -506,7 +515,13 @@
             inb[u] = i < LT_HH * LT_HW && (unsigned)y < (unsigned)p.H && (unsigned)x < (unsigned)p.W;
             rbv[u] = (b * p.H + y) * p.W;
             qv[u] = rbv[u] + x;
-            dv[u] = mh_buf_load1(rs_d, inb[u] ? qv[u] * 4 : MH_OOB);
+            if (RESIZE) {
+                const float v = resize_fwd_value(p.rz, b, inb[u] ? y : 0, inb[u] ? x : 0);
+                dv[u] = inb[u] ? v : 0.f;
+                const int ly2 = ly - 2, lx2 = lx - 2;
+                if (inb[u] && (unsigned)ly2 < (unsigned)LT_H && (unsigned)lx2 < (unsigned)LT_W) p.rz.out[qv[u]] = v;
+            } else
+                dv[u] = mh_buf_load1(rs_d, inb[u] ? qv[u] * 4 : MH_OOB);
         }
         float av[NI][3], bv[NI][3], lv[NI][3], w0v[NI], w1v[NI];
 #pragma unroll
@@ -879,16 +894,24 @@
     if (threadIdx.x == 0 && blockIdx.x == 0) { state[0] *= b1; state[1] *= b2; }
 }
 
-__global__ __launch_bounds__(256) void copy_channels_kernel(const float* src, int src_ld, float* dst, int dst_ld, int64_t npix,
-                                                            int nch, float scale, int accumulate) {
-    const int64_t total = npix * nch;
-    for (int64_t q = (int64_t)blockIdx.x * 256 + threadIdx.x; q < total; q += (int64_t)gridDim.x * 256) {
-        const int c = (int)(q % nch);
-        const int64_t pix = q / nch;
-        const float v = scale * src[pix * src_ld + c];
-        float* d = dst + pix * dst_ld + c;
-        *d = accumulate ? *d + v : v;
-    }
+struct CopyChArgs { const float* src; float* dst; int64_t npix; int src_ld, dst_ld, nch, accumulate; float scale; };
+__device__ __forceinline__ void copy_channels_body(const CopyChArgs& p, int blk, int nblk) {
+    const int64_t total = p.npix * p.nch;
+    for (int64_t q = (int64_t)blk * 256 + threadIdx.x; q < total; q += (int64_t)nblk * 256) {
+        const int c = (int)(q % p.nch);
+        const int64_t pix = q / p.nch;
+        const float v = p.scale * p.src[pix * p.src_ld + c];
+        float* d = p.dst + pix * p.dst_ld + c;
+        *d = p.accumulate ? *d + v : v;
+    }
+}
+__global__ __launch_bounds__(256) void copy_channels_kernel(CopyChArgs p) { copy_channels_body(p, blockIdx.x, gridDim.x); }
+
+__global__ __launch_bounds__(256) void head_bwd_copy_kernel(HeadBwdArgs p, CopyChArgs c, int head_wgs) {
+    __shared__ float sV[(HB_TH + 2) * (HB_TW + 2)];
+    __shared__ __attribute__((aligned(16))) float sW[9 * 64];
+    if ((int)blockIdx.x < head_wgs) head_bwd_body(p, blockIdx.x, sV, sW);
+    else copy_channels_body(c, (int)blockIdx.x - head_wgs, (int)gridDim.x - head_wgs);
 }
 
 __global__ __launch_bounds__(256) void leaky_bwd_kernel(float* dy, int dy_ld, const float* y, int y_ld, int64_t npix, int nch, float alpha) {
@@ -1906,14 +1929,14 @@
     return mh_check_launch("resize_bwd");
 }
 
-extern "C" int mh_head_bwd(const mh_head_bwd_desc* d, const float* src0, const float* src1, float* dV, void* dV_shadow, const float* w,
-                           float* dx, const float* mask_ref, void* dx_shadow, void* stream) {
+static int head_bwd_args(HeadBwdArgs& a, int64_t& grid, const mh_head_bwd_desc* d, const float* src0, const float* src1, float* dV, void* dV_shadow, const float* w,
+                         float* dx, const float* mask_ref, void* dx_shadow) {
     MH_REQUIRE(d && dV && w && dx && (src0 || src1), MH_ERR_ARG, "mh_head_bwd: null argument");
     MH_REQUIRE(d->kind == 0 || d->kind == 1, MH_ERR_ARG, "mh_head_bwd: kind must be 0 (resize gradient of a finer level's du) or 1 (addends)");
     MH_REQUIRE(d->B > 0 && d->H > 0 && d->W > 0 && d->N >= 4 && d->N <= 64 && d->N % 4 == 0, MH_ERR_ARG, "mh_head_bwd: bad dimension (N = 4 .. 64, multiple of 4)");
     MH_REQUIRE(d->dx_ld % 4 == 0 && d->dx_ld >= d->N && mh_aligned16(dx) && mh_aligned16(w) && (!mask_ref || (d->mask_ld % 4 == 0 && mh_aligned16(mask_ref))) &&
                (!dx_shadow || mh_aligned16(dx_shadow)), MH_ERR_ALIGN, "mh_head_bwd: dx / mask / w must be 16-byte aligned with lds that are multiples of 4");
-    HeadBwdArgs a{};
+    a = HeadBwdArgs{};
     if (d->kind == 0) {
         MH_REQUIRE(src0, MH_ERR_ARG, "mh_head_bwd: kind 0 needs the finer level's coordinate gradient");
         a.rz.g = src0;
@@ -1928,11 +1951,30 @@
     a.N = d->N; a.dx_ld = d->dx_ld; a.mask_ld = d->mask_ld; a.dx_sh_ld = (d->N + 31) / 32 * 32; a.acc_dx = d->accumulate_dx; a.kind = d->kind;
     a.mask_alpha = d->mask_alpha;
     a.tiles_x = (d->W + HB_TW - 1) / HB_TW; a.tiles_y = (d->H + HB_TH - 1) / HB_TH;
-    const int64_t grid = (int64_t)d->B * a.tiles_x * a.tiles_y;
-    MH_REQUIRE(grid < (1ll << 31), MH_ERR_ARG, "mh_head_bwd: too many tiles");
+    grid = (int64_t)d->B * a.tiles_x * a.tiles_y;
+    MH_REQUIRE(grid < (1ll << 31) - 256 * 16, MH_ERR_ARG, "mh_head_bwd: too many tiles");
+    return 0;
+}
+
+extern "C" int mh_head_bwd(const mh_head_bwd_desc* d, const float* src0, const float* src1, float* dV, void* dV_shadow, const float* w,
+                           float* dx, const float* mask_ref, void* dx_shadow, void* stream) {
+    HeadBwdArgs a; int64_t grid = 0;
+    if (int e = head_bwd_args(a, grid, d, src0, src1, dV, dV_shadow, w, dx, mask_ref, dx_shadow)) return e;
     hipLaunchKernelGGL(head_bwd_kernel, dim3((unsigned)grid), dim3(256), 0, (hipStream_t)stream, a);
     mh_note_kernel("head_bwd_kernel kind %d N=%d", d->kind, d->N);
     return mh_check_launch("head_bwd");
+}
+
+extern "C" int mh_fuse_head_bwd_copy(const mh_head_bwd_desc* d, const float* src0, const float* src1, float* dV, void* dV_shadow, const float* w,
+                                     float* dx, const float* mask_ref, void* dx_shadow, const float* csrc, int32_t csrc_ld, float* cdst, int32_t cdst_ld,
+                                     int64_t cnpix, int32_t cnch, float cscale, void* stream) {
+    HeadBwdArgs a; int64_t grid = 0;
+    if (int e = head_bwd_args(a, grid, d, src0, src1, dV, dV_shadow, w, dx, mask_ref, dx_shadow)) return e;
+    MH_REQUIRE(csrc && cdst && cnpix > 0 && cnch > 0 && csrc_ld >= cnch && cdst_ld >= cnch, MH_ERR_ARG, "mh_copy_channels: bad argument");
+    const CopyChArgs c{csrc, cdst, cnpix, csrc_ld, cdst_ld, cnch, 0, cscale};
+    hipLaunchKernelGGL(head_bwd_copy_kernel, dim3((unsigned)(grid + grid_for(cnpix * cnch))), dim3(256), 0, (hipStream_t)stream, a, c, (int)grid);
+    mh_note_kernel("head_bwd_copy_kernel kind %d N=%d + copy of %d channels", d->kind, d->N, cnch);
+    return mh_check_launch("head_bwd_copy");
 }
 
 extern "C" int mh_pad_reflect(const float* in, float* out, int32_t B, int32_t H, int32_t W, int32_t C,
@@ -1962,8 +2004,8 @@
     return mh_reprojection_loss_phase(left, right, disp, ws, result, ddisp, grad_scale, B, H, W, 0, stream);
 }
 
-extern "C" int mh_reprojection_loss_phase(const float* left, const float* right, const float* disp, float* ws, float* result,
-                                          float* ddisp, float grad_scale, int32_t B, int32_t H, int32_t W, int32_t phase, void* stream) {
+static int reprojection_loss_impl(const float* left, const float* right, const float* disp, float* ws, float* result,
+                                  float* ddisp, float grad_scale, int32_t B, int32_t H, int32_t W, int32_t phase, const ResizeArgs* rz, void* stream) {
     MH_REQUIRE(phase >= 0 && phase <= 2, MH_ERR_ARG, "mh_reprojection_loss_phase: phase must be 0 (all), 1 (maps + gradient) or 2 (final reduction)");
     MH_REQUIRE(left && right && disp && ws && result, MH_ERR_ARG, "mh_reprojection_loss: null argument");
     MH_REQUIRE(B > 0 && H >= 3 && W >= 3, MH_ERR_ARG, "mh_reprojection_loss: image must be at least 3x3");
@@ -1980,9 +2022,28 @@
     a.part1 = ws + 8 * n + 12 * nw; a.nblk1 = (int)ntiles;
     a.part2 = a.part1 + ntiles; a.nblk2 = (int)ntiles;
     hipStream_t s = (hipStream_t)stream;
-    if (phase != 2) hipLaunchKernelGGL(loss_tile_kernel, dim3((unsigned)ntiles), dim3(256), 0, s, a, tiles_x, tiles_y, ddisp ? 1 : 0);
+    if (rz) {
+        a.rz = *rz;
+        hipLaunchKernelGGL(loss_tile_kernel<true>, dim3((unsigned)ntiles), dim3(256), 0, s, a, tiles_x, tiles_y, ddisp ? 1 : 0);
+        mh_note_kernel("loss_tile_kernel<resize mode %d>", rz->mode);
+    } else if (phase != 2) hipLaunchKernelGGL(loss_tile_kernel<false>, dim3((unsigned)ntiles), dim3(256), 0, s, a, tiles_x, tiles_y, ddisp ? 1 : 0);
     if (phase != 1) hipLaunchKernelGGL(loss_final_kernel, dim3(1), dim3(256), 0, s, a);
     return mh_check_launch("reprojection_loss");
+}
+
+extern "C" int mh_reprojection_loss_phase(const float* left, const float* right, const float* disp, float* ws, float* result,
+                                          float* ddisp, float grad_scale, int32_t B, int32_t H, int32_t W, int32_t phase, void* stream) {
+    return reprojection_loss_impl(left, right, disp, ws, result, ddisp, grad_scale, B, H, W, phase, nullptr, stream);
+}
+
+extern "C" int mh_fuse_resize_loss(const float* in, float* disp, int32_t Hi, int32_t Wi, int32_t Hr, int32_t Wr, int32_t cy, int32_t cx, float mul, int32_t mode,
+                                   const float* left, const float* right, float* ws, float* result, float* ddisp, float grad_scale, int32_t B, int32_t H, int32_t W,
+                                   int32_t phase, void* stream) {
+    MH_REQUIRE(in && disp, MH_ERR_ARG, "mh_resize_fwd: null argument");
+    MH_REQUIRE((mode == 1 || mode == 2) && (phase == 0 || phase == 1), MH_ERR_UNSUPPORTED, "mh_fuse_resize_loss: resize mode 1 / 2 and loss phase 0 / 1 only");
+    ResizeArgs rz{}; rz.in = in; rz.out = disp;
+    if (int e = resize_args(rz, B, Hi, Wi, Hr, Wr, cy, cx, H, W, mul, mode)) return e;
+    return reprojection_loss_impl(left, right, disp, ws, result, ddisp, grad_scale, B, H, W, phase, &rz, stream);
 }
 
 extern "C" int64_t mh_metrics_ws_floats(int32_t B, int32_t H, int32_t W) { return 3 * nblk((int64_t)B * H * W) + 16; }
@@ -2089,8 +2150,8 @@
 extern "C" int mh_copy_channels(const float* src, int32_t src_ld, float* dst, int32_t dst_ld, int64_t npix,
                                 int32_t nch, float scale, int32_t accumulate, void* stream) {
     MH_REQUIRE(src && dst && npix > 0 && nch > 0 && src_ld >= nch && dst_ld >= nch, MH_ERR_ARG, "mh_copy_channels: bad argument");
-    hipLaunchKernelGGL(copy_channels_kernel, dim3(grid_for(npix * nch)), dim3(256), 0, (hipStream_t)stream,
-                       src, src_ld, dst, dst_ld, npix, nch, scale, accumulate);
+    const CopyChArgs a{src, dst, npix, src_ld, dst_ld, nch, accumulate, scale};
+    hipLaunchKernelGGL(copy_channels_kernel, dim3(grid_for(npix * nch)), dim3(256), 0, (hipStream_t)stream, a);
     return mh_check_launch("copy_channels");
 }
 
diff --git a/real-time-self-adaptive-deep-stereo_amd/madnet_hip/_ffi.py b/real-time-self-adaptive-deep-stereo_amd/madnet_hip/_ffi.py
--- a/real-time-self-adaptive-deep-stereo_amd/madnet_hip/_ffi.py
+++ b/real-time-self-adaptive-deep-stereo_amd/madnet_hip/_ffi.py
@@ -138,6 +138,7 @@
     "mh_wgrad_stream_plan": (_I, [C.POINTER(WgsLayer), _I, _I, _I, C.POINTER(C.c_int32)]),
     "mh_wgrad_stream": (_I, [_P, _I, _I, _I, _I, _P]),
     "mh_tune_wgrad_stream": (_I, [_I]),
+    "mh_tune_plan_fuse": (_I, [_I]),
     "mh_proxy_ws_floats": (_L, [_I, _I, _I]),
     "mh_proxy_loss": (_I, [_P, _P, _P, _P, _P, _F, _F, _I, _I, _I, _P]),
     "mh_proxy_scaled_ws_floats": (_L, [_I, _I, _I, _I]),
@@ -212,7 +213,7 @@
     "mh_event_destroy": (_I, [_P]),
     "mh_stream_sync": (_I, [_P]),
 }
-_NO_STATUS = {"mh_comm_available", "mh_deterministic_overflow", "mh_bias_grad_blocks", "mh_tune_conv_bank_small", "mh_conv_image_ok", "mh_level_front_head_ok", "mh_deterministic_ranges", "mh_planes_kc16", "mh_conv2d_planes_bwd_ok", "mh_stamp_rate_khz", "mh_pack32_bytes", "mh_conv2d_planes_ok", "mh_tune_conv_planes", "mh_tune_wgrad_target_pct", "mh_tune_wgrad_image", "mh_conv2d_takes_shadows", "mh_tune_conv_bank_tile", "mh_tune_conv_rows", "mh_last_error", "mh_last_kernel", "mh_tune_conv_bank", "mh_pack_bytes", "mh_abi_version", "mh_tune_conv_patch", "mh_crc32c", "mh_device_count", "mh_loss_ws_floats", "mh_metrics_ws_floats", "mh_proxy_ws_floats", "mh_proxy_scaled_ws_floats", "mh_metrics_kitti_ws_floats", "mh_frame_prepare_ws_floats", "mh_sgm_ws_bytes", "mh_sgm_ws_bytes_ex", "mh_sgm_ws_bytes_scaled", "mh_sgm_speckle_ws_bytes"}
+_NO_STATUS = {"mh_tune_plan_fuse", "mh_comm_available", "mh_deterministic_overflow", "mh_bias_grad_blocks", "mh_tune_conv_bank_small", "mh_conv_image_ok", "mh_level_front_head_ok", "mh_deterministic_ranges", "mh_planes_kc16", "mh_conv2d_planes_bwd_ok", "mh_stamp_rate_khz", "mh_pack32_bytes", "mh_conv2d_planes_ok", "mh_tune_conv_planes", "mh_tune_wgrad_target_pct", "mh_tune_wgrad_image", "mh_conv2d_takes_shadows", "mh_tune_conv_bank_tile", "mh_tune_conv_rows", "mh_last_error", "mh_last_kernel", "mh_tune_conv_bank", "mh_pack_bytes", "mh_abi_version", "mh_tune_conv_patch", "mh_crc32c", "mh_device_count", "mh_loss_ws_floats", "mh_metrics_ws_floats", "mh_proxy_ws_floats", "mh_proxy_scaled_ws_floats", "mh_metrics_kitti_ws_floats", "mh_frame_prepare_ws_floats", "mh_sgm_ws_bytes", "mh_sgm_ws_bytes_ex", "mh_sgm_ws_bytes_scaled", "mh_sgm_speckle_ws_bytes"}
 
 
 class MadnetHipError(RuntimeError):
```

New measurement: 747.3 pairs/s (median of 6 runs). About the same (+0.3%).
